# brunohs1993/Nanokappa

Hardware: AMD Instinct MI355X
Metric: phonon-steps/sec (whole node) (higher is better)
Workload: dtype f64

## Files before the change

nanokappa_amd/csrc/nk_device.h:

```cpp
#pragma once
#include <hip/hip_runtime.h>
#include <stdint.h>

#define NK_WG 256
#ifndef NK_NREP
#define NK_NREP 8
#endif
#define NK_PLANE_DOUBLES 6
#define NK_FACE_DOUBLES 16
#define NK_LDS_FACES 256
#define NK_LDS_RESFACES 64
#define NK_TAU_ROWS 3
#define NK_MAX_SEGMENTS 16384
#define NK_EMIT_CHUNK 128
#define NK_LREC 128
#define NK_NEWBORN 0x80000000u
#define NK_LOST 0x40000000u

#define NK_TAG_REFLECT 0x00000u
#define NK_TAG_EMIT 0x10000u
#define NK_TAG_RESAMP 0x20000u
#define NK_TAG_DICE 0x30000u
#define NK_TAG_INIT 0x40000u

template <class T>
struct NkField {
    T *p;
    int32_t blk;
    __host__ __device__ __forceinline__ int64_t off(int64_t i) const { return (i >> 6) * (int64_t)blk + (i & 63); }
    __host__ __device__ __forceinline__ T &operator[](int64_t i) const { return p[off(i)]; }
    __host__ __device__ __forceinline__ T *operator+(int64_t i) const { return p + off(i); }
    __host__ __device__ __forceinline__ T *tile(int64_t i0, int lane) const { return p + ((i0 >> 6) * (int64_t)blk + lane); }
    __host__ __device__ __forceinline__ explicit operator bool() const { return p != nullptr; }
};

template <bool NTS, bool PID>
struct NkBlock {
    static constexpr int NF = 4 + (NTS ? 1 : 0) + (PID ? 1 : 0);
    static constexpr int BD = NF * 64 + 32;
    static constexpr int O_Y = 64, O_Z = 128, O_OCC = 192, O_NTS = 256, O_PID = 64 * (NTS ? 5 : 4), O_W0 = 64 * NF;
    static __device__ __forceinline__ double *slot(double *s0, int64_t i) { return s0 + (i >> 6) * (int64_t)BD + (i & 63); }
    static __device__ __forceinline__ double *tile(double *s0, int64_t i0, int lane) { return s0 + (i0 >> 6) * (int64_t)BD + lane; }
    static __device__ __forceinline__ uint32_t *word(double *s0, int64_t i) { return reinterpret_cast<uint32_t *>(s0 + (i >> 6) * (int64_t)BD + O_W0) + (i & 63); }
};

struct __attribute__((aligned(16))) NkFacet {
    double cx, cy, cz;
    double nx, ny, nz;
    double tx, ty, tz;
    int32_t bc;
    int32_t partner;
    int32_t res;
    int32_t rough;
    int32_t pad[2];
};

struct __attribute__((aligned(64))) NkMode {
    double omega, vx, vy, vz;
    double E0;
    double tau[NK_TAU_ROWS];
};

struct NkDev {
    int32_t Q, J, NT, M;
    const NkMode *modetab;
    const NkMode *modetab_p;
    const int32_t *m2s;
    const int32_t *s2m;
    const int32_t *seg_nl;
    int32_t tau_row0;
    double tau_g[NK_TAU_ROWS];
    double tau_ig[NK_TAU_ROWS - 1];
    double T0, invT0;
    double c_hk;
    const double *tau;
    const double *Tgrid;
    int32_t nE;
    const double *Tarr, *Earr;
    double Tfill_lo, Tfill_hi;
    double hbar, kb, QV;
    double active_modes;
    int32_t F, Fc, NP;
    const float *tree_boxes;
    double tree_bound;
    const int32_t *tree_tags;
    const double *facet_skip;
    const double *tree_faces;
    int32_t tree_base[8];
    int32_t tree_top, tree_leaves;
    int32_t tree_nfam, tree_lds_fam0, tree_lds_off;
    int32_t NG;
    const double *planes;
    const double *faces;
    const NkFacet *facets;
    double tol;
    double bbox[6];
    int32_t box;
    double box_k[6];
    uint64_t box_ids;
    double inv_dt;
    const double *face_verts;
    const int32_t *facet_face_off;
    const int32_t *facet_face_idx;
    const double *facet_face_cdf;
    int32_t nS;
    const double *simplex_pts;
    const double *simplex_cdf;
    int32_t S, sv_kind, sv_axis, sv_interp;
    const double *centers;
    const double *sv_volume;
    double sv_lo, sv_invL;
    double *T_sv;
    const double *rbf_inv;
    int32_t rbf_P, rbf_used[3];
    double rbf_shift[3], rbf_scale[3];
    int32_t R, res_gen;
    const int32_t *res_facet;
    const double *res_T;
    const int32_t *res_face_off;
    const double *res_face_cdf;
    const double *res_face_verts;
    int32_t res_nf;
    int32_t res_lds;
    const double *enter_prob;
    double *res_counter;
    const double *ep_p;
    double *rc_p;
    int64_t rc_len;
    const double *res_roulette;
    int32_t *nleave_prev;
    uint64_t *sp_inbox;
    int32_t *sp_inbox_n;
    int32_t sp_icap;
    int32_t Fr;
    const double *specularity;
    const uint8_t *true_spec;
    const int32_t *spec_map;
    const double *roulette;
    const int32_t *roul_lut;
    int32_t roul_nlut;
    const int32_t *degen_j2;
    double dt;
    int32_t norm_fixed, T_ref_local;
    double particle_density, T_ref;
    uint64_t seed;
    int32_t rank, nranks;
    int64_t cap;
    int32_t nseg, segcap;
    int32_t *seg_count;
    int32_t *seg_new;
    int32_t *seg_lo;
    int32_t down;
    int32_t *seg_bound;
    NkField<double> x, y, z, occ, nts;
    NkField<uint32_t> w0;
    NkField<uint64_t> pid;
    int32_t part;
    int32_t lb;
    int32_t nlmax;
    int32_t nlrec;
    int32_t *ticket;
    int32_t *overflow;
    int32_t *halt;
    double *qx, *qy, *qz, *qocc, *qnts;
    uint32_t *qw0;
    uint64_t *qpid;
    int32_t *seg_evq;
    int32_t *ev_ticket;
    double2 *mig_buf;
    int32_t *mig_n;
    int32_t mig_cap;
    double *partials;
    int32_t NB;
    unsigned long long *stamps;
};

struct NkSlot { int64_t od, ow; };
__device__ __forceinline__ NkSlot nk_slot(const NkDev &d, int64_t i) {
    const int64_t b = i >> 6, l = i & 63;
    NkSlot s;
    s.od = b * (int64_t)d.x.blk + l;
    s.ow = b * (int64_t)d.w0.blk + l;
    return s;
}

__device__ __forceinline__ void nk_philox(uint32_t c0, uint32_t c1, uint32_t c2, uint32_t c3, uint32_t k0, uint32_t k1,
                                          uint32_t o[4]) {
#pragma unroll
    for (int r = 0; r < 10; ++r) {
        uint32_t hi0 = __umulhi(0xD2511F53u, c0), lo0 = 0xD2511F53u * c0;
        uint32_t hi1 = __umulhi(0xCD9E8D57u, c2), lo1 = 0xCD9E8D57u * c2;
        uint32_t n0 = hi1 ^ c1 ^ k0, n2 = hi0 ^ c3 ^ k1;
        c0 = n0; c1 = lo1; c2 = n2; c3 = lo0;
        k0 += 0x9E3779B9u; k1 += 0xBB67AE85u;
    }
    o[0] = c0; o[1] = c1; o[2] = c2; o[3] = c3;
}
__device__ __forceinline__ double nk_u53(uint32_t hi, uint32_t lo) {
    uint64_t w = ((uint64_t)hi << 32) | lo;
    return (double)(w >> 11) * (1.0 / 9007199254740992.0);
}
__device__ __forceinline__ void nk_uniform2_dev(uint64_t seed, uint64_t pid, uint32_t step, uint32_t tag, double &u0,
                                                double &u1) {
    uint32_t o[4];
    nk_philox((uint32_t)pid, (uint32_t)(pid >> 32), step, tag, (uint32_t)seed, (uint32_t)(seed >> 32), o);
    u0 = nk_u53(o[0], o[1]);
    u1 = nk_u53(o[2], o[3]);
}

__device__ __forceinline__ int nk_ss_left(const double *a, int n, double x) {
    int lo = 0, hi = n;
    while (lo < hi) { int mid = (lo + hi) >> 1; if (a[mid] < x) lo = mid + 1; else hi = mid; }
    return lo;
}
__device__ __forceinline__ int nk_ss_right(const double *a, int n, double x) {
    int lo = 0, hi = n;
    while (lo < hi) { int mid = (lo + hi) >> 1; if (a[mid] <= x) lo = mid + 1; else hi = mid; }
    return lo;
}
__device__ __forceinline__ int nk_ss_left_hint(const double *a, int n, double x, int hint) {
    int lo, hi;
    hint = hint < 0 ? 0 : (hint > n - 1 ? n - 1 : hint);
    if (a[hint] < x) {
        int stepw = 1;
        lo = hint + 1; hi = lo;
        while (hi < n && a[hi] < x) { lo = hi + 1; hi += stepw; stepw <<= 1; }
        if (hi > n) hi = n;
    } else {
        int stepw = 1;
        hi = hint; lo = hint;
        while (lo > 0 && !(a[lo - 1] < x)) { hi = lo - 1; lo -= stepw; stepw <<= 1; if (lo < 0) lo = 0; }
        if (lo > 0 && !(a[lo - 1] < x)) lo = 0;
    }
    while (lo < hi) { int mid = (lo + hi) >> 1; if (a[mid] < x) lo = mid + 1; else hi = mid; }
    return lo;
}
__device__ __forceinline__ double nk_interp_lin_hint(const double *xs, const double *ys, int n, double x, int hint, int &idx_out) {
    int idx = nk_ss_left_hint(xs, n, x, hint);
// ... 664 lines not shown
```

nanokappa_amd/csrc/nk_engine.hip:

```cpp
#include <hip/hip_runtime.h>
#include <dlfcn.h>
#include <math.h>
#include <stdio.h>
#include <stdlib.h>
#include <string.h>
#include <algorithm>
#include <functional>
#include <queue>
#include <string>
#include <type_traits>
#include <chrono>
#include <time.h>
#include <vector>

#include <rccl/rccl.h>

#include "../../include/nanokappa_hip.h"
#include "nk_kernels.h"
#include "nk_field.h"
#include "nk_fgroups.h"
#include "nk_modes.h"
#include "nk_group.h"
#ifndef NK_PLAIN_IN_ENGINE
extern template __global__ void k_sweep<1, false, false, false, false, true, 1>(NkDev, uint32_t, int, int);
// ... 59 lines not shown
    double *rb_k2 = nullptr, *rb_nin = nullptr, *rb_eta = nullptr, *rb_sub = nullptr, *rb_spec = nullptr, *rb_roul = nullptr;
    uint8_t *rb_ts = nullptr;
    unsigned int *rb_map = nullptr;
    std::vector<int32_t> rb_facet;
    int64_t o2o_first = 0;
    bool stepped = false;
    int64_t emitted_for = -1;
    std::vector<double> h_vg;
    std::vector<int32_t> h_m2s, h_s2m;
    int32_t *m2s_dev = nullptr, *s2m_dev = nullptr, *nl_dev = nullptr;
    unsigned int *rbar = nullptr;
    bool walked = false;
    int64_t ev_lds_set = -1;
    int map_nseg = 0;
    NkMode *modetab_p = nullptr;
    int64_t modetab_p_len = 0;
    void *inbox = nullptr, *inbox_n = nullptr;
    void *mig_buf = nullptr, *mig_n = nullptr;
    double *ep_p = nullptr, *rc_p = nullptr;
    int rm_nseg = 0, rm_nlmax = 0;
    void *pin = nullptr;
    size_t pin_bytes = 0;
    int32_t halt_words[4] = {0, 0, 0, 0};
    double *acc = nullptr;
    double *hist = nullptr;
    int hist_cap = 0;
    nk_params params;
    nk_timing timing;
    NkRccl rccl;
    ncclComm_t comm = nullptr;
    int comm_rank = -1, comm_nranks = 0;
    double comm_selftest = 0.0;
    int num_cu = 256;
    std::vector<int32_t> h_ffo, h_ffi;
    std::vector<double> h_fcdf, h_verts;
    std::vector<double> h_rbf_inv;
    std::vector<NkFacet> host_facets;
    const double *d_omega = nullptr, *d_vg = nullptr;
    std::vector<double> h_Tgrid;
    double T_lo = 0.0, T_hi = 0.0;
    int32_t band_B = 0;
    int32_t *band_map = nullptr;
    double *band_slabs = nullptr;
    size_t band_slabs_n = 0;
    double *band_rows_d = nullptr;
    size_t band_rows_n = 0;
    std::vector<double> band_rows;
    std::vector<int64_t> band_steps;
    NkFieldHost field;
    NkFGroupsHost fgroups;
    int64_t map_gen = 0;
    NkModesHost modes;
    double res_T_max = 0.0;
};

#define NK_HIP(call)                                                                                   \
    do {                                                                                               \
        hipError_t e_ = (call);                                                                        \
        if (e_ != hipSuccess) {                                                                        \
            ctx->err = std::string(#call) + ": " + hipGetErrorString(e_);                              \
            return NK_ERR_HIP;                                                                         \
        }                                                                                              \
    } while (0)
#define NK_ARG(cond, msg)                                                                              \
    do {                                                                                               \
        if (!(cond)) { ctx->err = msg; return NK_ERR_ARG; }                                            \
    } while (0)

template <class T>
static int nk_upload(nk_ctx *ctx, const T *src, size_t n, const T **dst, bool particle = false) {
    void *p = nullptr;
    size_t bytes = (n ? n : 1) * sizeof(T);
    NK_HIP(hipMalloc(&p, bytes));
    (particle ? ctx->pallocs : ctx->allocs).push_back(p);
    if (src && n) NK_HIP(hipMemcpy(p, src, n * sizeof(T), hipMemcpyHostToDevice));
    else NK_HIP(hipMemset(p, 0, bytes));
    *dst = (const T *)p;
    return NK_OK;
}
#define NK_UP(src, n, dst)                                                                             \
    do { int rc_ = nk_upload(ctx, src, n, dst); if (rc_) return rc_; } while (0)

static inline bool nk_layout_soa() { return false; }
static inline int nk_particle_bytes(bool with_pid, bool with_nts) { return 36 + (with_nts ? 8 : 0) + (with_pid ? 8 : 0); }
static inline size_t nk_store_bytes(int64_t cap, bool with_pid, bool with_nts) {
    const int64_t nblk = (cap + 63) / 64;
    const int nf = 4 + (with_nts ? 1 : 0) + (with_pid ? 1 : 0);
    const int bd = nf * 64 + 32;
    const size_t bytes = nk_layout_soa() ? (size_t)nblk * 64 * (nf * 8 + 4) : (size_t)nblk * bd * 8;
    return bytes ? bytes : 64;
}
static void nk_point_fields(NkDev &d, double *b, int64_t cap, bool with_pid, bool with_nts) {
    const int64_t nblk = (cap + 63) / 64;
    const int nf = 4 + (with_nts ? 1 : 0) + (with_pid ? 1 : 0);
    const int bd = nf * 64 + 32;
    if (nk_layout_soa()) {
        const int64_t n = nblk * 64;
        int k = 4;
        d.x = {b, 64}; d.y = {b + n, 64}; d.z = {b + 2 * n, 64}; d.occ = {b + 3 * n, 64};
        d.nts = {with_nts ? b + (k++) * n : nullptr, 64};
        d.pid = {with_pid ? (uint64_t *)(b + (k++) * n) : nullptr, 64};
        d.w0 = {(uint32_t *)(b + k * n), 64};
    } else {
        int k = 4;
        d.x = {b, bd}; d.y = {b + 64, bd}; d.z = {b + 128, bd}; d.occ = {b + 192, bd};
        d.nts = {with_nts ? b + 64 * (k++) : nullptr, bd};
        d.pid = {with_pid ? (uint64_t *)(b + 64 * (k++)) : nullptr, bd};
        d.w0 = {(uint32_t *)(b + 64 * k), 2 * bd};
    }
}
static int nk_alloc_fields(nk_ctx *ctx, NkDev &d, int64_t cap, bool with_pid, bool with_nts) {
    const size_t bytes = nk_store_bytes(cap, with_pid, with_nts);
    void *buf = nullptr;
    const size_t pad = getenv("NK_STORE_PAD_KB") ? (size_t)atol(getenv("NK_STORE_PAD_KB")) * 1024 : 0;
    NK_HIP(hipMalloc(&buf, bytes + pad));
    ctx->pallocs.push_back(buf);
    NK_HIP(hipMemsetAsync(buf, 0, bytes + pad, ctx->stream));
    ctx->store_buf = buf; ctx->store_pad = pad; ctx->store_pid = with_pid; ctx->store_nts = with_nts;
    nk_point_fields(d, (double *)((char *)buf + pad), cap, with_pid, with_nts);
    return NK_OK;
}
template <class T>
static int nk_field_download(nk_ctx *ctx, const NkDev &d, const NkField<T> &f, std::vector<T> &out) {
    out.resize((size_t)d.cap);
    const int64_t nblk = d.cap / 64;
    if (nblk == 0) return NK_OK;
    NK_HIP(hipMemcpy2D(out.data(), 64 * sizeof(T), f.p, (size_t)f.blk * sizeof(T), 64 * sizeof(T), (size_t)nblk, hipMemcpyDeviceToHost));
    return NK_OK;
}
template <class T>
static int nk_field_upload(nk_ctx *ctx, const NkDev &d, const NkField<T> &f, const T *src) {
    const int64_t nblk = d.cap / 64;
    if (nblk == 0) return NK_OK;
    NK_HIP(hipMemcpy2D(f.p, (size_t)f.blk * sizeof(T), src, 64 * sizeof(T), 64 * sizeof(T), (size_t)nblk, hipMemcpyHostToDevice));
    return NK_OK;
}

static inline int nk_geom_mode(const nk_ctx *ctx) { return (ctx->d.F <= NK_LDS_FACES && ctx->d.Fc <= NK_LDS_FACES) ? 1 : 2; }
static inline bool nk_want_split(const nk_ctx *ctx);
static inline size_t nk_lds(const nk_ctx *ctx, bool geom, int kind = 0) {
    const NkDev &d = ctx->d;
    const int gm = geom ? nk_geom_mode(ctx) : 0;
    return nk_lds_bytes(d.S, d.R, d.F, d.NP, d.Fc, gm, kind, (gm == 1 && d.res_lds) ? d.res_nf : 0, d.rbf_P, d.nlrec, nk_want_split(ctx) ? 0 : 1);
}
#define NK_GEOM_LAUNCH(kernel, grid, lds, ...)                                                        \
    do {                                                                                               \
        if (nk_geom_mode(ctx) == 1) kernel<1><<<grid, NK_WG, lds, ctx->stream>>>(__VA_ARGS__);         \
        else kernel<2><<<grid, NK_WG, lds, ctx->stream>>>(__VA_ARGS__);                                \
    } while (0)
#define NK_EMIT_LAUNCH(kernel, grid, lds, ...)                                                        \
    do {                                                                                               \
        if (ctx->d.box) kernel<1, true><<<grid, NK_WG, lds, ctx->stream>>>(__VA_ARGS__);               \
        else if (nk_geom_mode(ctx) == 1) kernel<1, false><<<grid, NK_WG, lds, ctx->stream>>>(__VA_ARGS__);   \
        else kernel<2, false><<<grid, NK_WG, lds, ctx->stream>>>(__VA_ARGS__);                         \
    } while (0)
static inline int nk_sweep_grid(const nk_ctx *ctx) { return ctx->num_cu * 8; }
#define NK_SWEEP_CASE(G, R, B, P, S, lrec, STMT) { if (lrec) { auto KERNEL = k_sweep<G, R, B, P, S, true>; STMT; } else { auto KERNEL = k_sweep<G, R, B, P, S, false>; STMT; } }
#define NK_SWEEP_CASE_FAST(lrec, fast, STMT)                                                                                   \
    { if (lrec) { if ((fast) == 1) { auto KERNEL = k_sweep<1, false, false, false, false, true, 1>; STMT; } else { auto KERNEL = k_sweep<1, false, false, false, false, true, 2>; STMT; } } \
      else { if ((fast) == 1) { auto KERNEL = k_sweep<1, false, false, false, false, false, 1>; STMT; } else { auto KERNEL = k_sweep<1, false, false, false, false, false, 2>; STMT; } } }
#define NK_SWEEP_CASE_S(G, R, B, P, split, lrec, STMT) { if (split) NK_SWEEP_CASE(G, R, B, P, true, lrec, STMT) else NK_SWEEP_CASE(G, R, B, P, false, lrec, STMT) }
#define NK_SWEEP_CASE_RP(G, B, rough, pid, split, lrec, STMT)                                         \
    { if (rough) NK_SWEEP_CASE_S(G, true, B, true, split, lrec, STMT) else if (pid) NK_SWEEP_CASE_S(G, false, B, true, split, lrec, STMT) else NK_SWEEP_CASE_S(G, false, B, false, split, lrec, STMT) }
#define NK_SWEEP_CASE_BOX(R, B, P, lrec, STMT) { if (lrec) { auto KERNEL = k_sweep<1, R, B, P, false, true, 0, true>; STMT; } else { auto KERNEL = k_sweep<1, R, B, P, false, false, 0, true>; STMT; } }
#define NK_SWEEP_CASE_BOX_RP(B, rough, pid, lrec, STMT)                                               \
    { if (rough) NK_SWEEP_CASE_BOX(true, B, true, lrec, STMT) else if (pid) NK_SWEEP_CASE_BOX(false, B, true, lrec, STMT) else NK_SWEEP_CASE_BOX(false, B, false, lrec, STMT) }
#define NK_SWEEP_CASE_FAST_BOX(lrec, fast, STMT)                                                                               \
    { if (lrec) { if ((fast) == 1) { auto KERNEL = k_sweep<1, false, false, false, false, true, 1, true>; STMT; } else { auto KERNEL = k_sweep<1, false, false, false, false, true, 2, true>; STMT; } } \
      else { if ((fast) == 1) { auto KERNEL = k_sweep<1, false, false, false, false, false, 1, true>; STMT; } else { auto KERNEL = k_sweep<1, false, false, false, false, false, 2, true>; STMT; } } }
#define NK_SWEEP_DISPATCH(gm, rough, rbf, pid, split, lrec, STMT)                                     \
    do {                                                                                               \
        const int fast_ = ((gm) == 1 && !(rough) && !(rbf) && !(pid) && !(split)) ? nk_sweep_fast(ctx) : 0;   \
        if (ctx->d.box && (gm) == 1 && !(split)) {                                                     \
            if (fast_) { NK_SWEEP_CASE_FAST_BOX(lrec, fast_, STMT) break; }                            \
            if (rbf) NK_SWEEP_CASE_BOX_RP(true, rough, pid, lrec, STMT) else NK_SWEEP_CASE_BOX_RP(false, rough, pid, lrec, STMT)   \
            break;                                                                                     \
        }                                                                                              \
        if (fast_) { NK_SWEEP_CASE_FAST(lrec, fast_, STMT) break; }                                    \
        if ((gm) == 1) { if (rbf) NK_SWEEP_CASE_RP(1, true, rough, pid, split, lrec, STMT) else NK_SWEEP_CASE_RP(1, false, rough, pid, split, lrec, STMT) }   \
        else { if (rbf) NK_SWEEP_CASE_RP(2, true, rough, pid, split, lrec, STMT) else NK_SWEEP_CASE_RP(2, false, rough, pid, split, lrec, STMT) }             \
    } while (0)
static inline int nk_sweep_fast(const nk_ctx *ctx) {
    const NkDev &d = ctx->d;
    if (getenv("NK_NO_FAST")) return 0;
    return (d.sv_kind == 0 && d.T_ref_local && (d.sv_interp == 0 || d.sv_interp == 1)) ? 1 + d.sv_interp : 0;
}
static inline bool nk_want_lrec(const nk_ctx *ctx) { return ctx->d.nlrec > 0; }
#define NK_EVENTS_CASE(G, R, B, P, STMT) { auto KERNEL = k_events<G, R, B, P>; STMT; }
#define NK_EVENTS_CASE_RP(G, B, rough, pid, STMT)                                                     \
    { if (rough) NK_EVENTS_CASE(G, true, B, true, STMT) else if (pid) NK_EVENTS_CASE(G, false, B, true, STMT) else NK_EVENTS_CASE(G, false, B, false, STMT) }
#define NK_EVENTS_DISPATCH(gm, rough, rbf, pid, STMT)                                                 \
// ... 478 lines not shown
    ctx->host_facets = fct;
    NK_UP(fct.data(), fct.size(), &d.facets);
    {
        std::vector<double> fs((size_t)m->Fc * 2, 0.0);
        for (int f = 0; f < m->F; ++f) {
            const int fc = m->face_facet[f];
            if (fc < 0 || fc >= m->Fc) continue;
            const NkFacet &q = fct[fc];
            const double nx = m->normals[3 * f], ny = m->normals[3 * f + 1], nz = m->normals[3 * f + 2];
            const double dn = std::max(fabs(nx - q.nx), std::max(fabs(ny - q.ny), fabs(nz - q.nz)));
            const double dk = fabs(nx * q.cx + ny * q.cy + nz * q.cz + m->k[f]);
            fs[2 * (size_t)fc] = std::max(fs[2 * (size_t)fc], dn);
            fs[2 * (size_t)fc + 1] = std::max(fs[2 * (size_t)fc + 1], dk);
        }
        std::vector<int> nfaces((size_t)m->Fc, 0);
        for (int f = 0; f < m->F; ++f) if (m->face_facet[f] >= 0 && m->face_facet[f] < m->Fc) ++nfaces[m->face_facet[f]];
        for (int fc = 0; fc < m->Fc; ++fc) if (nfaces[fc] < 16) fs[2 * (size_t)fc] = 1e300;
        NK_UP(fs.data(), fs.size(), &d.facet_skip);
    }
    d.nS = m->nS;
    if (m->nS > 0) {
        NK_UP(m->simplex_pts, (size_t)m->nS * 12, &d.simplex_pts);
        std::vector<double> sc((size_t)m->nS);
        double tot = 0.0, acc = 0.0;
        for (int s = 0; s < m->nS; ++s) tot += m->simplex_vol[s];
        for (int s = 0; s < m->nS; ++s) { acc += m->simplex_vol[s] / tot; sc[s] = acc; }
        for (int s = 0; s < m->nS; ++s) sc[s] /= sc[m->nS - 1];
        NK_UP(sc.data(), sc.size(), &d.simplex_cdf);
    }
    ctx->mesh_box = false;
    if (d.cap == 0) d.box = 0;
    if (m->F == 12 && m->Fc == 6 && d.NP == 6) {
        bool ok = true;
        int seen = 0;
        int box_facet[6] = {0, 0, 0, 0, 0, 0};
        d.box_ids = 0;
        for (int pl = 0; pl < 6 && ok; ++pl) {
            const double *pn = &planes[(size_t)pl * NK_PLANE_DOUBLES];
            int a = -1, sgn = 0;
            for (int k = 0; k < 3; ++k) {
                if (pn[k] == 1.0 || pn[k] == -1.0) { if (a >= 0) ok = false; a = k; sgn = pn[k] > 0 ? 1 : 0; }
                else if (pn[k] != 0.0) ok = false;
            }
            if (!ok || a < 0) { ok = false; break; }
            const int w = 2 * a + sgn;
            if (seen & (1 << w)) { ok = false; break; }
            seen |= 1 << w;
            const double wall = sgn ? -pn[3] : pn[3];
            if (!(fabs(wall - m->bbox[(sgn ? 3 : 0) + a]) <= 1e-9 * (1.0 + fabs(wall)))) { ok = false; break; }
            if (members[pl].size() != 2) { ok = false; break; }
            int fct0 = -1, face0 = 0x7fffffff;
            double area = 0.0;
            for (int f : members[pl]) {
                if (fct0 < 0) fct0 = m->face_facet[f]; else if (m->face_facet[f] != fct0) ok = false;
                face0 = std::min(face0, f);
                area += m->face_area[f];
                const double *V = m->vertices + 9 * (size_t)f;
                for (int c = 0; c < 3 && ok; ++c)
                    for (int k = 0; k < 3; ++k) {
                        const double v = V[3 * c + k], lo = m->bbox[k], hi = m->bbox[3 + k];
                        const double e = 1e-9 * (1.0 + fabs(lo) + fabs(hi));
                        if (k == a) { if (fabs(v - wall) > e) ok = false; }
                        else if (fabs(v - lo) > e && fabs(v - hi) > e) ok = false;
                    }
            }
            const int b = (a + 1) % 3, c = (a + 2) % 3;
            const double side = (m->bbox[3 + b] - m->bbox[b]) * (m->bbox[3 + c] - m->bbox[c]);
            if (!(fabs(area - side) <= 1e-9 * side) || fct0 < 0 || fct0 >= m->Fc) ok = false;
            if (!ok) break;
            d.box_k[w] = pn[3];
            box_facet[w] = fct0;
            d.box_ids = (d.box_ids & ~(0xFFull << (8 * w))) | ((uint64_t)(fct0 & 15) << (8 * w)) | ((uint64_t)(face0 & 15) << (8 * w + 4));
        }
        if (ok && seen == 63) {
            int fm = 0;
            for (int w = 0; w < 6; ++w) fm |= 1 << box_facet[w];
            ctx->mesh_box = fm == 63;
        }
    }
    ctx->have_mesh = true;
    return NK_OK;
}

static inline bool nk_want_box(const nk_ctx *ctx) {
    return ctx->have_mesh && ctx->mesh_box && !ctx->box_forbidden && !getenv("NK_NO_BOX") && !getenv("NK_SPLIT") && !nk_layout_soa() &&
           ctx->d.F <= NK_LDS_FACES && ctx->d.Fc <= NK_LDS_FACES;
}

static int nk_patch_facets(nk_ctx *ctx) {
    NK_HIP(hipMemcpy((void *)ctx->d.facets, ctx->host_facets.data(), (size_t)ctx->d.Fc * sizeof(NkFacet), hipMemcpyHostToDevice));
    return NK_OK;
}

static int nk_entry_tables_drop(nk_ctx *ctx, bool keep_counters) {
    NkDev &d = ctx->d;
    if (ctx->rm_nseg > 0 && keep_counters && d.R > 0 && d.res_counter) {
        const int64_t n = (int64_t)d.R * d.M;
        k_perm_rm<<<(int)((n + 255) / 256), 256, 0, ctx->stream>>>(0, d.R, d.M, ctx->rm_nseg, ctx->rm_nlmax,
                                                                   d.m2s, d.res_counter, ctx->rc_p + (ctx->step & 1) * d.rc_len);
        NK_HIP(hipGetLastError());
        NK_HIP(hipStreamSynchronize(ctx->stream));
    }
    if (ctx->ep_p) { hipFree(ctx->ep_p); ctx->ep_p = nullptr; }
    if (ctx->rc_p) { hipFree(ctx->rc_p); ctx->rc_p = nullptr; }
    d.ep_p = nullptr; d.rc_p = nullptr;
    ctx->rm_nseg = 0;
    return NK_OK;
}
static int nk_entry_tables_build(nk_ctx *ctx) {
    NkDev &d = ctx->d;
    if (!(d.R > 0 && d.nseg > 0 && d.m2s && d.enter_prob && d.res_counter) || ctx->rm_nseg == d.nseg) return NK_OK;
    int rc = nk_entry_tables_drop(ctx, true);
    if (rc) return rc;
    const size_t len = (size_t)d.nseg * d.R * d.nlmax;
    NK_HIP(hipMalloc((void **)&ctx->ep_p, len * 8));
    NK_HIP(hipMalloc((void **)&ctx->rc_p, 2 * len * 8));
    NK_HIP(hipMemsetAsync(ctx->ep_p, 0, len * 8, ctx->stream));
    NK_HIP(hipMemsetAsync(ctx->rc_p, 0, 2 * len * 8, ctx->stream));
    d.rc_len = (int64_t)len;
    const int64_t n = (int64_t)d.R * d.M;
    k_perm_rm<<<(int)((n + 255) / 256), 256, 0, ctx->stream>>>(1, d.R, d.M, d.nseg, d.nlmax, d.m2s, (double *)d.enter_prob, ctx->ep_p);
    k_perm_rm<<<(int)((n + 255) / 256), 256, 0, ctx->stream>>>(1, d.R, d.M, d.nseg, d.nlmax, d.m2s, d.res_counter, ctx->rc_p + (ctx->step & 1) * d.rc_len);
    NK_HIP(hipGetLastError());
    d.ep_p = ctx->ep_p; d.rc_p = ctx->rc_p;
    ctx->rm_nseg = d.nseg;
    ctx->rm_nlmax = d.nlmax;
    return NK_OK;
}

static int nk_alloc_tally(nk_ctx *ctx) {
    NkDev &d = ctx->d;
    d.NB = 5 * d.S + 5 * d.R + 1;
    if (ctx->acc) { hipFree(ctx->acc); ctx->acc = nullptr; }
    if (ctx->hist) { hipHostFree(ctx->hist); ctx->hist = nullptr; }
    ctx->hist_cap = 0;
    NK_HIP(hipMalloc((void **)&ctx->acc, (size_t)(d.NB + 2) * sizeof(double)));
    NK_HIP(hipMemset(ctx->acc, 0, (size_t)(d.NB + 2) * sizeof(double)));
    const double *p;
    NK_UP((const double *)nullptr, (size_t)(ctx->num_cu * 16) * d.NB, &p);
    d.partials = (double *)p;
    return NK_OK;
}

static void nk_rbf_coefficients(nk_ctx *ctx, std::vector<double> &T) {
    const int S = ctx->d.S, P = ctx->d.rbf_P;
    T.resize((size_t)S + P);
    for (int j = 0; j < P; ++j) {
        double a = 0.0;
        for (int i = 0; i < S; ++i) a += ctx->h_rbf_inv[(size_t)j * P + i] * T[i];
        T[(size_t)S + j] = a;
    }
}

int nk_set_subvolumes(nk_ctx *ctx, const nk_subvols *s, const double *T_sv_init) {
    if (ctx) ctx->emitted_for = -1;
    NK_ARG(ctx && s && T_sv_init, "nk_set_subvolumes: NULL argument");
    NK_ARG(s->S > 0 && s->S <= 512, "nk_set_subvolumes: S must be in [1, 512]");
    NK_ARG(ctx->have_material, "nk_set_subvolumes: call nk_set_material first");
    NK_HIP(hipSetDevice(ctx->device));
    NkDev &d = ctx->d;
    d.S = s->S; d.sv_kind = s->kind; d.sv_axis = s->axis; d.sv_interp = s->interp;
    NK_ARG(s->axis >= 0 && s->axis < 3, "nk_set_subvolumes: axis");
    NK_ARG(!(s->kind != 0 && s->interp != 2 && s->interp != 3), "nk_set_subvolumes: slice interpolation needs slice subvolumes");
    NK_ARG(s->interp >= 0 && s->interp <= 3, "nk_set_subvolumes: interp must be 0..3");
    NK_UP(s->centers, (size_t)s->S * 3, &d.centers);
    NK_UP(s->volumes, (size_t)s->S, &d.sv_volume);
    d.rbf_P = 0;
// ... 134 lines not shown
        }
        if (r->degen_j2) NK_UP(r->degen_j2, (size_t)d.M, &d.degen_j2); else d.degen_j2 = nullptr;
        for (int i = 0; i < r->Fr; ++i) {
            NK_ARG(r->facet[i] >= 0 && r->facet[i] < d.Fc, "nk_set_rough: facet index");
            ctx->host_facets[r->facet[i]].rough = i;
        }
        return nk_patch_facets(ctx);
    }
    return NK_OK;
}

int nk_set_params(nk_ctx *ctx, const nk_params *p) {
    if (ctx) ctx->emitted_for = -1;
    NK_ARG(ctx && p, "nk_set_params: NULL argument");
    NK_ARG(p->dt > 0, "nk_set_params: dt must be positive");
    ctx->params = *p;
    NkDev &d = ctx->d;
    d.dt = p->dt; d.inv_dt = 1.0 / p->dt; d.norm_fixed = p->norm_fixed; d.particle_density = p->particle_density;
    d.T_ref_local = p->T_ref_local; d.T_ref = p->T_ref;
    ctx->have_params = true;
    return NK_OK;
}

struct NkHostParticles {
    std::vector<double> x, y, z, occ, nts;
    std::vector<int32_t> mode, facet;
    std::vector<uint64_t> pid;
};
static int nk_normalize(nk_ctx *ctx, int honor_halt = 0) {
    NkDev &d = ctx->d;
    d.down = 0;
    if (!ctx->walked || !d.seg_lo) return NK_OK;
    k_anchor<<<ctx->num_cu * 8, NK_WG, 0, ctx->stream>>>(d, honor_halt);
    NK_HIP(hipGetLastError());
    if (!honor_halt) ctx->walked = false;
    return NK_OK;
}
static int nk_gather_live(nk_ctx *ctx, NkHostParticles &h, bool want_all) {
    NkDev &d = ctx->d;
    if (d.cap == 0) return NK_OK;
    { int rcn_ = nk_normalize(ctx); if (rcn_) return rcn_; }
    NK_HIP(hipStreamSynchronize(ctx->stream));
    std::vector<int32_t> cnt((size_t)d.nseg);
    NK_HIP(hipMemcpy(cnt.data(), d.seg_count, (size_t)d.nseg * 4, hipMemcpyDeviceToHost));
    int64_t live = 0;
    for (int c : cnt) live += c;
    ctx->h_seg_count = cnt;
    if (!want_all) { h.x.resize((size_t)live); return NK_OK; }
    std::vector<double> bd;
    std::vector<uint32_t> bw;
    std::vector<uint64_t> bu;
    auto keep = [&](const auto &all, auto *dst) {
        for (int sgm = 0; sgm < d.nseg; ++sgm) {
            memcpy(dst, all.data() + (size_t)sgm * d.segcap, (size_t)cnt[sgm] * sizeof(*dst));
            dst += cnt[sgm];
        }
    };
    h.x.resize(live); h.y.resize(live); h.z.resize(live); h.occ.resize(live); h.nts.resize(live);
    h.mode.resize(live); h.facet.resize(live); h.pid.assign(live, 0);
    std::vector<uint32_t> w0((size_t)live);
    int rc;
    if ((rc = nk_field_download(ctx, d, d.x, bd))) return rc; keep(bd, h.x.data());
    if ((rc = nk_field_download(ctx, d, d.y, bd))) return rc; keep(bd, h.y.data());
    if ((rc = nk_field_download(ctx, d, d.z, bd))) return rc; keep(bd, h.z.data());
    if ((rc = nk_field_download(ctx, d, d.occ, bd))) return rc; keep(bd, h.occ.data());
    std::vector<int32_t> bfc;
    if (d.nts) { if ((rc = nk_field_download(ctx, d, d.nts, bd))) return rc; keep(bd, h.nts.data()); }
    else {
        if (ctx->have_material && ctx->have_mesh && ctx->have_sv && d.modetab) {
            double *dn = nullptr; int32_t *df = nullptr;
            NK_HIP(hipMalloc((void **)&dn, (size_t)d.cap * 8));
            if (hipMalloc((void **)&df, (size_t)d.cap * 4) != hipSuccess) { hipFree(dn); ctx->err = "nk_gather_live: out of memory"; return NK_ERR_HIP; }
            hipMemsetAsync(dn, 0, (size_t)d.cap * 8, ctx->stream); hipMemsetAsync(df, 0xff, (size_t)d.cap * 4, ctx->stream);
            k_next_hit<1><<<nk_sweep_grid(ctx), NK_WG, nk_lds(ctx, true), ctx->stream>>>(d, dn, df);
            bd.resize((size_t)d.cap); bfc.resize((size_t)d.cap);
            hipError_t e1 = hipGetLastError();
            if (e1 == hipSuccess) e1 = hipMemcpy(bd.data(), dn, (size_t)d.cap * 8, hipMemcpyDeviceToHost);
            if (e1 == hipSuccess) e1 = hipMemcpy(bfc.data(), df, (size_t)d.cap * 4, hipMemcpyDeviceToHost);
            hipFree(dn); hipFree(df);
            if (e1 != hipSuccess) { ctx->err = std::string("nk_gather_live: ") + hipGetErrorString(e1); return NK_ERR_HIP; }
            keep(bd, h.nts.data());
        } else { std::fill(h.nts.begin(), h.nts.end(), 0.0); }
    }
    if ((rc = nk_field_download(ctx, d, d.w0, bw))) return rc; keep(bw, w0.data());
    if (d.pid) { if ((rc = nk_field_download(ctx, d, d.pid, bu))) return rc; keep(bu, h.pid.data()); }
    const uint32_t lbmask = (1u << d.lb) - 1u;
    int64_t k = 0;
    for (int sgm = 0; sgm < d.nseg; ++sgm)
        for (int j = 0; j < cnt[sgm]; ++j, ++k) {
            const uint32_t idx = w0[(size_t)k] & lbmask;
            h.mode[(size_t)k] = d.part ? ctx->h_s2m[(size_t)sgm * d.nlmax + idx] : (int32_t)idx;
            if (d.nts) h.facet[(size_t)k] = (int32_t)(w0[(size_t)k] >> d.lb) - 1;
            else h.facet[(size_t)k] = (w0[(size_t)k] & NK_LOST) ? -1 : (bfc.empty() ? 0 : bfc[(size_t)sgm * d.segcap + j]);
        }
    return NK_OK;
}

static int nk_scatter(nk_ctx *ctx, int64_t N, const double *x, const double *y, const double *z, const int32_t *mode,
                      const double *occ, const double *n_ts, const int32_t *facet, const uint64_t *pid, uint64_t pid_offset) {
    if (ctx) ctx->emitted_for = -1;
    NkDev &d = ctx->d;
    const int M = d.M;
    for (int64_t i = 0; i < N; ++i) NK_ARG(mode[i] >= 0 && mode[i] < M, "nk_upload_particles: mode index out of range");
    std::vector<int64_t> order((size_t)N);
    std::vector<int64_t> start((size_t)d.nseg + 1, 0);
    if (d.part) {
        const std::vector<int32_t> &m2s = ctx->h_m2s;
        for (int64_t i = 0; i < N; ++i) start[(size_t)(m2s[(size_t)mode[i]] % d.nseg) + 1] += 1;
        for (int sgm = 0; sgm < d.nseg; ++sgm) start[(size_t)sgm + 1] += start[(size_t)sgm];
        std::vector<int64_t> key((size_t)N);
        for (int64_t i = 0; i < N; ++i) { order[(size_t)i] = i; key[(size_t)i] = (int64_t)(m2s[(size_t)mode[i]] % d.nseg) * ((int64_t)d.nlmax + 1) + m2s[(size_t)mode[i]] / d.nseg; }
        std::stable_sort(order.begin(), order.end(), [&](int64_t a, int64_t b) { return key[(size_t)a] < key[(size_t)b]; });
    } else {
        std::vector<int64_t> mstart((size_t)M + 1, 0);
        for (int64_t i = 0; i < N; ++i) mstart[(size_t)mode[i] + 1] += 1;
        for (int m = 0; m < M; ++m) mstart[(size_t)m + 1] += mstart[(size_t)m];
        std::vector<int64_t> cur(mstart.begin(), mstart.end() - 1);
        for (int64_t i = 0; i < N; ++i) order[(size_t)cur[(size_t)mode[i]]++] = i;
        for (int sgm = 0; sgm <= d.nseg; ++sgm) start[(size_t)sgm] = (N * sgm) / d.nseg;
    }
    std::vector<int32_t> cnt((size_t)d.nseg);
    for (int sgm = 0; sgm < d.nseg; ++sgm) {
        cnt[(size_t)sgm] = (int32_t)(start[(size_t)sgm + 1] - start[(size_t)sgm]);
        NK_ARG(cnt[(size_t)sgm] <= d.segcap, "nk_upload_particles: segment capacity too small");
    }
    auto put = [&](const auto *src, const auto &field) -> int {
        typedef typename std::remove_const<typename std::remove_pointer<decltype(src)>::type>::type T;
        std::vector<T> all((size_t)d.cap, T(0));
        for (int sgm = 0; sgm < d.nseg; ++sgm) {
            const int64_t lo = start[(size_t)sgm], n = cnt[(size_t)sgm];
            T *o = all.data() + (size_t)sgm * d.segcap;
            for (int64_t k = 0; k < n; ++k) o[k] = src[order[(size_t)(lo + k)]];
        }
        return nk_field_upload(ctx, d, field, all.data());
    };
    int rc;
    if ((rc = put(x, d.x)) || (rc = put(y, d.y)) || (rc = put(z, d.z)) || (rc = put(occ, d.occ))) return rc;
    if (n_ts && d.nts && (rc = put(n_ts, d.nts))) return rc;
    {
        std::vector<uint32_t> w0((size_t)N);
        for (int64_t i = 0; i < N; ++i) {
            const int32_t fc = facet ? facet[i] : -1;
            NK_ARG(fc >= -1 && fc < d.Fc, "nk_upload_particles: facet index out of range");
            const uint32_t idx = d.part ? (uint32_t)(ctx->h_m2s[(size_t)mode[i]] / d.nseg) : (uint32_t)mode[i];
            w0[(size_t)i] = d.nts ? (((uint32_t)(fc + 1) << d.lb) | idx) : (((facet && fc < 0) ? NK_LOST : 0u) | idx);
        }
        if ((rc = put((const uint32_t *)w0.data(), d.w0))) return rc;
    }
    if (d.pid) {
        if (pid) { if ((rc = put(pid, d.pid))) return rc; }
        else {
            std::vector<uint64_t> ids((size_t)N);
            for (int64_t i = 0; i < N; ++i) ids[(size_t)i] = pid_offset + (uint64_t)i;
            if ((rc = put((const uint64_t *)ids.data(), d.pid))) return rc;
        }
    }
    NK_HIP(hipMemcpy(d.seg_count, cnt.data(), (size_t)d.nseg * 4, hipMemcpyHostToDevice));
    if (d.seg_lo) NK_HIP(hipMemset(d.seg_lo, 0, (size_t)d.nseg * 4));
    ctx->walked = false;
    ctx->h_seg_count = cnt;
    return NK_OK;
}

static inline bool nk_want_pid(const nk_ctx *ctx) { return ctx->d.Fr > 0 || ctx->params.track_ids != 0; }
static inline bool nk_want_split(const nk_ctx *ctx) {
    if (const char *e = getenv("NK_SPLIT")) return atoi(e) != 0;
    return ctx->have_mesh && !(ctx->d.F <= NK_LDS_FACES && ctx->d.Fc <= NK_LDS_FACES);
}
static inline bool nk_want_part(const nk_ctx *ctx) { return !getenv("NK_NO_PARTITION"); }

static int nk_sweep_blocks(nk_ctx *ctx) {
    NkDev &d = ctx->d;
    if (!(ctx->have_material && ctx->have_mesh && ctx->have_sv)) return ctx->num_cu * NK_SWEEP_OCC;
    const int gm_ = nk_geom_mode(ctx);
    const bool rough_ = d.Fr > 0, rbf_ = d.sv_interp == 3, pid_ = nk_want_pid(ctx), split_ = nk_want_split(ctx);
    const bool lrec_ = nk_want_lrec(ctx);
    const int key = gm_ | (rough_ << 2) | (rbf_ << 3) | (pid_ << 4) | (split_ << 5) | (lrec_ << 6) | (nk_sweep_fast(ctx) << 7) | ((d.box ? 1 : 0) << 9);
    const size_t lds_w = nk_lds(ctx, true, pid_ ? 3 : 2);
    if (ctx->g_sweep == 0 || ctx->g_sweep_key != key || ctx->g_sweep_lds != lds_w) {
        int per_cu = 0;
        hipError_t e_ = hipSuccess;
        NK_SWEEP_DISPATCH(gm_, rough_, rbf_, pid_, split_, lrec_, (e_ = hipOccupancyMaxActiveBlocksPerMultiprocessor(&per_cu, KERNEL, NK_WG, lds_w)));
        if (e_ != hipSuccess || per_cu < 1) per_cu = 1;
        if (per_cu > 8) per_cu = 8;
        { const int bound = NK_SWEEP_BOUND(gm_, rough_, rbf_, split_); if (per_cu > bound) per_cu = bound; }
        if (const char *e = getenv("NK_SWEEP_PER_CU")) { int v = atoi(e); if (v >= 1 && v < per_cu) per_cu = v; }
        ctx->g_sweep = ctx->num_cu * per_cu;
        ctx->g_sweep_key = key;
        ctx->g_sweep_lds = lds_w;
        if (getenv("NK_VERBOSE")) fprintf(stderr, "[nanokappa_hip] sweep: %d workgroups per CU (occupancy query rc %d), %zu B LDS each\n", per_cu, (int)e_, lds_w);
    }
    return ctx->g_sweep;
}

static inline int nk_mode_seg(const nk_ctx *ctx, int m, int nseg) {
    return (ctx->map_nseg == nseg && !ctx->h_m2s.empty()) ? ctx->h_m2s[(size_t)m] % nseg : m % nseg;
}

static int nk_build_mode_map(nk_ctx *ctx) {
    NkDev &d = ctx->d;
    if (ctx->m2s_dev) { hipFree(ctx->m2s_dev); ctx->m2s_dev = nullptr; }
    if (ctx->s2m_dev) { hipFree(ctx->s2m_dev); ctx->s2m_dev = nullptr; }
    if (ctx->nl_dev) { hipFree(ctx->nl_dev); ctx->nl_dev = nullptr; }
    d.m2s = nullptr; d.s2m = nullptr; d.seg_nl = nullptr;
    ctx->h_m2s.clear(); ctx->h_s2m.clear(); ctx->map_nseg = 0;
    ctx->map_gen += 1;
    if (d.M <= 0 || d.nseg <= 0) return NK_OK;
    const int M = d.M, nseg = d.nseg, nlmax = d.nlmax;
    const bool plain = !d.part;
    std::vector<int32_t> nl((size_t)nseg, 0);
    ctx->h_m2s.assign((size_t)M, 0);
    ctx->h_s2m.assign((size_t)nseg * nlmax, -1);
    auto place = [&](int m, int seg) {
        const int l = nl[(size_t)seg]++;
        ctx->h_m2s[(size_t)m] = l * nseg + seg;
        ctx->h_s2m[(size_t)seg * nlmax + l] = m;
    };
    if (plain) {
        for (int m = 0; m < M; ++m) place(m, m % nseg);
    } else {
        std::vector<double> rate((size_t)M, 0.0);
        std::vector<char> active((size_t)M, 1);
        const bool have_v = ctx->h_vg.size() == (size_t)M * 3;
        if (have_v) {
            double inv[3] = {0, 0, 0};
            if (ctx->have_mesh) for (int a = 0; a < 3; ++a) { const double e = d.bbox[3 + a] - d.bbox[a]; inv[a] = e > 0.0 ? 1.0 / e : 0.0; }
            for (int m = 0; m < M; ++m) {
                const double *v = &ctx->h_vg[3 * (size_t)m];
                active[(size_t)m] = (v[0] != 0.0 || v[1] != 0.0 || v[2] != 0.0) ? 1 : 0;
                rate[(size_t)m] = fabs(v[0]) * inv[0] + fabs(v[1]) * inv[1] + fabs(v[2]) * inv[2];
// ... 102 lines not shown
        if (hi > 1.12 * lo && !force) break;
        if (bytes * cand.size() > free_b / 3) break;
        if (std::chrono::duration<double, std::milli>(std::chrono::steady_clock::now() - wall0).count() > 1000.0) break;
        void *buf = nullptr;
        if (hipMalloc(&buf, bytes) != hipSuccess) { (void)hipGetLastError(); break; }
        cand.push_back(buf); ms.push_back(0.0);
        if (hipMemsetAsync(buf, 0, bytes, ctx->stream) != hipSuccess) { rc = NK_ERR_HIP; ctx->err = "nk_place_store: hipMemsetAsync failed"; break; }
        rc = probe(buf, ms.back());
    }
    hipEventDestroy(e0); hipEventDestroy(e1);
    size_t best = 0, worst = 0;
    for (size_t k = 1; k < cand.size(); ++k) { if (ms[k] < ms[best]) best = k; if (ms[k] > ms[worst]) worst = k; }
    if (force) best = cand.size() - 1;
    if (!rc && best != 0 && (ms[best] < 0.97 * ms[0] || force)) {
        if (hipMemcpyAsync(cand[best], cand[0], bytes, hipMemcpyDeviceToDevice, ctx->stream) != hipSuccess ||
            hipStreamSynchronize(ctx->stream) != hipSuccess) { rc = NK_ERR_HIP; ctx->err = "nk_place_store: copy into the chosen store failed"; }
        else {
            for (void *&p : ctx->pallocs) if (p == cand[0]) p = cand[best];
            ctx->store_buf = cand[best];
            nk_point_fields(d, (double *)cand[best], d.cap, ctx->store_pid, ctx->store_nts);
            std::swap(cand[0], cand[best]);
        }
    } else best = 0;
    for (size_t k = 1; k < cand.size(); ++k) hipFree(cand[k]);
    const double gb = 2.0 * (double)d.nseg * tiles * 64 * (pbytes - (ctx->store_pid ? 8 : 0)) / 1e9;
    ctx->timing.place_tries = (int64_t)cand.size();
    ctx->timing.place_gbps = ms[best] > 0.0 ? gb / (ms[best] * 1e-3) : 0.0;
    ctx->timing.place_worst_gbps = ms[worst] > 0.0 ? gb / (ms[worst] * 1e-3) : 0.0;
    if (rc) {
        if (getenv("NK_VERBOSE")) fprintf(stderr, "[nanokappa_hip] store placement: probe failed (%s); the store stays where it is\n", ctx->err.c_str());
        (void)hipGetLastError();
        rc = NK_OK;
    }
    if (getenv("NK_VERBOSE")) {
        fprintf(stderr, "[nanokappa_hip] store placement: %zu allocation(s) of %.0f MB probed:", cand.size(), (double)bytes / 1048576.0);
        for (size_t k = 0; k < ms.size(); ++k) fprintf(stderr, " %.1f", ms[k] * 1e3);
        fprintf(stderr, " us per pass; kept number %zu (%.2f TB/s); %.1f ms\n", best, ctx->timing.place_gbps / 1e3,
                std::chrono::duration<double, std::milli>(std::chrono::steady_clock::now() - wall0).count());
    }
    return rc;
}

static inline int64_t nk_tiled_count(int64_t u, int64_t nu, int64_t pid_lo, int64_t N) {
    const int64_t first = pid_lo % nu;
    return N / nu + (((u - first + nu) % nu) < N % nu ? 1 : 0);
}
static int nk_alloc_particles(nk_ctx *ctx, int64_t capacity, const int32_t *mode = nullptr, int64_t N = 0,
                              const int32_t *umodes = nullptr, int64_t nu = 0, int64_t pid_lo = 0) {
    if (ctx) ctx->emitted_for = -1;
    NkDev &d = ctx->d;
    { int rc0 = nk_entry_tables_drop(ctx, true); if (rc0) return rc0; }
    for (void *p : ctx->pallocs) hipFree(p);
    ctx->pallocs.clear();
    d.part = nk_want_part(ctx) ? 1 : 0;
    d.box = nk_want_box(ctx) ? 1 : 0;
    d.nlrec = 0;
    int64_t nseg = 0;
    for (int round = 0; round < 4; ++round) {
        const int64_t waves = (int64_t)nk_sweep_blocks(ctx) * (NK_WG / 64);
        int64_t ns = capacity / 128;
        if (const char *e = getenv("NK_SEGMENTS")) ns = atoi(e) > 0 ? atoi(e) : ns;
        else if (ns >= waves) ns = waves;
        ns = ns < 64 ? 64 : (ns > NK_MAX_SEGMENTS ? NK_MAX_SEGMENTS : ns);
        const bool same = ns == nseg;
        nseg = ns;
        d.nseg = (int32_t)nseg;
        d.nlmax = d.M > 0 ? (int32_t)((d.M + nseg - 1) / nseg) : 1;
        if (d.part && d.M > nseg) d.nlmax += d.nlmax / 6 + 2;
        d.nlrec = 0;
        if (d.part && d.nlmax <= NK_LREC && !getenv("NK_NO_LREC")) {
            const int without = nk_sweep_blocks(ctx);
            d.nlrec = d.nlmax;
            if (nk_sweep_blocks(ctx) < without) d.nlrec = 0;
        }
        if (same) break;
    }
    NK_ARG(d.nlmax < (1 << 14), "too many modes per segment for k_emit's packed entry word: use more particles (segments) or fewer modes");
    { int rcm = nk_build_mode_map(ctx); if (rcm) return rcm; }
    {
        const int64_t maxidx = d.part ? d.nlmax - 1 : (d.M > 0 ? d.M - 1 : 0);
        int lb = 1;
        while ((1ll << lb) <= maxidx) ++lb;
        NK_ARG(lb < 30 && (int64_t)d.Fc + 1 < (1ll << (31 - lb)), "mesh has too many facets for the packed particle word (facets x modes)");
        d.lb = lb;
    }
    int64_t segcap = (capacity + nseg - 1) / nseg;
    if (d.part && (mode || umodes) && N > 0) {
        std::vector<int64_t> per((size_t)nseg, 0);
        if (mode) { for (int64_t i = 0; i < N; ++i) if (mode[i] >= 0 && mode[i] < d.M) per[(size_t)nk_mode_seg(ctx, mode[i], (int)nseg)] += 1; }
        else for (int64_t u = 0; u < nu; ++u) per[(size_t)nk_mode_seg(ctx, umodes[u], (int)nseg)] += nk_tiled_count(u, nu, pid_lo, N);
        int64_t mx = 0;
        for (int64_t v : per) mx = std::max(mx, v);
        segcap = std::max(segcap, mx + mx / 4 + 64);
    }
    const bool tight = getenv("NK_TIGHT_STORE") != nullptr;
    if (ctx->have_material && d.R > 0 && !ctx->h_enter_prob.empty())
        segcap = (tight ? segcap : std::max(segcap, segcap / 8 * 9)) + (tight ? 1 : 2) * nk_spawn_bound(ctx, (int)nseg) + 2 * NK_TILE;
    segcap = ((segcap + 63) / 64) * 64;
    NK_ARG(nseg * segcap < (1ll << 31), "particle store too large for 32-bit slot arithmetic");
    d.segcap = (int32_t)segcap;
    d.cap = nseg * segcap;
    ctx->timing.slots = d.cap;
    const double *pd; const uint32_t *pw; const int32_t *pi; const uint64_t *pu;
#define NK_PALLOC(T, field, ptr, count)                                                                \
    do { int rc_ = nk_upload<T>(ctx, nullptr, (size_t)(count), &ptr, true); if (rc_) return rc_; d.field = (T *)ptr; } while (0)
    { int rcf = nk_alloc_fields(ctx, d, d.cap, nk_want_pid(ctx), !d.box); if (rcf) return rcf; }
    NK_PALLOC(int32_t, seg_count, pi, d.nseg);
    NK_PALLOC(int32_t, seg_new, pi, d.nseg);
    NK_PALLOC(int32_t, seg_bound, pi, d.nseg);
    d.seg_lo = nullptr; d.down = 0; ctx->walked = false;
    NK_PALLOC(int32_t, seg_lo, pi, d.nseg);
    d.qx = d.qy = d.qz = d.qocc = d.qnts = nullptr; d.qw0 = nullptr; d.qpid = nullptr; d.seg_evq = nullptr;
    if (nk_want_split(ctx)) {
        NK_PALLOC(double, qx, pd, d.cap); NK_PALLOC(double, qy, pd, d.cap); NK_PALLOC(double, qz, pd, d.cap);
        NK_PALLOC(double, qocc, pd, d.cap); NK_PALLOC(double, qnts, pd, d.cap);
        NK_PALLOC(uint32_t, qw0, pw, d.cap);
        if (d.pid) NK_PALLOC(uint64_t, qpid, pu, d.cap);
        NK_PALLOC(int32_t, seg_evq, pi, 2 * (size_t)d.nseg + 1);
    }
#ifdef NK_STAMPS
    { const unsigned long long *ps; int rc_ = nk_upload<unsigned long long>(ctx, nullptr, (size_t)d.nseg * 16, &ps, true); if (rc_) return rc_; d.stamps = (unsigned long long *)ps; }
#endif
#undef NK_PALLOC
    ctx->layout_key = (d.part ? 1 : 0) | (d.pid ? 2 : 0) | (d.qx ? 4 : 0) | (d.box ? 8 : 0);
    if (ctx->have_material) { int rc = nk_update_tau_window(ctx, true); if (rc) return rc; }
    if (ctx->inbox) { hipFree(ctx->inbox); ctx->inbox = nullptr; }
    if (ctx->inbox_n) { hipFree(ctx->inbox_n); ctx->inbox_n = nullptr; }
    d.sp_inbox = nullptr; d.sp_inbox_n = nullptr; d.sp_icap = 0;
    if (ctx->mig_buf) { hipFree(ctx->mig_buf); ctx->mig_buf = nullptr; }
    if (ctx->mig_n) { hipFree(ctx->mig_n); ctx->mig_n = nullptr; }
    d.mig_buf = nullptr; d.mig_n = nullptr; d.mig_cap = 0;
    { int rcp = nk_place_store(ctx); if (rcp) return rcp; }
    return nk_entry_tables_build(ctx);
}

static int nk_ensure_migration(nk_ctx *ctx, int64_t cap) {
    NkDev &d = ctx->d;
    if (!(d.Fr > 0 && d.part)) return NK_OK;
    if (cap <= 0) cap = std::max<int64_t>(256, d.segcap / 2);
    if (d.mig_buf && d.mig_cap >= cap) return NK_OK;
    if (ctx->mig_buf) { hipFree(ctx->mig_buf); ctx->mig_buf = nullptr; }
    if (ctx->mig_n) { hipFree(ctx->mig_n); ctx->mig_n = nullptr; }
    d.mig_buf = nullptr; d.mig_n = nullptr; d.mig_cap = 0;
    NK_HIP(hipMalloc(&ctx->mig_buf, (size_t)d.nseg * cap * 64));
    NK_HIP(hipMalloc(&ctx->mig_n, (size_t)d.nseg * 4));
    NK_HIP(hipMemset(ctx->mig_n, 0, (size_t)d.nseg * 4));
    d.mig_buf = (double2 *)ctx->mig_buf; d.mig_n = (int32_t *)ctx->mig_n; d.mig_cap = (int32_t)cap;
    return NK_OK;
}

static int nk_ensure_inbox(nk_ctx *ctx) {
    NkDev &d = ctx->d;
    if (!(d.R > 0 && d.res_gen == 2) || d.sp_inbox) return NK_OK;
    const int64_t icap = 4 * (ctx->o2o_first / d.nseg + 64);
    NK_HIP(hipMalloc(&ctx->inbox, (size_t)d.nseg * icap * 8));
    NK_HIP(hipMalloc(&ctx->inbox_n, (size_t)d.nseg * 4));
    NK_HIP(hipMemset(ctx->inbox_n, 0, (size_t)d.nseg * 4));
    d.sp_inbox = (uint64_t *)ctx->inbox; d.sp_inbox_n = (int32_t *)ctx->inbox_n; d.sp_icap = (int32_t)icap;
    return NK_OK;
}

static int nk_regrow(nk_ctx *ctx, int64_t segcap_new) {
    if (ctx) ctx->emitted_for = -1;
    { int rcn_ = nk_normalize(ctx); if (rcn_) return rcn_; }
    NkDev &d = ctx->d;
    NK_HIP(hipStreamSynchronize(ctx->stream));
// ... 1866 lines not shown
    NK_BUF(double, dxc, nullptr, n * 3); NK_BUF(double, dtc, nullptr, n); NK_BUF(int32_t, dfc, nullptr, n);
    const bool verbose = getenv("NK_VERBOSE") != nullptr;
    hipEvent_t e0 = nullptr, e1 = nullptr;
    if (verbose) { NK_HIP(hipEventCreate(&e0)); NK_HIP(hipEventCreate(&e1)); NK_HIP(hipEventRecord(e0, ctx->stream)); }
    NK_GEOM_LAUNCH(k_tap_find_boundary, (int)((n + NK_WG - 1) / NK_WG), nk_lds(ctx, true), d, n, dx.p, dv.p, dxc.p, dtc.p, dfc.p);
    NK_HIP(hipGetLastError());
    if (verbose) NK_HIP(hipEventRecord(e1, ctx->stream));
    NK_HIP(hipStreamSynchronize(ctx->stream));
    if (verbose) {
        float ms = 0.f;
        hipEventElapsedTime(&ms, e0, e1);
        fprintf(stderr, "[nanokappa_hip] find_boundary: %lld rays in %.3f ms\n", (long long)n, ms);
        hipEventDestroy(e0); hipEventDestroy(e1);
    }
    NK_HIP(dxc.get(xc, n * 3)); NK_HIP(dtc.get(tc, n)); NK_HIP(dfc.get(fc, n));
    return NK_OK;
}
int nk_classify(nk_ctx *ctx, int64_t n, const double *x, int32_t *id) {
    NK_ARG(ctx && ctx->have_sv && n > 0 && x && id, "nk_classify: bad arguments");
    NK_HIP(hipSetDevice(ctx->device));
    NK_BUF(double, dx, x, n * 3); NK_BUF(int32_t, did, nullptr, n);
    k_tap_classify<<<(int)((n + NK_WG - 1) / NK_WG), NK_WG, nk_lds(ctx, false), ctx->stream>>>(ctx->d, n, dx.p, did.p);
    NK_HIP(hipGetLastError());
    NK_HIP(hipStreamSynchronize(ctx->stream));
    NK_HIP(did.get(id, n));
    return NK_OK;
}
int nk_eval(nk_ctx *ctx, int32_t what, int64_t n, const double *a, const int32_t *mode, double *out) {
    NK_ARG(ctx && ctx->have_material && n > 0 && a && out && what >= 0 && what <= 5, "nk_eval: bad arguments");
    NK_ARG(what > 1 || mode, "nk_eval: mode required");
    NK_ARG(ctx->have_sv, "nk_eval: subvolumes required");
    NK_HIP(hipSetDevice(ctx->device));
    const int64_t na = what == 4 ? 3 * n : n;
    NK_BUF(double, da, a, na); NK_BUF(int32_t, dm, mode, n); NK_BUF(double, dout, nullptr, n);
    k_tap_eval<<<(int)((n + NK_WG - 1) / NK_WG), NK_WG, nk_lds(ctx, false), ctx->stream>>>(ctx->d, what, n, da.p, mode ? dm.p : nullptr, dout.p);
    NK_HIP(hipGetLastError());
    NK_HIP(hipStreamSynchronize(ctx->stream));
    NK_HIP(dout.get(out, n));
    return NK_OK;
}
int nk_reflect(nk_ctx *ctx, int64_t n, const int32_t *facet, const int32_t *mode_in, const double *col_pos,
               const double *n_in, const double *omega_in, const double *r_spec, const double *r_deg,
               const double *r_diff, int32_t *mode_out, double *n_out, double *omega_out) {
    NK_ARG(ctx && ctx->have_material && ctx->have_sv && ctx->have_mesh && ctx->d.Fr > 0 && n > 0, "nk_reflect: engine not configured");
    NK_ARG(facet && mode_in && col_pos && n_in && omega_in && r_spec && r_diff, "nk_reflect: NULL input");
    for (int64_t i = 0; i < n; ++i)
        NK_ARG(facet[i] >= 0 && facet[i] < ctx->d.Fc && ctx->host_facets[facet[i]].rough >= 0, "nk_reflect: facet is not rough");
    NK_HIP(hipSetDevice(ctx->device));
    NK_BUF(int32_t, df, facet, n); NK_BUF(int32_t, dm, mode_in, n); NK_BUF(double, dc, col_pos, n * 3);
    NK_BUF(double, dn, n_in, n); NK_BUF(double, dom, omega_in, n); NK_BUF(double, drs, r_spec, n);
    NK_BUF(double, drd, r_deg, n); NK_BUF(double, drf, r_diff, n);
    NK_BUF(int32_t, dmo, nullptr, n); NK_BUF(double, dno, nullptr, n); NK_BUF(double, doo, nullptr, n);
    k_tap_reflect<<<(int)((n + NK_WG - 1) / NK_WG), NK_WG, nk_lds(ctx, false), ctx->stream>>>(
        ctx->d, n, df.p, dm.p, dc.p, dn.p, dom.p, drs.p, r_deg ? drd.p : nullptr, drf.p, dmo.p, dno.p, doo.p);
    NK_HIP(hipGetLastError());
    NK_HIP(hipStreamSynchronize(ctx->stream));
    NK_HIP(dmo.get(mode_out, n)); NK_HIP(dno.get(n_out, n)); NK_HIP(doo.get(omega_out, n));
    return NK_OK;
}
int nk_calibrate_stream(nk_ctx *ctx, int32_t launches, int64_t *bytes_read, int64_t *bytes_written) {
    NK_ARG(ctx && launches > 0 && ctx->d.cap > 0, "nk_calibrate_stream: bad arguments");
    NK_HIP(hipSetDevice(ctx->device));
    NK_HIP(hipStreamSynchronize(ctx->stream));
    NkHostParticles h;
    { int rc = nk_gather_live(ctx, h, false); if (rc) return rc; }
    const int64_t ns = (int64_t)h.x.size();
    for (int k = 0; k < launches; ++k) k_cal_stream<<<nk_sweep_grid(ctx), NK_WG, 0, ctx->stream>>>(ctx->d);
    NK_HIP(hipGetLastError());
    NK_HIP(hipStreamSynchronize(ctx->stream));
    if (const char *pc = getenv("NK_PROBE_COPY")) {
        hipEvent_t e0, e1;
        NK_HIP(hipEventCreate(&e0)); NK_HIP(hipEventCreate(&e1));
        const int g = ctx->g_sweep > 0 ? ctx->g_sweep : ctx->num_cu * 3;
        for (int w = 8; w <= 16; w += 8) {
            if (atoi(pc) != w && atoi(pc) != 0) continue;
            for (int rep = 0; rep < 3; ++rep) {
                NK_HIP(hipEventRecord(e0, ctx->stream));
                for (int k = 0; k < 10; ++k) { if (w == 8) k_probe_copy<8><<<g, NK_WG, 0, ctx->stream>>>(ctx->d); else k_probe_copy<16><<<g, NK_WG, 0, ctx->stream>>>(ctx->d); }
                NK_HIP(hipEventRecord(e1, ctx->stream));
                NK_HIP(hipStreamSynchronize(ctx->stream));
                float ms = 0.f;
                hipEventElapsedTime(&ms, e0, e1);
                fprintf(stderr, "[nanokappa_hip] copy probe, %d-byte accesses: %.1f us per pass over %lld particles (%.2f TB/s)\n", w, 100.0 * ms,
                        (long long)ns, (ctx->d.nts ? 88.0 : 72.0) * ns / (ms * 1e-4) / 1e12);
            }
        }
        hipEventDestroy(e0); hipEventDestroy(e1);
    }
    if (bytes_read) *bytes_read = ns * (ctx->d.nts ? 44 : 36);
    if (bytes_written) *bytes_written = ns * (ctx->d.nts ? 32 : 24);
    return NK_OK;
}
int nk_uniform2(uint64_t seed, uint64_t pid, uint32_t step, uint32_t tag, double *u0, double *u1) {
    if (!u0 || !u1) return NK_ERR_ARG;
    double *dout = nullptr, h[2];
    if (hipMalloc((void **)&dout, 16) != hipSuccess) return NK_ERR_HIP;
    k_tap_uniform<<<1, 1>>>(seed, pid, step, tag, dout);
    if (hipMemcpy(h, dout, 16, hipMemcpyDeviceToHost) != hipSuccess) { hipFree(dout); return NK_ERR_HIP; }
    hipFree(dout);
    *u0 = h[0]; *u1 = h[1];
    return NK_OK;
}

}


static void nk_specular_free(nk_ctx *ctx) {
    for (void *p : {(void *)ctx->spec_v, (void *)ctx->spec_om, (void *)ctx->spec_dl, (void *)ctx->spec_modes,
                    (void *)ctx->spec_in, (void *)ctx->spec_out, (void *)ctx->spec_count, (void *)ctx->spec_svx,
                    (void *)ctx->spec_rank, (void *)ctx->ks_kv, (void *)ctx->ks_mat})
        if (p) hipFree(p);
    ctx->ks_kv = ctx->ks_mat = nullptr; ctx->ks_Q = 0;
    ctx->spec_v = ctx->spec_om = ctx->spec_dl = ctx->spec_svx = nullptr;
    ctx->spec_rank = nullptr;
    ctx->spec_modes = nullptr; ctx->spec_in = ctx->spec_out = nullptr; ctx->spec_count = nullptr;
    ctx->spec_M = 0; ctx->spec_cap = 0;
}
int nk_specular_begin(nk_ctx *ctx, int64_t M, const double *group_vel, const double *omega, const double *delta_omega) {
    NK_ARG(ctx && M > 0 && M < (1ll << 31) && group_vel && omega && delta_omega, "nk_specular_begin: bad arguments");
    NK_HIP(hipSetDevice(ctx->device));
    nk_specular_free(ctx);
    NK_HIP(hipMalloc((void **)&ctx->spec_v, (size_t)M * 24));
    NK_HIP(hipMalloc((void **)&ctx->spec_om, (size_t)M * 8));
    NK_HIP(hipMalloc((void **)&ctx->spec_dl, (size_t)M * 8));
    NK_HIP(hipMalloc((void **)&ctx->spec_modes, (size_t)M * sizeof(NkSpecMode)));
    NK_HIP(hipMalloc((void **)&ctx->spec_count, 8));
    NK_HIP(hipMemcpy(ctx->spec_v, group_vel, (size_t)M * 24, hipMemcpyHostToDevice));
    NK_HIP(hipMemcpy(ctx->spec_om, omega, (size_t)M * 8, hipMemcpyHostToDevice));
    NK_HIP(hipMemcpy(ctx->spec_dl, delta_omega, (size_t)M * 8, hipMemcpyHostToDevice));
    std::vector<int32_t> order((size_t)M), rank((size_t)M);
    for (int64_t m = 0; m < M; ++m) order[(size_t)m] = (int32_t)m;
    std::stable_sort(order.begin(), order.end(), [&](int32_t p, int32_t q) { return group_vel[3 * (size_t)p] < group_vel[3 * (size_t)q]; });
    std::vector<double> svx((size_t)M);
    double vmax = 0.0;
    for (int64_t k = 0; k < M; ++k) {
        const size_t m = (size_t)order[(size_t)k];
        rank[m] = (int32_t)k;
        svx[(size_t)k] = group_vel[3 * m];
        const double vx = group_vel[3 * m], vy = group_vel[3 * m + 1], vz = group_vel[3 * m + 2];
        vmax = std::max(vmax, sqrt((vx * vx + vy * vy) + vz * vz));
    }
    NK_HIP(hipMalloc((void **)&ctx->spec_rank, (size_t)M * 4));
    NK_HIP(hipMalloc((void **)&ctx->spec_svx, (size_t)M * 8));
    NK_HIP(hipMemcpy(ctx->spec_rank, rank.data(), (size_t)M * 4, hipMemcpyHostToDevice));
    NK_HIP(hipMemcpy(ctx->spec_svx, svx.data(), (size_t)M * 8, hipMemcpyHostToDevice));
    ctx->spec_vmax = vmax;
    ctx->spec_M = M;
    return NK_OK;
}
int nk_specular_pairs(nk_ctx *ctx, const double *normal, double crit, int64_t cap, int32_t *pair_in, int32_t *pair_out,
                      int64_t *n_pairs) {
    NK_ARG(ctx && normal && n_pairs && cap >= 0 && ((pair_in != nullptr) == (pair_out != nullptr)), "nk_specular_pairs: bad arguments");
    NK_ARG(ctx->spec_M > 0, "nk_specular_pairs: call nk_specular_begin first");
    NK_HIP(hipSetDevice(ctx->device));
    const int M = (int)ctx->spec_M;
    if (cap > ctx->spec_cap) {
        if (ctx->spec_in) hipFree(ctx->spec_in);
        if (ctx->spec_out) hipFree(ctx->spec_out);
        ctx->spec_in = ctx->spec_out = nullptr;
        NK_HIP(hipMalloc((void **)&ctx->spec_in, (size_t)cap * 4));
        NK_HIP(hipMalloc((void **)&ctx->spec_out, (size_t)cap * 4));
        ctx->spec_cap = cap;
    }
    const int blocks = (M + NK_WG - 1) / NK_WG;
    NK_HIP(hipMemsetAsync(ctx->spec_count, 0, 8, ctx->stream));
    k_specular_prepare<<<blocks, NK_WG, 0, ctx->stream>>>(M, ctx->spec_v, ctx->spec_om, ctx->spec_dl, ctx->spec_rank, normal[0],
                                                          normal[1], normal[2], ctx->spec_modes);
    k_specular_pairs<<<blocks, NK_WG, 0, ctx->stream>>>(M, ctx->spec_modes, ctx->spec_svx, ctx->spec_vmax, normal[0], normal[1],
                                                        normal[2], crit, cap, ctx->spec_in, ctx->spec_out, ctx->spec_count);
    NK_HIP(hipGetLastError());
    NK_HIP(hipStreamSynchronize(ctx->stream));
    unsigned long long n = 0;
    NK_HIP(hipMemcpy(&n, ctx->spec_count, 8, hipMemcpyDeviceToHost));
// ... 179 lines not shown
```

nanokappa_amd/csrc/nk_fgroups.hip:

```cpp
#include <hip/hip_runtime.h>
#include <math.h>
#include <stdint.h>
#include <stdlib.h>
#include <string.h>
#include <algorithm>
#include "../../include/nanokappa_hip.h"
#define NK_KERNEL_LINKAGE template <int NK_NOT_IN_THIS_TU = 0>
#include "nk_kernels.h"
#include "nk_fgroups.h"

static const size_t NK_FG_LDS_MAX = 160 * 1024;
static const size_t NK_FG_LDS_LINE = 36;

struct NkFGroupsDev {
    const int32_t *gtab;
    int32_t gstride, glim;
    int32_t G, lines;
    unsigned long long *grid;
};
template <bool STATE>
__global__ __launch_bounds__(NK_FIELD_WG) void k_field_groups(NkDev d, NkFieldDev f, NkFGroupsDev q) {
    extern __shared__ __align__(16) unsigned char smem[];
    if (!STATE && d.halt[0]) return;
    NkLds L;
    nk_lds_setup<0, 0>(d, smem, L);
    const int nl = q.lines;
    unsigned long long *bR = (unsigned long long *)(smem + f.lds0);
    unsigned int *bN = (unsigned int *)(bR + 4 * (size_t)nl);
    if (f.lds_bins) {
        for (int i = threadIdx.x; i < 4 * nl; i += blockDim.x) bR[i] = 0ull;
        for (int i = threadIdx.x; i < nl; i += blockDim.x) bN[i] = 0u;
        __syncthreads();
    }
    unsigned long long *hdr = q.grid + (size_t)nl * 8;
    unsigned int n_clamped = 0, n_ovE = 0, n_ovF = 0, n_ung = 0, stuck = 0;
    const uint32_t lbmask = (1u << d.lb) - 1u;
    for (int seg = blockIdx.x; seg < d.nseg; seg += gridDim.x) {
        const int64_t base = (int64_t)seg * d.segcap + (d.seg_lo ? d.seg_lo[seg] : 0);
        const int count = d.seg_count[seg];
        if (!STATE && d.mig_buf && threadIdx.x == 0 && d.mig_n[seg] > 0) stuck = 1;
        const NkSegModes sm = nk_seg_modes(d, seg);
        const int32_t *gs = q.gtab + (int64_t)seg * q.gstride;
        for (int k = threadIdx.x; k < count; k += blockDim.x) {
            const int64_t i = base + k;
            const int idx = (int)(d.w0[i] & lbmask);
            const int g = idx < q.glim ? gs[idx] : -1;
            if ((unsigned)g >= (unsigned)q.G) { n_ung += 1u; continue; }
            const NkMode *rec = sm.rec + idx;
            const double x = d.x[i], y = d.y[i], z = d.z[i];
            double e;
            if (STATE) {
                double invT;
                const double T = nk_interp_T(d, L.tb, x, y, z, invT);
                const double n0 = !d.T_ref_local ? nk_occupation(d, d.T_ref, rec->omega, rec->E0)
                                                 : (T > 0.0 ? nk_be(rec->omega * d.c_hk, rec->E0, invT, d.invT0) : 0.0);
                e = d.hbar * rec->omega * (d.occ[i] - n0);
            } else {
                const int s = nk_classify(d, L.tb, x, y, z);
                e = nk_tally_e(d, L.tb, s, d.occ[i], rec->omega, rec->E0);
            }
            bool cl = false;
            const int ix = nk_field_axis(x, f.lo[0], f.inv_h[0], f.n[0], cl);
            const int iy = nk_field_axis(y, f.lo[1], f.inv_h[1], f.n[1], cl);
            const int iz = nk_field_axis(z, f.lo[2], f.inv_h[2], f.n[2], cl);
            n_clamped += cl ? 1u : 0u;
            const int b = ((ix * f.n[1] + iy) * f.n[2] + iz) * q.G + g;
            const double fx = rec->vx * e, fy = rec->vy * e, fz = rec->vz * e;
            const bool okE = fabs(e) <= f.BE;
            const bool okF = fabs(fx) <= f.BF && fabs(fy) <= f.BF && fabs(fz) <= f.BF;
            n_ovE += okE ? 0u : 1u;
            n_ovF += okF ? 0u : 1u;
            const unsigned long long qE = okE ? (unsigned long long)(long long)rint(e * f.sE) : 0ull;
            const unsigned long long qx = okF ? (unsigned long long)(long long)rint(fx * f.sF) : 0ull;
            const unsigned long long qy = okF ? (unsigned long long)(long long)rint(fy * f.sF) : 0ull;
            const unsigned long long qz = okF ? (unsigned long long)(long long)rint(fz * f.sF) : 0ull;
            if (f.lds_bins) {
                atomicAdd(bN + b, 1u);
                atomicAdd(bR + 4 * b + 0, qE);
                atomicAdd(bR + 4 * b + 1, qx);
                atomicAdd(bR + 4 * b + 2, qy);
                atomicAdd(bR + 4 * b + 3, qz);
            } else {
                unsigned long long *w = q.grid + (size_t)b * 8;
                atomicAdd(w + 0, 1ull);
                atomicAdd(w + 1, qE);
                atomicAdd(w + 2, qx);
                atomicAdd(w + 3, qy);
                atomicAdd(w + 4, qz);
            }
        }
    }
    if (n_clamped) atomicAdd(hdr + NK_FG_CLAMPED, (unsigned long long)n_clamped);
    if (n_ovE) atomicAdd(hdr + NK_FG_OVE, (unsigned long long)n_ovE);
    if (n_ovF) atomicAdd(hdr + NK_FG_OVF, (unsigned long long)n_ovF);
    if (n_ung) atomicAdd(hdr + NK_FG_UNGROUPED, (unsigned long long)n_ung);
    if (stuck) atomicAdd(hdr + NK_FG_SKIP, 1ull);
    if (blockIdx.x == 0 && threadIdx.x == 0) atomicAdd(hdr + NK_FG_RAN, 1ull);
    if (f.lds_bins) {
        __syncthreads();
        for (int b = threadIdx.x; b < nl; b += blockDim.x) {
            const unsigned int n = bN[b];
            if (n == 0u) continue;
            unsigned long long *w = q.grid + (size_t)b * 8;
            atomicAdd(w + 0, (unsigned long long)n);
#pragma unroll
            for (int k = 0; k < 4; ++k) { const unsigned long long v = bR[4 * b + k]; if (v) atomicAdd(w + 1 + k, v); }
        }
    }
}
__global__ __launch_bounds__(256) void k_fgroups_permute(const int32_t *s2m, const int32_t *table, int32_t *slot, int64_t n, int M) {
    const int64_t i = (int64_t)blockIdx.x * blockDim.x + threadIdx.x;
    if (i >= n) return;
    const int m = s2m[i];
    slot[i] = (unsigned)m < (unsigned)M ? table[m] : -1;
}
__global__ __launch_bounds__(256) void k_fgroups_accum(unsigned long long *grid, int lines, double sE, double sF, double *acc, int nranks) {
    const int b = blockIdx.x * blockDim.x + threadIdx.x;
    if (b >= lines) return;
    const unsigned long long *hdr = grid + (size_t)lines * 8;
    const bool take = hdr[NK_FG_RAN] == (unsigned long long)nranks && hdr[NK_FG_SKIP] == 0ull;
    unsigned long long *w = grid + (size_t)b * 8;
    if (take) {
        const double iE = 1.0 / sE, iF = 1.0 / sF;
        double *a = acc + (size_t)b * 5;
        a[0] += (double)(long long)w[0];
        a[1] += (double)(long long)w[1] * iE;
        a[2] += (double)(long long)w[2] * iF;
        a[3] += (double)(long long)w[3] * iF;
// ... 144 lines not shown
```

nanokappa_amd/csrc/nk_kernels.h:

```cpp
#pragma once
#ifndef NK_KERNEL_LINKAGE
#define NK_KERNEL_LINKAGE
#endif
#include "nk_device.h"

#define NK_TILE 64
#ifndef NK_NT
#define NK_NT 0
#endif
#if NK_NT
#define NK_LD(p) __builtin_nontemporal_load(p)
#define NK_ST(p, v) __builtin_nontemporal_store(v, p)
#else
#define NK_LD(p) (*(p))
#define NK_ST(p, v) (*(p) = (v))
#endif
#ifdef NK_STAMPS
#define NK_STAMP(k)                                                                                    \
    do {                                                                                               \
        unsigned long long t_;                                                                         \
        __builtin_amdgcn_sched_barrier(0);                                                             \
        asm volatile("s_memtime %0\n\ts_waitcnt lgkmcnt(0)" : "=s"(t_)::"memory");                     \
        __builtin_amdgcn_sched_barrier(0);                                                             \
        st_acc[k] += t_ - st_last;                                                                     \
// ... 345 lines not shown
        if (!em_t2) em_t2 = __builtin_amdgcn_s_memrealtime();
#endif
        for (int spj = 0; spj < spn; spj += NK_TILE) {
            const int j = spj + lane;
            if (j >= spn) continue;
            int64_t rm;
            int level, r, idx;
            double prob = 0.0, cval = 0.0;
            uint64_t o2o = 0;
            if (d.res_gen == 2) {
                const uint64_t recd = d.sp_inbox[(int64_t)seg * d.sp_icap + j];
                rm = (int64_t)((recd >> 12) & 0xFFFFFFFull);
                level = 0;
                o2o = recd >> 40;
                r = (int)((uint32_t)rm / (uint32_t)d.M);
                const int mode = (int)((uint32_t)rm - (uint32_t)r * (uint32_t)d.M);
                idx = d.part ? (int)((uint32_t)d.m2s[mode] / (uint32_t)d.nseg) : mode;
            } else {
                int lo = 0, hi = NK_EMIT_CHUNK;
                while (hi - lo > 1) { const int mid = (lo + hi) >> 1; if ((int)sp_pref[mid] <= j) lo = mid; else hi = mid; }
                const unsigned int cw = sp_cnt[lo];
                const int q = j - (int)sp_pref[lo], c = (int)(cw & 0xFFFu);
                r = (int)((cw >> 12) & 0x3Fu);
                rm = (int64_t)sp_rm[lo];
                idx = d.part ? (int)(cw >> 18) : (int)((uint32_t)rm - (uint32_t)r * (uint32_t)d.M);
                cval = sp_cv[lo];
                prob = sp_pr[lo];
                if (d.nranks == 1) level = c - q;
                else {
                    const uint32_t n = (uint32_t)d.nranks;
                    const uint32_t tq = ((uint32_t)d.rank + n - (((uint32_t)rm + step) % n)) % n;
                    const uint32_t top = (uint32_t)c - (((uint32_t)c + n - tq) % n);
                    level = (int)(top - (uint32_t)q * n);
                }
            }
            const NkMode *rec = sm.rec + idx;
            const double4 ra = *reinterpret_cast<const double4 *>(rec);
            const double E0 = rec->E0;
            const uint64_t pid = level > 0 ? ((uint64_t)((step + 1u) & 0xFFFFFFu) << 40) | ((uint64_t)rm << 12) | (uint64_t)level
                                           : ((uint64_t)((step + 1u) & 0xFFFFFFu) << 40) | ((uint64_t)r << 32) | o2o;
            double uf, us, ur, ut;
            nk_uniform2_dev(d.seed, pid, step, NK_TAG_EMIT, uf, us);
            nk_uniform2_dev(d.seed, pid, step, NK_TAG_EMIT + 1, ur, ut);
            const double iprob = level > 0 ? nk_rcp(prob) : 0.0;
            const double dt_in = (level == 0) ? d.dt * ut
                               : (level == 1) ? d.dt * (1.0 - cval * iprob)
                                              : d.dt * (1.0 - ((double)(level - 1) + ut) * iprob);
            double x0, y0, z0;
            if (GEOM == 1 && d.res_lds) nk_sample_res_face(L.rf_off, L.rf_cdf, L.rf_verts, r, uf, us, ur, x0, y0, z0);
            else nk_sample_res_face(d.res_face_off, d.res_face_cdf, d.res_face_verts, r, uf, us, ur, x0, y0, z0);
            const double omega = ra.x, vx = ra.y, vy = ra.z, vz = ra.w;
            const double occ = nk_be(omega * d.c_hk, E0, L.resT[2 * r + 1], d.invT0);
            if (GEOM == 2 && to_queue) {
                const int o = made + j;
                if (o < d.segcap) {
                    const int64_t i = base + o;
                    const int rf = d.res_facet[r];
                    const NkFacet &fq = d.facets[rf];
                    const int skip = nk_tree_skip(d, rf, fq.cx, fq.cy, fq.cz, fq.nx, fq.ny, fq.nz, x0, y0, z0, vx, vy, vz);
                    d.qx[i] = x0; d.qy[i] = y0; d.qz[i] = z0; d.qocc[i] = occ; d.qnts[i] = dt_in;
                    d.qw0[i] = NK_NEWBORN | ((uint32_t)((skip == rf ? rf : -1) + 1) << d.lb) | (uint32_t)idx;
                    if (d.qpid) d.qpid[i] = pid;
                } else if (!(ahead && d.halt[1])) atomicOr(d.overflow, 1);
                continue;
            }
            double tc = 0.0;
            int facet = -1;
            int skip = NK_TREE_NO_SKIP;
            if (GEOM == 2 && d.NG > 0) {
                const int rf = d.res_facet[r];
                const NkFacet &fq = d.facets[rf];
                skip = nk_tree_skip(d, rf, fq.cx, fq.cy, fq.cz, fq.nx, fq.ny, fq.nz, x0, y0, z0, vx, vy, vz);
            }
            if (!BOX) NK_RAY(GEOM, d, L, skip, x0, y0, z0, vx, vy, vz, tc, facet);
            const int o = count + made + j;
            if (plo + o < d.segcap) {
                const int64_t i = base + plo + o;
                const NkSlot q = nk_slot(d, i);
                double xa, ya, za, na;
                nk_newborn_place(d, x0, y0, z0, vx, vy, vz, dt_in, tc, xa, ya, za, na);
                d.x.p[q.od] = xa; d.y.p[q.od] = ya; d.z.p[q.od] = za;
                d.occ.p[q.od] = occ;
                if (!BOX) d.nts.p[q.od] = na;
                d.w0.p[q.ow] = BOX ? (NK_NEWBORN | (uint32_t)idx) : (NK_NEWBORN | ((uint32_t)(facet + 1) << d.lb) | (uint32_t)idx);
                if (d.pid) d.pid.p[q.od] = pid;
            } else if (!(ahead && d.halt[1])) atomicOr(d.overflow, 1);
        }
        made += spn;
        __builtin_amdgcn_fence(__ATOMIC_SEQ_CST, "wavefront");
    }
#pragma unroll
    for (int o = 32; o > 0; o >>= 1) sp_bound += __shfl_xor(sp_bound, o, 64);
    const int room = d.segcap - plo - count;
    const int put = (GEOM == 2 && to_queue) ? 0 : (made < room ? made : (room > 0 ? room : 0));
    if (lane == 0) {
        if (GEOM == 2 && to_queue) { d.seg_new[seg] = 0; d.seg_evq[seg] = made < d.segcap ? made : d.segcap; }
        else d.seg_new[seg] = put;
        d.seg_bound[seg] = sp_bound;
        if (d.res_gen == 2) d.sp_inbox_n[seg] = 0;
#ifdef NK_STAMPS
        if (d.stamps) { unsigned long long *w = d.stamps + ((int64_t)d.nseg + seg) * 8 + 4; w[0] = em_t0; w[1] = em_t1; w[2] = em_t2; w[3] = __builtin_amdgcn_s_memrealtime(); }
#endif
    }
    bound_out = sp_bound;
    return put;
}

template <int GEOM, bool BOX = false>
__device__ __forceinline__ void nk_emit_segments(const NkDev &d, NkLds L, uint32_t step, int bid, int nblocks, bool ahead
#ifdef NK_STAMPS
                                                 , unsigned long long em_t0, unsigned long long em_t1
#endif
) {
#ifdef NK_STAMPS
    unsigned long long em_t2 = 0;
#endif
    const int tid = threadIdx.x, lane = tid & 63, wave = __builtin_amdgcn_readfirstlane(tid >> 6);
    unsigned int *sp_pref = L.sp_pref + wave * NK_EMIT_CHUNK, *sp_cnt = L.sp_cnt + wave * NK_EMIT_CHUNK,
                 *sp_rm = L.sp_rm + wave * NK_EMIT_CHUNK;
    double *sp_cv = L.sp_cv + wave * NK_EMIT_CHUNK, *sp_pr = L.sp_pr + wave * NK_EMIT_CHUNK;
    const int nwaves = nblocks * (NK_WG / 64);
    const bool to_queue = GEOM == 2 && d.NG > 0 && d.qx != nullptr;
    for (int seg = bid * (NK_WG / 64) + wave; seg < d.nseg; seg += nwaves) {
        int bound_;
#ifdef NK_STAMPS
        (void)nk_emit_one<GEOM, BOX>(d, L, step, seg, lane, sp_pref, sp_cnt, sp_rm, sp_cv, sp_pr, ahead, to_queue, bound_, em_t0, em_t1, em_t2);
#else
        (void)nk_emit_one<GEOM, BOX>(d, L, step, seg, lane, sp_pref, sp_cnt, sp_rm, sp_cv, sp_pr, ahead, to_queue, bound_);
#endif
    }
}

template <int GEOM, bool BOX = false>
__device__ __forceinline__ void nk_emit_body(const NkDev &d, uint32_t step, unsigned char *smem, int bid, int nblocks, bool ahead = false) {
#ifdef NK_STAMPS
    const unsigned long long em_t0 = __builtin_amdgcn_s_memrealtime();
#endif
    if (d.halt[0]) return;
    NkLds L;
    nk_lds_setup<GEOM, 1>(d, smem, L);
#ifdef NK_STAMPS
    nk_emit_segments<GEOM, BOX>(d, L, step, bid, nblocks, ahead, em_t0, __builtin_amdgcn_s_memrealtime());
#else
    nk_emit_segments<GEOM, BOX>(d, L, step, bid, nblocks, ahead);
#endif
}

template <int GEOM, bool BOX = false>
__global__ __launch_bounds__(NK_WG) void k_emit(NkDev d, uint32_t step) {
    extern __shared__ __align__(16) unsigned char smem[];
    nk_emit_body<GEOM, BOX>(d, step, smem, (int)blockIdx.x, (int)gridDim.x);
}

template <bool PID>
struct NkOut {
    double *x, *y, *z, *occ, *nts, *pid;
    unsigned int *w0;
    int on, ob, wout;
    int64_t m0; int ms, mroom;
    __device__ __forceinline__ void place(int64_t first, int sign, int room) { m0 = first; ms = sign; mroom = room; }
    __device__ __forceinline__ void init(const NkLds &L, int wave) {
        double *p = L.oring + wave * NK_ORING * (PID ? 6 : 5);
        x = p; y = p + NK_ORING; z = p + 2 * NK_ORING; occ = p + 3 * NK_ORING; nts = p + 4 * NK_ORING; pid = PID ? p + 5 * NK_ORING : nullptr;
        w0 = L.oring_w + wave * NK_ORING;
        on = ob = wout = 0;
    }
    __device__ __forceinline__ int reserve(int rank, int n) { const int o = wout + rank; wout += n; return o; }
    template <bool BOX>
    static __device__ __forceinline__ void put_slot(const NkDev &d, int64_t i, double px, double py, double pz, double pocc, double pnts,
                                                    uint32_t pw0, unsigned long long ppid) {
        typedef NkBlock<!BOX, PID> B;
        double *q = B::slot(d.x.p, i);
        NK_ST(q, px); NK_ST(q + B::O_Y, py); NK_ST(q + B::O_Z, pz); NK_ST(q + B::O_OCC, pocc);
        if (!BOX) NK_ST(q + B::O_NTS, pnts);
        if (PID) NK_ST(reinterpret_cast<unsigned long long *>(q + B::O_PID), ppid);
        NK_ST(B::word(d.x.p, i), pw0);
    }
    template <bool BOX = false>
    __device__ __forceinline__ void store(const NkDev &d, int64_t base, bool put, int o, double px, double py, double pz, double pocc,
                                          double pnts, uint32_t pw0, unsigned long long ppid) {
        if (put) {
            if (o < mroom) put_slot<BOX>(d, m0 + ms * (int64_t)o, px, py, pz, pocc, pnts, pw0, ppid);
            else atomicOr(d.overflow, 2);
        }
    }
    template <bool BOX = false>
    __device__ __forceinline__ void push(const NkDev &d, int64_t base, int lane, bool put, int rank, int n, double px, double py,
                                         double pz, double pocc, double pnts, uint32_t pw0, unsigned long long ppid) {
        if (!NK_OUT_RING) {
            if (put) {
                const int o = wout + rank;
                if (o < mroom) put_slot<BOX>(d, m0 + ms * (int64_t)o, px, py, pz, pocc, pnts, pw0, ppid);
                else atomicOr(d.overflow, 2);
            }
            wout += n;
            return;
        }
        if (put) {
            const int e = (ob + on + rank) & (NK_ORING - 1);
            x[e] = px; y[e] = py; z[e] = pz; occ[e] = pocc; nts[e] = pnts; w0[e] = pw0;
            if (PID) pid[e] = __longlong_as_double((long long)ppid);
        }
        on += n;
        __builtin_amdgcn_fence(__ATOMIC_SEQ_CST, "wavefront");
        if (on >= NK_TILE) flush(d, base, lane, NK_TILE);
    }
    __device__ __forceinline__ void flush(const NkDev &d, int64_t base, int lane, int n) {
        if (wout + n <= d.segcap) {
            if (lane < n) {
                const int e = (ob + lane) & (NK_ORING - 1);
                const int64_t i = base + wout + lane;
                d.x[i] = x[e]; d.y[i] = y[e]; d.z[i] = z[e]; d.occ[i] = occ[e]; d.nts[i] = nts[e]; d.w0[i] = w0[e];
                if (PID) d.pid[i] = (unsigned long long)__double_as_longlong(pid[e]);
            }
            wout += n;
        } else if (lane == 0) atomicOr(d.overflow, 2);
        ob = (ob + n) & (NK_ORING - 1);
        on -= n;
        __builtin_amdgcn_fence(__ATOMIC_SEQ_CST, "wavefront");
    }
};

typedef double nk_v2d __attribute__((ext_vector_type(2)));
typedef const __attribute__((address_space(3))) nk_v2d *NkLdsRec;
__device__ __forceinline__ NkLdsRec nk_lds_rec(const double2 *q) { return (NkLdsRec)(const void *)q; }

#ifndef NK_SWEEP_OCC
#define NK_SWEEP_OCC 3
#endif
#ifndef NK_PREFETCH2
#define NK_PREFETCH2 0
#endif
#ifndef NK_PARK_TAU
#define NK_PARK_TAU 1
#endif
#ifndef NK_PRIO_ROT
#define NK_PRIO_ROT 0
#endif
#ifndef NK_DEFER_STORE
#define NK_DEFER_STORE 0
#endif
#ifndef NK_SWEEP_OCC_BIG
#define NK_SWEEP_OCC_BIG 2
#endif
#ifndef NK_SWEEP_OCC_SPLIT
#define NK_SWEEP_OCC_SPLIT 4
#endif
#define NK_SWEEP_BOUND(GEOM, ROUGH, RBF, SPLIT) ((SPLIT) ? NK_SWEEP_OCC_SPLIT : (((GEOM) == 2 || (RBF)) ? NK_SWEEP_OCC_BIG : NK_SWEEP_OCC))
template <int GEOM, bool ROUGH, bool RBF, bool PID, bool SPLIT, bool LREC, int FAST = 0, bool BOX = false>
__device__ __forceinline__ void nk_sweep_body(const NkDev &d, NkLds L, uint32_t step, int do_relax, int flags, int wg, int nwg
#ifdef NK_STAMPS
                                              , unsigned long long st_entry_r
#endif
) {
    static_assert(!BOX || (GEOM == 1 && !SPLIT && !NK_PREFETCH2 && !NK_OUT_RING), "the box store goes with the fused sweep over LDS tables");
    const bool do_flux = (flags & 1) != 0;
    const int tid = threadIdx.x, lane = tid & 63, wave = __builtin_amdgcn_readfirstlane(tid >> 6);
    const int rep = lane & (NK_NREP - 1);
    const uint32_t lbmask = (1u << d.lb) - 1u;
    NkBoxWalls bw;
    if (BOX) bw.load(d);
    NkTauWin tw;
    tw.load(d, NK_PARK_TAU != 0);
    double2 *lrec = reinterpret_cast<double2 *>(L.lrec) + wave * d.nlrec * NK_LREC_STRIDE;
    double *const cX = L.carry ? L.carry + wave * NK_CARRY_DOUBLES(PID ? 3 : 2) : nullptr;
    double *const cP = cX + 6 * 64;
    uint32_t *const cW = reinterpret_cast<uint32_t *>(cX + (PID ? 7 : 6) * 64);
    const int nwaves = nwg * (NK_WG / 64);
#if NK_PRIO_ROT
    const int prio_phase = (int)(wg / (nwg > 3 ? (nwg + 3) / 4 : 1));
#endif
    for (int seg = wg * (NK_WG / 64) + wave; seg < d.nseg; seg += nwaves) {
        const int64_t base = (int64_t)seg * d.segcap;
        const int nnew = d.R > 0 ? d.seg_new[seg] : 0;
        const int count = d.seg_count[seg] + nnew;
        if (lane == 0 && nnew > 0) atomicAdd(&L.bins.misc[0], (unsigned int)nnew);
        const NkSegModes sm = nk_seg_modes(d, seg);
        constexpr bool use_lrec = LREC;
        if (use_lrec) {
            for (int r0 = lane; r0 < sm.nl; r0 += 64) {
                const double4 *g = reinterpret_cast<const double4 *>(sm.rec + r0);
                const double4 a = g[0], b = g[1];
                double2 *q = lrec + r0 * NK_LREC_STRIDE;
                q[0] = make_double2(a.x, a.y); q[1] = make_double2(a.z, a.w); q[2] = make_double2(b.x, b.y); q[3] = make_double2(b.z, b.w);
                if (NK_LREC_STRIDE > 4 && (ROUGH || PID)) *reinterpret_cast<int *>(q + 4) = sm.mode(r0);
            }
            __builtin_amdgcn_fence(__ATOMIC_SEQ_CST, "wavefront");
        }
        auto mode_of = [&](int i) -> int {
            if (use_lrec && NK_LREC_STRIDE > 4) return *(const __attribute__((address_space(3))) int *)(const void *)(lrec + i * NK_LREC_STRIDE + 4);
            return sm.mode(i);
        };
        constexpr bool ALT = GEOM == 1 || SPLIT;
        const bool down = ALT && d.down != 0;
        const int lo = (ALT && d.seg_lo) ? d.seg_lo[seg] : 0, hi = lo + count;
        const int blo = lo & ~(NK_TILE - 1), bhi = count > 0 ? ((hi - 1) & ~(NK_TILE - 1)) : blo;
        const int nA = count > 0 ? (bhi - blo) / NK_TILE + 1 : 0;
        const int wlo = (!down && lo > (d.segcap - count) / 2) ? 0 : lo;
        NkOut<PID> O;
        O.init(L, wave);
        O.place(down ? base + hi - 1 : base + wlo, down ? -1 : 1, down ? count : d.segcap - wlo);
        int qn = SPLIT ? d.seg_evq[seg] : 0;
        if (SPLIT && lane == 0 && qn > 0) atomicAdd(&L.bins.misc[0], (unsigned int)qn);
        int cn = 0;
#ifdef NK_STAMPS
        unsigned long long st_acc[8] = {0, 0, 0, 0, 0, 0, 0, 0}, st_last;
        asm volatile("s_memtime %0\n\ts_waitcnt lgkmcnt(0)" : "=s"(st_last)::"memory");
        const unsigned long long st_c0 = st_last, st_r0 = __builtin_amdgcn_s_memrealtime();
#endif
        constexpr bool PF2 = NK_PREFETCH2 || SPLIT;
        constexpr bool DEFER = (NK_DEFER_STORE || PF2) && !NK_OUT_RING;
        struct NkTileBuf { uint32_t w0; double x, y, z, occ, nts; unsigned long long pid; };
        NkTileBuf bA = {0u, 0, 0, 0, 0, 0, 0ull}, bB = bA;
        auto fetch = [&](NkTileBuf &b, int r) {
            int rr = down ? bhi - r : blo + r;
            rr = rr < 0 ? 0 : (rr < d.segcap - NK_TILE ? rr : d.segcap - NK_TILE);
            const int64_t i0 = base + rr;
            if (PF2) {
                typedef NkBlock<!BOX, PID> B;
                const double *px = B::tile(d.x.p, i0, lane), *py = px + B::O_Y, *pz = px + B::O_Z, *po = px + B::O_OCC, *pn = px + B::O_NTS;
                const uint32_t *pw = B::word(d.x.p, i0) + lane;
                asm volatile("global_load_dword %0, %1, off" : "=v"(b.w0) : "v"(pw) : "memory");
                asm volatile("global_load_dwordx2 %0, %1, off" : "=v"(b.x) : "v"(px) : "memory");
                asm volatile("global_load_dwordx2 %0, %1, off" : "=v"(b.y) : "v"(py) : "memory");
                asm volatile("global_load_dwordx2 %0, %1, off" : "=v"(b.z) : "v"(pz) : "memory");
                asm volatile("global_load_dwordx2 %0, %1, off" : "=v"(b.occ) : "v"(po) : "memory");
                asm volatile("global_load_dwordx2 %0, %1, off" : "=v"(b.nts) : "v"(pn) : "memory");
                if (PID) { const double *pp = px + B::O_PID; asm volatile("global_load_dwordx2 %0, %1, off" : "=v"(b.pid) : "v"(pp) : "memory"); }
                return;
            }
            if (rr + lane >= lo && rr + lane < hi && r < nA * NK_TILE) {
                typedef NkBlock<!BOX, PID> B;
                const double *q = B::tile(d.x.p, i0, lane);
                b.w0 = NK_LD(B::word(d.x.p, i0) + lane); b.x = NK_LD(q); b.y = NK_LD(q + B::O_Y); b.z = NK_LD(q + B::O_Z); b.occ = NK_LD(q + B::O_OCC);
                if (!BOX) b.nts = NK_LD(q + B::O_NTS);
                if (PID) b.pid = NK_LD(reinterpret_cast<const unsigned long long *>(q + B::O_PID));
            }
        };
        auto arrived = [&](NkTileBuf &b) {
            if (!PF2) return;
            if (PID) asm volatile("s_waitcnt vmcnt(7)" : "+v"(b.w0), "+v"(b.x), "+v"(b.y), "+v"(b.z), "+v"(b.occ), "+v"(b.nts), "+v"(b.pid) : : "memory");
            else asm volatile("s_waitcnt vmcnt(6)" : "+v"(b.w0), "+v"(b.x), "+v"(b.y), "+v"(b.z), "+v"(b.occ), "+v"(b.nts) : : "memory");
        };
        auto drained = [&](NkTileBuf &b) {
            if (PF2) asm volatile("s_waitcnt vmcnt(0)" : "+v"(b.w0), "+v"(b.x), "+v"(b.y), "+v"(b.z), "+v"(b.occ), "+v"(b.nts), "+v"(b.pid) : : "memory");
        };
        fetch(bA, 0);
        if (PF2) fetch(bB, NK_TILE);
        bool sdone = false, sev = false;
        int so = 0, sq = 0;
        double sx = 0, sy = 0, sz = 0, socc = 0, snts = 0;
        uint32_t sw0 = 0u;
        unsigned long long spid = 0;
        auto turn = [&](NkTileBuf &buf, const int t) __attribute__((always_inline)) {
            const bool flush = t == nA;
            arrived(buf);
#if NK_PRIO_ROT
            if ((t & ((1 << NK_PRIO_ROT) - 1)) == 0) {
                switch (((t >> NK_PRIO_ROT) + prio_phase) & 3) {
                    case 0: __builtin_amdgcn_s_setprio(0); break;
                    case 1: __builtin_amdgcn_s_setprio(1); break;
                    case 2: __builtin_amdgcn_s_setprio(2); break;
                    default: __builtin_amdgcn_s_setprio(3); break;
                }
            }
#endif
            bool act = false;
            double x = 0, y = 0, z = 0, occ = 0, nts = 0, omega = 0, E0 = 0, vx = 0, vy = 0, vz = 0;
            uint32_t w0 = 0u;
            unsigned long long pid = 0;
            if (!flush) {
                const int r = t * NK_TILE;
                { const int rr = down ? bhi - r : blo + r; act = rr + lane >= lo && rr + lane < hi; }
                w0 = buf.w0; x = buf.x; y = buf.y; z = buf.z; occ = buf.occ; nts = buf.nts; pid = buf.pid;
            }
            if (DEFER) {
                asm volatile("" : "+v"(x), "+v"(y), "+v"(z), "+v"(occ), "+v"(nts), "+v"(w0));
                O.template store<BOX>(d, base, sdone, so, sx, sy, sz, socc, snts, sw0, spid);
                sdone = false;
                if (SPLIT && sev) {
                    if (sq < d.segcap) {
                        const int64_t i = base + sq;
                        d.qx[i] = sx; d.qy[i] = sy; d.qz[i] = sz; d.qocc[i] = socc; d.qnts[i] = snts; d.qw0[i] = sw0;
                        if (PID) d.qpid[i] = spid;
                    }
                }
                sev = false;
            }
            if (PF2) fetch(buf, (t + 2) * NK_TILE);
            if (!flush) {
                const int r = t * NK_TILE;
                if (!PF2) fetch(buf, r + NK_TILE);
                const bool newborn = (w0 & NK_NEWBORN) != 0u;
                w0 &= ~NK_NEWBORN;
                const int idx = act ? (int)(w0 & lbmask) : 0;
                double4 ra, rb;
                if (use_lrec) {
                    const NkLdsRec q = nk_lds_rec(lrec + idx * NK_LREC_STRIDE);
                    const nk_v2d q0 = q[0], q1 = q[1], q2 = q[2], q3 = q[3];
                    ra = make_double4(q0.x, q0.y, q1.x, q1.y); rb = make_double4(q2.x, q2.y, q3.x, q3.y);
                }
                else { const double4 *g = reinterpret_cast<const double4 *>(sm.rec + idx); ra = g[0]; rb = g[1]; }
                omega = ra.x; vx = ra.y; vy = ra.z; vz = ra.w; E0 = rb.x;
#ifdef NK_STAMPS
                { const double fence_ = x + omega; asm volatile("" ::"v"(fence_)); }
#endif
                NK_STAMP(0);
                if (act && !newborn) {
                    if (do_relax) occ = nk_relax<RBF>(d, L, tw, ra, rb, x, y, z, occ, sm, idx);
                    x += vx * d.dt; y += vy * d.dt; z += vz * d.dt;
                    if (!BOX) nts -= 1.0;
                }
#ifdef NK_STAMPS
                { const double fence_ = x + occ; asm volatile("" ::"v"(fence_)); }
#endif
                NK_STAMP(1);
            }
            const bool ev = BOX ? (act && (w0 & NK_LOST) == 0u && nk_box_out(bw, x, y, z, vx, vy, vz)) : (act && nts < 0.0);
            const bool done = act && !ev;
            const unsigned long long mD = __ballot(done), mE = __ballot(ev);
            if (done) nk_tally_one(d, L.tb, L.bins, x, y, z, occ, omega, E0, vx, vy, vz, do_flux, rep);
            if (DEFER) {
                so = O.reserve(nk_rank(mD), __popcll(mD));
                sdone = done; sx = x; sy = y; sz = z; socc = occ; snts = nts; sw0 = w0; spid = pid;
            } else O.template push<BOX>(d, base, lane, done, nk_rank(mD), __popcll(mD), x, y, z, occ, nts, w0, pid);
            NK_STAMP(2);
            if (SPLIT) {
                if (DEFER) { sev = ev; sq = qn + nk_rank(mE); }
                else if (ev) {
                    const int o = qn + nk_rank(mE);
                    if (o < d.segcap) {
                        const int64_t i = base + o;
                        d.qx[i] = x; d.qy[i] = y; d.qz[i] = z; d.qocc[i] = occ; d.qnts[i] = nts; d.qw0[i] = w0;
                        if (PID) d.qpid[i] = pid;
                    }
                }
                qn += __popcll(mE);
                return;
            }
            const int pn = __popcll(mE), erank = nk_rank(mE);
            int taken = 0;
            while (taken < pn || (flush && cn > 0)) {
                if (taken < pn) {
                    const int k = pn - taken < 64 - cn ? pn - taken : 64 - cn;
                    if (ev && erank >= taken && erank < taken + k) {
                        const int sl = cn + erank - taken;
                        cX[sl] = x; cX[64 + sl] = y; cX[128 + sl] = z; cX[192 + sl] = occ; cX[256 + sl] = nts; cX[320 + sl] = 0.0;
                        cW[sl] = w0; cW[64 + sl] = 0u;
                        if (PID) { cP[sl] = __longlong_as_double((long long)pid); cW[128 + sl] = (uint32_t)mode_of((int)(w0 & lbmask)); cW[192 + sl] = (w0 & lbmask) * (uint32_t)d.nseg + (uint32_t)seg; }
                    }
                    cn += k; taken += k;
                }
                if (cn < 64 && !(flush && taken == pn)) break;
                NK_STAMP(3);
                __builtin_amdgcn_fence(__ATOMIC_SEQ_CST, "wavefront");
                const bool eact = lane < cn;
                NkParticle p;
// ... 268 lines not shown
            const int st = nk_event_pre<ROUGH, RBF>(d, L.facets, L.tb, L.resT, L.bins, p, cts, evc, pid, step);
            if (st == NK_EV_DEAD) phase = NK_PH_NEED;
            else if (tree) { nk_walk_begin(d, W, p.x, p.y, p.z, p.vx, p.vy, p.vz); npend = 0; wdone = false; skipl = NK_TREE_NO_SKIP; phase = NK_PH_WALK; }
            else {
                nk_find_boundary(L.planes, L.faces, d.NP, d.tol, p.x, p.y, p.z, p.vx, p.vy, p.vz, W.h.t, W.h.facet);
                phase = NK_PH_POST;
            }
        }
        {
            const int low = more ? NK_EVENTS_LOW : 0;
#ifdef NK_STAMPS
            unsigned long long st_a, st_b;
            asm volatile("s_memtime %0\n\ts_waitcnt lgkmcnt(0)" : "=s"(st_a)::"memory");
#endif
            for (;;) {
                const bool walking = phase == NK_PH_WALK;
                const bool boxes = walking && !wdone && npend < NK_EVENTS_PEND;
                const unsigned long long mW = __ballot(walking), mB = __ballot(boxes), mL = __ballot(walking && npend > 0);
                const int nw = __popcll(mW), nb = __popcll(mB), nl = __popcll(mL);
                if (nw <= low) break;
                if (nb == 0 || nl >= NK_EVENTS_LEAVES || nw - nb >= NK_EVENTS_STUCK) {
#ifdef NK_STAMPS
                    unsigned long long st_c, st_d;
                    asm volatile("s_memtime %0\n\ts_waitcnt lgkmcnt(0)" : "=s"(st_c)::"memory");
#endif
                    if (walking && npend > 0) {
                        --npend;
                        W.leaf = pend[npend * NK_EV_WG + tid];
                        nk_walk_leaf(d, W, p.x, p.y, p.z, p.vx, p.vy, p.vz);
                        if (wdone && npend == 0) phase = NK_PH_POST;
                    }
#ifdef NK_STAMPS
                    asm volatile("s_waitcnt vmcnt(0)\n\ts_memtime %0\n\ts_waitcnt lgkmcnt(0)" : "=s"(st_d)::"memory");
                    st_leaf += st_d - st_c; st_nleaf += 1;
#endif
                } else {
                    bool over = false;
                    if (__ballot(boxes && skipl != NK_TREE_NO_SKIP) != 0ull) { if (boxes) over = nk_walk_boxes(d, skipl, W, tl, tl_fam0); }
                    else if (boxes) over = nk_walk_boxes(d, NK_TREE_NO_SKIP, W, tl, tl_fam0);
                    if (boxes) {
                        if (W.leaf >= 0) { pend[npend * NK_EV_WG + tid] = W.leaf; ++npend; W.leaf = -1; }
                        if (over) { wdone = true; if (npend == 0) phase = NK_PH_POST; }
                    }
                }
#ifdef NK_STAMPS
                st_pass += 1;
#endif
            }
#ifdef NK_STAMPS
            asm volatile("s_memtime %0\n\ts_waitcnt lgkmcnt(0)" : "=s"(st_b)::"memory");
            st_walk += st_b - st_a;
#endif
        }
        bool fin = false;
        if (phase == NK_PH_POST) {
            if (first) {
                first = false;
                double xa, ya, za, na;
                nk_newborn_place(d, p.x, p.y, p.z, p.vx, p.vy, p.vz, p.nts, W.h.t, xa, ya, za, na);
                p.x = xa; p.y = ya; p.z = za; p.nts = na;
                p.facet = W.h.facet;
                if (na < 0.0) phase = NK_PH_PRE; else { fin = true; phase = NK_PH_NEED; }
            } else {
                const int st = nk_event_post(d, p, cts, evc, W.h.t, W.h.facet);
                if (st == NK_EV_MORE) phase = NK_PH_PRE; else { fin = true; phase = NK_PH_NEED; }
            }
        }
        if (fin) {
            nk_tally_one(d, L.tb, L.bins, p.x, p.y, p.z, p.occ, p.omega, p.E0, p.vx, p.vy, p.vz, do_flux, rep);
            bool stay = true;
            uint32_t idxe = (uint32_t)idx0;
            int hseg = seg;
            if (ROUGH) {
                if (d.part) { const uint32_t hi = (uint32_t)p.slot / (uint32_t)d.nseg; hseg = (int)((uint32_t)p.slot - hi * (uint32_t)d.nseg); stay = hseg == seg; idxe = hi; }
                else idxe = (uint32_t)p.mode;
            }
            const uint32_t w0e = ((uint32_t)(p.facet + 1) << d.lb) | idxe;
            if (stay) {
                const int slo = d.seg_lo ? d.seg_lo[seg] : 0;
                const int o = atomicAdd(d.seg_count + seg, 1);
                if (slo + o < d.segcap) {
                    const int64_t i = (int64_t)seg * d.segcap + slo + o;
                    const NkSlot q = nk_slot(d, i);
                    d.x.p[q.od] = p.x; d.y.p[q.od] = p.y; d.z.p[q.od] = p.z; d.occ.p[q.od] = p.occ; d.nts.p[q.od] = p.nts; d.w0.p[q.ow] = w0e;
                    if (PID) d.pid.p[q.od] = pid;
                } else atomicOr(d.overflow, 4);
            } else {
                const int dst = hseg;
                const int at = atomicAdd(d.mig_n + dst, 1);
                if (at < d.mig_cap) {
                    double2 *r = d.mig_buf + ((int64_t)dst * d.mig_cap + at) * 4;
                    r[0] = make_double2(p.x, p.y); r[1] = make_double2(p.z, p.occ);
                    r[2] = make_double2(p.nts, __longlong_as_double((long long)pid));
                    r[3] = make_double2(__longlong_as_double((long long)w0e), 0.0);
                } else atomicOr(d.overflow, 32);
            }
        }
        if (!more && __ballot(phase != NK_PH_NEED) == 0ull) break;
    }
#ifdef NK_STAMPS
    if (lane == 0 && d.stamps) {
        unsigned long long t1;
        asm volatile("s_memtime %0\n\ts_waitcnt lgkmcnt(0)" : "=s"(t1)::"memory");
        const int wv = blockIdx.x * (blockDim.x >> 6) + (tid >> 6);
        if (wv < d.nseg) {
            unsigned long long *o = d.stamps + (int64_t)wv * 8;
            o[3] = t1 - st_t0; o[4] = st_walk; o[5] = (st_got << 32) | st_pass; o[6] = (st_nleaf << 40) | st_leaf;
        }
    }
#endif
    nk_lds_flush(d, L, row0 + blockIdx.x);
}

NK_KERNEL_LINKAGE __global__ __launch_bounds__(NK_WG) void k_anchor(NkDev d, int honor_halt) {
    if (!d.seg_lo || (honor_halt && d.halt[0])) return;
    const int lane = threadIdx.x & 63, wave = threadIdx.x >> 6;
    const int nwaves = gridDim.x * (NK_WG / 64);
    for (int seg = blockIdx.x * (NK_WG / 64) + wave; seg < d.nseg; seg += nwaves) {
        const int lo = d.seg_lo[seg];
        if (lo <= 0) continue;
        const int64_t base = (int64_t)seg * d.segcap;
        int n = d.seg_count[seg] + (d.R > 0 ? d.seg_new[seg] : 0);
        n = lo + n <= d.segcap ? n : d.segcap - lo;
        for (int j0 = 0; j0 < n; j0 += 64) {
            const bool on = j0 + lane < n;
            const NkSlot qs = nk_slot(d, base + lo + j0 + (on ? lane : 0)), qd = nk_slot(d, base + j0 + (on ? lane : 0));
            double vx = 0, vy = 0, vz = 0, vo = 0, vn = 0;
            uint32_t vw = 0u;
            uint64_t vp = 0;
            if (on) {
                vx = d.x.p[qs.od]; vy = d.y.p[qs.od]; vz = d.z.p[qs.od]; vo = d.occ.p[qs.od]; vw = d.w0.p[qs.ow];
                if (d.nts.p) vn = d.nts.p[qs.od];
                if (d.pid.p) vp = d.pid.p[qs.od];
            }
            asm volatile("s_waitcnt vmcnt(0)" ::: "memory");
            __builtin_amdgcn_fence(__ATOMIC_SEQ_CST, "wavefront");
            if (on) {
                d.x.p[qd.od] = vx; d.y.p[qd.od] = vy; d.z.p[qd.od] = vz; d.occ.p[qd.od] = vo; d.w0.p[qd.ow] = vw;
                if (d.nts.p) d.nts.p[qd.od] = vn;
                if (d.pid.p) d.pid.p[qd.od] = vp;
            }
            asm volatile("s_waitcnt vmcnt(0)" ::: "memory");
        }
        if (lane == 0) d.seg_lo[seg] = 0;
    }
}

NK_KERNEL_LINKAGE __global__ __launch_bounds__(NK_WG) void k_regrow(NkDev o, NkDev n) {
    for (int seg = blockIdx.x; seg < o.nseg; seg += gridDim.x) {
        const int cnt = o.seg_count[seg];
        const int64_t a = (int64_t)seg * o.segcap, b = (int64_t)seg * n.segcap;
        for (int i = threadIdx.x; i < cnt; i += blockDim.x) {
            n.x[b + i] = o.x[a + i]; n.y[b + i] = o.y[a + i]; n.z[b + i] = o.z[a + i];
            n.occ[b + i] = o.occ[a + i]; if (o.nts && n.nts) n.nts[b + i] = o.nts[a + i];
            n.w0[b + i] = o.w0[a + i];
            if (o.pid && n.pid) n.pid[b + i] = o.pid[a + i];
        }
        if (threadIdx.x == 0) n.seg_count[seg] = cnt;
    }
}

NK_KERNEL_LINKAGE __global__ __launch_bounds__(NK_WG) void k_deliver(NkDev d, int in_step) {
    const int lane = threadIdx.x & 63, wave = __builtin_amdgcn_readfirstlane(threadIdx.x >> 6);
    const int nwaves = gridDim.x * (NK_WG / 64);
    for (int seg = blockIdx.x * (NK_WG / 64) + wave; seg < d.nseg; seg += nwaves) {
        int n = d.mig_n[seg];
        if (n <= 0) continue;
        if (n > d.mig_cap) n = d.mig_cap;
        const int count = d.seg_count[seg];
        const int lo = d.seg_lo ? d.seg_lo[seg] : 0;
        if (lo + count + n > d.segcap) { if (lane == 0 && !in_step) { atomicOr(d.halt + 2, 1); atomicOr(d.halt, 1); } continue; }
        const int64_t base = (int64_t)seg * d.segcap + lo + count;
        for (int j = lane; j < n; j += 64) {
            const double2 *r = d.mig_buf + ((int64_t)seg * d.mig_cap + j) * 4;
            const double2 a = r[0], b = r[1], c = r[2], e = r[3];
            d.x[base + j] = a.x; d.y[base + j] = a.y; d.z[base + j] = b.x; d.occ[base + j] = b.y; if (d.nts) d.nts[base + j] = c.x;
            d.pid[base + j] = (uint64_t)__double_as_longlong(c.y);
            d.w0[base + j] = (uint32_t)__double_as_longlong(e.x);
        }
        if (lane == 0) {
            d.seg_count[seg] = count + n;
            d.mig_n[seg] = 0;
            const int bound = d.R > 0 ? d.seg_bound[seg] : 0;
            if ((int64_t)lo + count + n + 2 * (bound + 2 * n) + NK_TILE > (int64_t)d.segcap) atomicOr(d.halt + 1, 1);
            if (2 * n > d.mig_cap) atomicOr(d.halt + 3, 1);
        }
    }
}

__device__ __forceinline__ void nk_update_sv(const NkDev &d, double Eraw, double Ns, double Told, int t, double Ta, double Tb, double Tz,
                                             double Ea, double Ez, double &Tnew_out, double &E_out) {
    const int n = d.nE;
        double norm;
        if (d.norm_fixed) norm = d.active_modes / (d.particle_density * d.sv_volume[t]);
        else { norm = d.active_modes / Ns; if (isnan(norm)) norm = 0.0; }
        double E = Eraw * norm / d.QV;
        int it = (int)((Told - Ta) / (Tb - Ta));
        it = it < 0 ? 0 : (it > n - 1 ? n - 1 : it);
        int base = it - 1;
        base = base < 0 ? 0 : (base > n - 4 ? n - 4 : base);
        double wT[4], wE[4];
#pragma unroll
        for (int j = 0; j < 4; ++j) { const int q = n >= 4 ? base + j : 0; wT[j] = d.Tarr[q]; wE[j] = d.Earr[q]; }
        double ref;
        if (Told < Ta) ref = Ea;
        else if (Told > Tz) ref = Ez;
        else if (n >= 4 && wT[0] < Told && !(wT[3] < Told)) {
            const int c = (wT[1] < Told) + (wT[2] < Told);
            const double xlo = c == 0 ? wT[0] : (c == 1 ? wT[1] : wT[2]), xhi = c == 0 ? wT[1] : (c == 1 ? wT[2] : wT[3]);
            const double ylo = c == 0 ? wE[0] : (c == 1 ? wE[1] : wE[2]), yhi = c == 0 ? wE[1] : (c == 1 ? wE[2] : wE[3]);
            ref = (yhi - ylo) / (xhi - xlo) * (Told - xlo) + ylo;
        } else { int io; ref = nk_interp_lin_hint(d.Tarr, d.Earr, n, Told, it, io); }
        E += ref;
        double Tnew;
        if (E < Ea) Tnew = d.Tfill_lo;
        else if (E > Ez) Tnew = d.Tfill_hi;
        else if (n >= 4 && wE[0] < E && !(wE[3] < E)) {
            const int c = (wE[1] < E) + (wE[2] < E);
            const double xlo = c == 0 ? wE[0] : (c == 1 ? wE[1] : wE[2]), xhi = c == 0 ? wE[1] : (c == 1 ? wE[2] : wE[3]);
            const double ylo = c == 0 ? wT[0] : (c == 1 ? wT[1] : wT[2]), yhi = c == 0 ? wT[1] : (c == 1 ? wT[2] : wT[3]);
            Tnew = (yhi - ylo) / (xhi - xlo) * (E - xlo) + ylo;
        } else { int io; Tnew = nk_interp_lin_hint(d.Earr, d.Tarr, n, E, it, io); }
        Tnew_out = Tnew;
        E_out = E;
}
__device__ __forceinline__ void nk_update_body(const NkDev &d, const double *acc, double *hist_row, int do_flux) {
    const int tid = threadIdx.x, nth = blockDim.x;
    const int S = d.S, NB = d.NB, n = d.nE;
    const double Ta = d.Tarr[0], Tb = d.Tarr[1], Tz = d.Tarr[n - 1], Ea = d.Earr[0], Ez = d.Earr[n - 1];
    for (int t = tid; t < S; t += nth) {
        double Tnew, E;
        nk_update_sv(d, acc[t], acc[S + t], d.T_ref_local ? d.T_sv[t] : d.T_ref, t, Ta, Tb, Tz, Ea, Ez, Tnew, E);
        hist_row[NB + t] = Tnew;
        hist_row[NB + S + t] = E;
        d.T_sv[t] = Tnew;
    }
    for (int b = tid; b < NB; b += nth) hist_row[b] = acc[b];
    if (d.sv_interp == 3) {
        __syncthreads();
        const int P = d.rbf_P;
        for (int j = tid; j < P; j += nth) {
            double a = 0.0;
            for (int i = 0; i < S; ++i) a += d.rbf_inv[(int64_t)j * P + i] * d.T_sv[i];
            d.T_sv[S + j] = a;
        }
    }
    if (d.res_gen == 2) for (int r = tid; r < d.R; r += nth) d.nleave_prev[r] = (int32_t)acc[5 * S + r];
    if (tid == 0) {
        hist_row[NB + 2 * S + 0] = (double)do_flux;
        hist_row[NB + 2 * S + 1] = 1.0;
        const bool hdel = acc[NB + 1] > 0.0;
        const bool hreq = acc[NB] > 0.0 || hdel;
        hist_row[NB + 2 * S + 2] = hreq ? 1.0 : 0.0;
        hist_row[NB + 2 * S + 3] = (double)*d.overflow;
        if (hreq) d.halt[0] = 1;
        if (hdel) d.halt[2] = 1;
        hist_row[NB + 2 * S + 4] = hreq ? 1.0 : 0.0;
        hist_row[NB + 2 * S + 5] = (double)d.halt[1];
        hist_row[NB + 2 * S + 6] = (hdel || d.halt[2]) ? 1.0 : 0.0;
        hist_row[NB + 2 * S + 7] = (double)d.halt[3];
    }
// ... 136 lines not shown
            for (int k = wg; k < ntask; k += G) {
                const int c0 = k < S ? k : 2 * S + (k - S), c1 = k < S ? S + k : -1;
                double v0 = 0.0, v1 = 0.0;
                for (int g = tid; g < G; g += NK_WG) {
                    v0 += __longlong_as_double((long long)__hip_atomic_load(rows_s + (size_t)g * NBP + c0, __ATOMIC_RELAXED, __HIP_MEMORY_SCOPE_AGENT));
                    if (c1 >= 0) v1 += __longlong_as_double((long long)__hip_atomic_load(rows_s + (size_t)g * NBP + c1, __ATOMIC_RELAXED, __HIP_MEMORY_SCOPE_AGENT));
                }
                double *red = L.colsum;
                red[tid] = v0; red[NK_WG + tid] = v1;
                __syncthreads();
                for (int o = NK_WG / 2; o > 0; o >>= 1) {
                    if (tid < o) { red[tid] += red[tid + o]; red[NK_WG + tid] += red[NK_WG + tid + o]; }
                    __syncthreads();
                }
                if (tid == 0) {
                    const double t0 = red[0], t1 = red[NK_WG];
                    if (k < S) {
                        double Tnew, E;
                        nk_update_sv(d, t0, t1, d.T_ref_local ? Tsv[k] : d.T_ref, k, Ta, Tb, Tz, Ea, Ez, Tnew, E);
                        __hip_atomic_store(Tpub + k, (unsigned long long)__double_as_longlong(Tnew), __ATOMIC_RELAXED, __HIP_MEMORY_SCOPE_AGENT);
                        if (k == 0 && hreq) { d.halt[0] = 1; __hip_atomic_store(bar + 1, 1u, __ATOMIC_RELAXED, __HIP_MEMORY_SCOPE_AGENT); }
                        asm volatile("s_waitcnt vmcnt(0) lgkmcnt(0)" ::: "memory");
                        __hip_atomic_store(flagsT + k, (unsigned int)(s + 1), __ATOMIC_RELAXED, __HIP_MEMORY_SCOPE_AGENT);
                        hrowp[k] = t0; hrowp[S + k] = t1; hrowp[NB + k] = Tnew; hrowp[NB + S + k] = E;
                        if (k == 0) {
                            hrowp[NB + 2 * S + 0] = (double)do_flux;
                            hrowp[NB + 2 * S + 1] = 1.0;
                            hrowp[NB + 2 * S + 2] = hreq ? 1.0 : 0.0;
                            hrowp[NB + 2 * S + 3] = (double)__hip_atomic_load(d.overflow, __ATOMIC_RELAXED, __HIP_MEMORY_SCOPE_AGENT);
                            hrowp[NB + 2 * S + 4] = hreq ? 1.0 : 0.0;
                            hrowp[NB + 2 * S + 5] = (double)hreq;
                            hrowp[NB + 2 * S + 6] = (double)d.halt[2];
                            hrowp[NB + 2 * S + 7] = (double)d.halt[3];
                        }
                    } else hrowp[c0] = t0;
                }
                __syncthreads();
            }
            if (mark) mk[5] = __builtin_amdgcn_s_memrealtime();
        }
        for (int t = tid; t < S; t += NK_WG) {
            if (!nk_wait_word(flagsT + t, (unsigned int)(s + 1))) ok = 0;
            else Tsv[t] = __longlong_as_double((long long)__hip_atomic_load(Tpub + t, __ATOMIC_RELAXED, __HIP_MEMORY_SCOPE_AGENT));
        }
        ok = __syncthreads_and(ok);
        if (!ok) { if (tid == 0) atomicOr(d.overflow, 256); return; }
        if (wg != 0) hreq = (int)__hip_atomic_load(bar + 1, __ATOMIC_RELAXED, __HIP_MEMORY_SCOPE_AGENT);
        hreq = __syncthreads_or(hreq);
        if (mark) mk[wg == 0 ? 6 : 3] = __builtin_amdgcn_s_memrealtime();
        __builtin_amdgcn_s_dcache_inv();
        __syncthreads();
        for (int t = tid; t < S; t += NK_WG) {
            const int jn = t + 1 < S ? t + 1 : t;
            NkSv q;
            q.c = L.tb.cen[3 * t + a]; q.T = Tsv[t];
            q.slope = jn > t ? (Tsv[jn] - Tsv[t]) / (L.tb.cen[3 * jn + a] - L.tb.cen[3 * t + a]) : 0.0;
            q.invT = 1.0 / Tsv[t];
            sv[t] = q;
        }
        __syncthreads();
        if (hreq) return;
    }
}

NK_KERNEL_LINKAGE __global__ __launch_bounds__(NK_WG) void k_update(NkDev d, const double *acc, double *hist_row, int do_flux) {
    if (d.halt[0]) return;
    nk_update_body(d, acc, hist_row, do_flux);
}

NK_KERNEL_LINKAGE __global__ __launch_bounds__(NK_WG) void k_relax(NkDev d, int honor_halt) {
    extern __shared__ __align__(16) unsigned char smem[];
    if (honor_halt && d.halt[0]) return;
    NkLds L;
    nk_lds_setup<0, 0>(d, smem, L);
    const uint32_t lbmask = (1u << d.lb) - 1u;
    NkTauWin tw;
    tw.load(d, false);
    for (int seg = blockIdx.x; seg < d.nseg; seg += gridDim.x) {
        const int64_t base = (int64_t)seg * d.segcap;
        const int count = d.seg_count[seg];
        const NkSegModes sm = nk_seg_modes(d, seg);
        for (int k = threadIdx.x; k < count; k += NK_WG) {
            const int64_t i = base + k;
            const int idx = (int)(d.w0[i] & lbmask);
            const double4 *mrec = reinterpret_cast<const double4 *>(sm.rec + idx);
            const double4 ra = mrec[0], rb = mrec[1];
            d.occ[i] = nk_relax(d, L, tw, ra, rb, d.x[i], d.y[i], d.z[i], d.occ[i], sm, idx);
        }
    }
}

template <int GEOM>
__global__ __launch_bounds__(NK_WG) void k_init_boundaries(NkDev d, int32_t *anomalies) {
    extern __shared__ __align__(16) unsigned char smem[];
    NkLds L;
    nk_lds_setup<GEOM, 0>(d, smem, L);
    const uint32_t lbmask = (1u << d.lb) - 1u;
    for (int seg = blockIdx.x; seg < d.nseg; seg += gridDim.x) {
        const int64_t base = (int64_t)seg * d.segcap;
        const int count = d.seg_count[seg];
        const NkSegModes sm = nk_seg_modes(d, seg);
        for (int k = threadIdx.x; k < count; k += NK_WG) {
            const int64_t i = base + k;
            const uint32_t idx = d.w0[i] & lbmask;
            const NkMode *rec = sm.rec + idx;
            double tc; int fc;
            const double x = d.x[i], y = d.y[i], z = d.z[i];
            NK_RAY(GEOM, d, L, NK_TREE_NO_SKIP, x, y, z, rec->vx, rec->vy, rec->vz, tc, fc);
            if (d.box) {
                const bool inside = x >= d.box_k[0] && x <= -d.box_k[1] && y >= d.box_k[2] && y <= -d.box_k[3] && z >= d.box_k[4] && z <= -d.box_k[5];
                if (!inside && fc >= 0) atomicAdd(anomalies, 1);
                d.w0[i] = (fc < 0 ? NK_LOST : 0u) | idx;
            } else {
                d.nts[i] = tc / d.dt;
                d.w0[i] = ((uint32_t)(fc + 1) << d.lb) | idx;
            }
        }
    }
}
template <int GEOM>
__global__ __launch_bounds__(NK_WG) void k_next_hit(NkDev d, double *nts_out, int32_t *facet_out) {
    extern __shared__ __align__(16) unsigned char smem[];
    NkLds L;
    nk_lds_setup<GEOM, 0>(d, smem, L);
    const uint32_t lbmask = (1u << d.lb) - 1u;
    for (int seg = blockIdx.x; seg < d.nseg; seg += gridDim.x) {
        const int64_t base = (int64_t)seg * d.segcap;
        const int count = d.seg_count[seg];
        const NkSegModes sm = nk_seg_modes(d, seg);
        for (int k = threadIdx.x; k < count; k += NK_WG) {
            const int64_t i = base + k;
            const uint32_t w0 = d.w0[i];
            if (w0 & NK_LOST) { nts_out[i] = __builtin_inf(); facet_out[i] = -1; continue; }
            const NkMode *rec = sm.rec + (w0 & lbmask);
            double x = d.x[i], y = d.y[i], z = d.z[i];
            const double vx = rec->vx, vy = rec->vy, vz = rec->vz;
            double tin = 0.0;
            if (vx > 0.0 && x < d.box_k[0]) tin = fmax(tin, (d.box_k[0] - x) / vx);
            if (vx < 0.0 && x > -d.box_k[1]) tin = fmax(tin, (-d.box_k[1] - x) / vx);
            if (vy > 0.0 && y < d.box_k[2]) tin = fmax(tin, (d.box_k[2] - y) / vy);
            if (vy < 0.0 && y > -d.box_k[3]) tin = fmax(tin, (-d.box_k[3] - y) / vy);
            if (vz > 0.0 && z < d.box_k[4]) tin = fmax(tin, (d.box_k[4] - z) / vz);
            if (vz < 0.0 && z > -d.box_k[5]) tin = fmax(tin, (-d.box_k[5] - z) / vz);
            if (tin > 0.0) { x += vx * tin; y += vy * tin; z += vz * tin; }
            double tc; int fc;
            NK_RAY(GEOM, d, L, NK_TREE_NO_SKIP, x, y, z, vx, vy, vz, tc, fc);
            nts_out[i] = (tc + tin) / d.dt;
            facet_out[i] = fc;
        }
    }
}

__device__ __forceinline__ uint64_t nk_state_key(int mode, double x, double y, double z) {
    uint64_t k = (uint64_t)(uint32_t)mode;
    k = k * 0x9E3779B97F4A7C15ull + (uint64_t)__double_as_longlong(x);
    k = k * 0x9E3779B97F4A7C15ull + (uint64_t)__double_as_longlong(y);
    k = k * 0x9E3779B97F4A7C15ull + (uint64_t)__double_as_longlong(z);
    return k;
}

#define NK_XMAX 24
NK_KERNEL_LINKAGE __global__ __launch_bounds__(NK_WG) void k_mesh_crossings(int64_t n, const double *orig, const double *dir, int64_t F, const double *v0,
                                                          const double *e1, const double *e2, int skip_self, int32_t *counts) {
#pragma clang fp contract(off)
    __shared__ double tile[NK_WG * 9];
    const int64_t r = (int64_t)blockIdx.x * NK_WG + threadIdx.x;
    const bool act = r < n;
    double ox = 0, oy = 0, oz = 0, dx = 0, dy = 0, dz = 1;
    if (act) { ox = orig[3 * r]; oy = orig[3 * r + 1]; oz = orig[3 * r + 2]; dx = dir[3 * r]; dy = dir[3 * r + 1]; dz = dir[3 * r + 2]; }
    double seen[NK_XMAX];
    int ns = 0;
    bool over = false;
    const double eps = 1e-9;
    for (int64_t f0 = 0; f0 < F; f0 += NK_WG) {
        __syncthreads();
        const int64_t tf = f0 + threadIdx.x;
        if (tf < F)
            for (int c = 0; c < 3; ++c) { tile[9 * threadIdx.x + c] = v0[3 * tf + c]; tile[9 * threadIdx.x + 3 + c] = e1[3 * tf + c]; tile[9 * threadIdx.x + 6 + c] = e2[3 * tf + c]; }
        __syncthreads();
        const int nt = F - f0 < NK_WG ? (int)(F - f0) : NK_WG;
        if (!act) continue;
        for (int i = 0; i < nt; ++i) {
            const double *q = tile + 9 * i;
            const double e1x = q[3], e1y = q[4], e1z = q[5], e2x = q[6], e2y = q[7], e2z = q[8];
            const double px = dy * e2z - dz * e2y, py = dz * e2x - dx * e2z, pz = dx * e2y - dy * e2x;
            const double det = e1x * px + e1y * py + e1z * pz;
            const double tx = ox - q[0], ty = oy - q[1], tz = oz - q[2];
            const double inv = 1.0 / det;
            const double u = (tx * px + ty * py + tz * pz) * inv;
            const double qx = ty * e1z - tz * e1y, qy = tz * e1x - tx * e1z, qz = tx * e1y - ty * e1x;
            const double w = (dx * qx + dy * qy + dz * qz) * inv;
            const double t = (e2x * qx + e2y * qy + e2z * qz) * inv;
            const bool ok = (fabs(det) > 1e-14) && (u >= -eps) && (w >= -eps) && (u + w <= 1 + eps) && (t > 1e-9);
            if (!ok || (skip_self && f0 + i == r)) continue;
            const double tr = rint(t * 1e8) / 1e8;
            bool dup = false;
            for (int k = 0; k < ns; ++k) dup |= seen[k] == tr;
            if (dup) continue;
            if (ns < NK_XMAX) seen[ns++] = tr; else over = true;
        }
    }
    if (act) counts[r] = over ? -1 : ns;
}

NK_KERNEL_LINKAGE __global__ __launch_bounds__(NK_WG) void k_init_particles(NkDev d, int64_t n, uint64_t pid_lo, const int32_t *umodes, int32_t nu,
                                                          const int64_t *sv_first) {
    extern __shared__ __align__(16) unsigned char smem[];
    NkLds L;
    nk_lds_setup<0, 0>(d, smem, L);
    const int64_t stride = (int64_t)gridDim.x * blockDim.x;
    for (int64_t i = (int64_t)blockIdx.x * blockDim.x + threadIdx.x; i < n; i += stride) {
        const uint64_t pid = pid_lo + (uint64_t)i;
        const int mode = umodes[pid % (uint64_t)nu];
        int seg, idx;
        nk_mode_home(d, mode, seg, idx);
        int want = -1;
        if (sv_first) { int lo = 0, hi = d.S; while (hi - lo > 1) { const int mid = (lo + hi) >> 1; if (sv_first[mid] <= (int64_t)pid) lo = mid; else hi = mid; } want = lo; }
        double x = 0.0, y = 0.0, z = 0.0;
        int s = 0;
        for (uint32_t t = 0; t < 4096u; ++t) {
            double u[6];
            nk_uniform2_dev(d.seed, pid, 0u, NK_TAG_INIT + 3u * t + 0u, u[0], u[1]);
            nk_uniform2_dev(d.seed, pid, 0u, NK_TAG_INIT + 3u * t + 1u, u[2], u[3]);
            nk_uniform2_dev(d.seed, pid, 0u, NK_TAG_INIT + 3u * t + 2u, u[4], u[5]);
            int sx = nk_ss_right(d.simplex_cdf, d.nS, u[0]);
            sx = sx > d.nS - 1 ? d.nS - 1 : sx;
            double a[4], asum = 0.0;
            for (int q = 0; q < 4; ++q) { a[q] = -log(u[1 + q]); asum += a[q]; }
            const double *sp = d.simplex_pts + 12 * (int64_t)sx;
            x = y = z = 0.0;
            for (int q = 0; q < 4; ++q) { const double wq = a[q] / asum; x += wq * sp[3 * q]; y += wq * sp[3 * q + 1]; z += wq * sp[3 * q + 2]; }
            s = nk_classify(d, L.tb, x, y, z);
            if (want < 0 || s == want) break;
            if (t == 4095u) atomicOr(d.overflow, 64);
        }
        const NkMode *rec = d.modetab + mode;
        const double occ = nk_occupation(d, L.tb.Tsv[s], rec->omega, rec->E0);
        const int slot = atomicAdd(d.seg_count + seg, 1);
        if (slot < d.segcap) {
            const int64_t o = (int64_t)seg * d.segcap + slot;
            d.x[o] = x; d.y[o] = y; d.z[o] = z; d.occ[o] = occ; if (d.nts) d.nts[o] = 0.0; d.w0[o] = (uint32_t)idx;
            if (d.pid) d.pid[o] = pid;
        } else atomicOr(d.overflow, 2);
    }
}
NK_KERNEL_LINKAGE __global__ __launch_bounds__(NK_WG) void k_tally_state(NkDev d) {
    extern __shared__ __align__(16) unsigned char smem[];
    NkLds L;
    nk_lds_setup<0, 0>(d, smem, L);
    const uint32_t lbmask = (1u << d.lb) - 1u;
    const int rep = threadIdx.x & (NK_NREP - 1);
    for (int seg = blockIdx.x; seg < d.nseg; seg += gridDim.x) {
        const int64_t base = (int64_t)seg * d.segcap;
        const int count = d.seg_count[seg];
        const NkSegModes sm = nk_seg_modes(d, seg);
        for (int k = threadIdx.x; k < count; k += NK_WG) {
            const int64_t i = base + k;
            const NkMode *rec = sm.rec + (d.w0[i] & lbmask);
            nk_tally_one(d, L.tb, L.bins, d.x[i], d.y[i], d.z[i], d.occ[i], rec->omega, rec->E0, rec->vx, rec->vy, rec->vz, true, rep);
        }
    }
    nk_lds_flush(d, L, blockIdx.x);
}

#define NK_SPEC_WG 1024
template <bool STATE>
__global__ __launch_bounds__(NK_SPEC_WG) void k_spectral(NkDev d, const int32_t *band_of_mode, int b0, int Bt, int lds0, double *slabs) {
    extern __shared__ __align__(16) unsigned char smem[];
    if (!STATE && d.halt[0]) return;
    NkLds L;
    nk_lds_setup<0, 0>(d, smem, L);
    const int nb = d.S * Bt;
    double *bF = (double *)(smem + lds0);
    unsigned int *bN = (unsigned int *)(bF + 3 * nb);
    for (int i = threadIdx.x; i < 3 * nb; i += blockDim.x) bF[i] = 0.0;
    for (int i = threadIdx.x; i < nb; i += blockDim.x) bN[i] = 0u;
    __syncthreads();
    const uint32_t lbmask = (1u << d.lb) - 1u;
    for (int seg = blockIdx.x; seg < d.nseg; seg += gridDim.x) {
        const int64_t base = (int64_t)seg * d.segcap + (d.seg_lo ? d.seg_lo[seg] : 0);
        const int count = d.seg_count[seg];
        const NkSegModes sm = nk_seg_modes(d, seg);
        for (int k = threadIdx.x; k < count; k += blockDim.x) {
            const int64_t i = base + k;
            const int idx = (int)(d.w0[i] & lbmask);
            const int b = band_of_mode[sm.mode(idx)] - b0;
            if ((unsigned)b >= (unsigned)Bt) continue;
            const NkMode *rec = sm.rec + idx;
            const double x = d.x[i], y = d.y[i], z = d.z[i];
            const int s = nk_classify(d, L.tb, x, y, z);
            double e;
            if (STATE) {
                double invT;
                const double T = nk_interp_T(d, L.tb, x, y, z, invT);
                const double n0 = !d.T_ref_local ? nk_occupation(d, d.T_ref, rec->omega, rec->E0)
                                                 : (T > 0.0 ? nk_be(rec->omega * d.c_hk, rec->E0, invT, d.invT0) : 0.0);
                e = d.hbar * rec->omega * (d.occ[i] - n0);
            } else {
                e = nk_tally_e(d, L.tb, s, d.occ[i], rec->omega, rec->E0);
            }
            const int q = s * Bt + b;
            atomicAdd(bF + 3 * q + 0, rec->vx * e);
            atomicAdd(bF + 3 * q + 1, rec->vy * e);
            atomicAdd(bF + 3 * q + 2, rec->vz * e);
            atomicAdd(bN + q, 1u);
        }
    }
    __syncthreads();
    double *out = slabs + (int64_t)blockIdx.x * 4 * nb;
    for (int c = threadIdx.x; c < 3 * nb; c += blockDim.x) out[c] = bF[c];
    for (int c = threadIdx.x; c < nb; c += blockDim.x) out[3 * nb + c] = (double)bN[c];
}
NK_KERNEL_LINKAGE __global__ __launch_bounds__(256) void k_spectral_reduce(const int32_t *halt, const double *slabs, int G, int S, int B,
                                                                           int b0, int Bt, double *row) {
    if (halt && halt[0]) return;
    const int nb = S * Bt, lane = threadIdx.x & 63;
    const int c = blockIdx.x * 4 + (threadIdx.x >> 6);
    if (c >= 4 * nb) return;
    double v = 0.0;
    for (int g = lane; g < G; g += 64) v += slabs[(int64_t)g * 4 * nb + c];
    for (int o = 32; o > 0; o >>= 1) v += __shfl_down(v, o, 64);
    if (lane == 0) {
        int64_t o;
        if (c < 3 * nb) {
            const int q = c / 3, k = c - 3 * q, s = q / Bt, bl = q - s * Bt;
            o = ((int64_t)s * B + b0 + bl) * 3 + k;
        } else {
            const int q = c - 3 * nb, s = q / Bt, bl = q - s * Bt;
            o = 3 * (int64_t)S * B + (int64_t)s * B + b0 + bl;
        }
        row[o] = v;
    }
}

struct NkFieldDev {
    double lo[3], inv_h[3];
    int32_t n[3], ncells;
    double sE, sF;
    double BE, BF;
    unsigned long long *grid;
    int32_t lds_bins, lds0;
};
#define NK_FIELD_WG 1024
__device__ __forceinline__ int nk_field_axis(double x, double lo, double inv_h, int n, bool &clamped) {
    const double f = floor((x - lo) * inv_h);
    if (!(f >= 0.0)) { clamped = true; return 0; }
    if (f >= (double)n) { clamped = true; return n - 1; }
    return (int)f;
}
template <bool STATE>
__global__ __launch_bounds__(NK_FIELD_WG) void k_field(NkDev d, NkFieldDev f) {
    extern __shared__ __align__(16) unsigned char smem[];
    if (!STATE && d.halt[0]) return;
    NkLds L;
    nk_lds_setup<0, 0>(d, smem, L);
    const int nc = f.ncells;
    unsigned long long *bR = (unsigned long long *)(smem + f.lds0);
    unsigned int *bN = (unsigned int *)(bR + 4 * (size_t)nc);
    if (f.lds_bins) {
        for (int i = threadIdx.x; i < 4 * nc; i += blockDim.x) bR[i] = 0ull;
        for (int i = threadIdx.x; i < nc; i += blockDim.x) bN[i] = 0u;
        __syncthreads();
    }
    unsigned long long *hdr = f.grid + (size_t)nc * 8;
    unsigned int n_clamped = 0, n_ovE = 0, n_ovF = 0, stuck = 0;
    const uint32_t lbmask = (1u << d.lb) - 1u;
    for (int seg = blockIdx.x; seg < d.nseg; seg += gridDim.x) {
        const int64_t base = (int64_t)seg * d.segcap + (d.seg_lo ? d.seg_lo[seg] : 0);
        const int count = d.seg_count[seg];
        if (!STATE && d.mig_buf && threadIdx.x == 0 && d.mig_n[seg] > 0) stuck = 1;
        const NkSegModes sm = nk_seg_modes(d, seg);
        for (int k = threadIdx.x; k < count; k += blockDim.x) {
            const int64_t i = base + k;
            const int idx = (int)(d.w0[i] & lbmask);
            const NkMode *rec = sm.rec + idx;
            const double x = d.x[i], y = d.y[i], z = d.z[i];
            double e;
            if (STATE) {
                double invT;
                const double T = nk_interp_T(d, L.tb, x, y, z, invT);
                const double n0 = !d.T_ref_local ? nk_occupation(d, d.T_ref, rec->omega, rec->E0)
                                                 : (T > 0.0 ? nk_be(rec->omega * d.c_hk, rec->E0, invT, d.invT0) : 0.0);
                e = d.hbar * rec->omega * (d.occ[i] - n0);
            } else {
                const int s = nk_classify(d, L.tb, x, y, z);
                e = nk_tally_e(d, L.tb, s, d.occ[i], rec->omega, rec->E0);
            }
            bool cl = false;
            const int ix = nk_field_axis(x, f.lo[0], f.inv_h[0], f.n[0], cl);
            const int iy = nk_field_axis(y, f.lo[1], f.inv_h[1], f.n[1], cl);
            const int iz = nk_field_axis(z, f.lo[2], f.inv_h[2], f.n[2], cl);
            n_clamped += cl ? 1u : 0u;
            const int c = (ix * f.n[1] + iy) * f.n[2] + iz;
            const double fx = rec->vx * e, fy = rec->vy * e, fz = rec->vz * e;
            const bool okE = fabs(e) <= f.BE;
            const bool okF = fabs(fx) <= f.BF && fabs(fy) <= f.BF && fabs(fz) <= f.BF;
            n_ovE += okE ? 0u : 1u;
            n_ovF += okF ? 0u : 1u;
            const unsigned long long qE = okE ? (unsigned long long)(long long)rint(e * f.sE) : 0ull;
            const unsigned long long qx = okF ? (unsigned long long)(long long)rint(fx * f.sF) : 0ull;
            const unsigned long long qy = okF ? (unsigned long long)(long long)rint(fy * f.sF) : 0ull;
            const unsigned long long qz = okF ? (unsigned long long)(long long)rint(fz * f.sF) : 0ull;
            if (f.lds_bins) {
                atomicAdd(bN + c, 1u);
                atomicAdd(bR + 4 * c + 0, qE);
                atomicAdd(bR + 4 * c + 1, qx);
                atomicAdd(bR + 4 * c + 2, qy);
                atomicAdd(bR + 4 * c + 3, qz);
            } else {
                unsigned long long *g = f.grid + (size_t)c * 8;
                atomicAdd(g + 0, 1ull);
                atomicAdd(g + 1, qE);
                atomicAdd(g + 2, qx);
                atomicAdd(g + 3, qy);
                atomicAdd(g + 4, qz);
            }
        }
    }
    if (n_clamped) atomicAdd(hdr + 0, (unsigned long long)n_clamped);
    if (n_ovE) atomicAdd(hdr + 1, (unsigned long long)n_ovE);
    if (n_ovF) atomicAdd(hdr + 2, (unsigned long long)n_ovF);
    if (stuck) atomicAdd(hdr + 4, 1ull);
    if (blockIdx.x == 0 && threadIdx.x == 0) atomicAdd(hdr + 3, 1ull);
    if (f.lds_bins) {
        __syncthreads();
        for (int c = threadIdx.x; c < nc; c += blockDim.x) {
            const unsigned int n = bN[c];
            if (n == 0u) continue;
            unsigned long long *g = f.grid + (size_t)c * 8;
            atomicAdd(g + 0, (unsigned long long)n);
#pragma unroll
            for (int k = 0; k < 4; ++k) { const unsigned long long v = bR[4 * c + k]; if (v) atomicAdd(g + 1 + k, v); }
        }
    }
}
template <int NK_TU = 0>
__global__ __launch_bounds__(256) void k_field_accum(NkFieldDev f, double *acc, int nranks) {
    const int c = blockIdx.x * blockDim.x + threadIdx.x;
    if (c >= f.ncells) return;
    const unsigned long long *hdr = f.grid + (size_t)f.ncells * 8;
    const bool take = hdr[3] == (unsigned long long)nranks && hdr[4] == 0ull;
    unsigned long long *g = f.grid + (size_t)c * 8;
    if (take) {
        const double iE = 1.0 / f.sE, iF = 1.0 / f.sF;
        double *a = acc + (size_t)c * 5;
        a[0] += (double)(long long)g[0];
        a[1] += (double)(long long)g[1] * iE;
        a[2] += (double)(long long)g[2] * iF;
        a[3] += (double)(long long)g[3] * iF;
        a[4] += (double)(long long)g[4] * iF;
    }
#pragma unroll
    for (int k = 0; k < 5; ++k) g[k] = 0ull;
}
template <int NK_TU = 0>
__global__ void k_field_finish(NkFieldDev f, long long *status, int nranks) {
    unsigned long long *hdr = f.grid + (size_t)f.ncells * 8;
    const bool take = hdr[3] == (unsigned long long)nranks && hdr[4] == 0ull;
    if (take) { status[0] += 1; status[1] += (long long)hdr[0]; }
    status[2] += (long long)hdr[1];
    status[3] += (long long)hdr[2];
    for (int k = 0; k < 8; ++k) hdr[k] = 0ull;
}

struct NkModesDev {
    double sE, BE;
    unsigned long long *tE;
    unsigned int *tN;
    unsigned long long *hdr;
    int32_t owner, lds0, slice;
    int32_t nteam;
};
#define NK_MODES_WG 1024
template <bool STATE>
__global__ __launch_bounds__(NK_MODES_WG) void k_modes(NkDev d, NkModesDev m) {
    extern __shared__ __align__(16) unsigned char smem[];
    if (!STATE && d.halt[0]) return;
    NkLds L;
    nk_lds_setup<0, 0>(d, smem, L);
    const int S = d.S, nteam = m.nteam, tsize = NK_MODES_WG / nteam;
    const int team = threadIdx.x / tsize, tl = threadIdx.x - team * tsize;
    unsigned long long *bE = (unsigned long long *)(smem + m.lds0 + (size_t)team * m.slice);
    unsigned int *bN = (unsigned int *)(bE + (size_t)d.nlmax * S);
    if (m.owner) {
        for (int b = tl; b < d.nlmax * S; b += tsize) { bE[b] = 0ull; bN[b] = 0u; }
        __syncthreads();
    }
    unsigned int n_ovE = 0, stuck = 0;
    const uint32_t lbmask = (1u << d.lb) - 1u;
    const int ngroups = (d.nseg + nteam - 1) / nteam;
    for (int grp = blockIdx.x; grp < ngroups; grp += gridDim.x) {
        const int seg = grp * nteam + team;
        const bool live = seg < d.nseg;
        const int64_t base = live ? (int64_t)seg * d.segcap + (d.seg_lo ? d.seg_lo[seg] : 0) : 0;
        const int count = live ? d.seg_count[seg] : 0;
        if (!STATE && live && d.mig_buf && tl == 0 && d.mig_n[seg] > 0) stuck = 1;
        const NkSegModes sm = nk_seg_modes(d, live ? seg : 0);
        const int nb = (m.owner && live) ? sm.nl * S : 0;
        for (int k = tl; k < count; k += tsize) {
            const int64_t i = base + k;
            const int idx = (int)(d.w0[i] & lbmask);
            const NkMode *rec = sm.rec + idx;
            const double x = d.x[i], y = d.y[i], z = d.z[i];
            const int s = nk_classify(d, L.tb, x, y, z);
            double e;
            if (STATE) {
                double invT;
                const double T = nk_interp_T(d, L.tb, x, y, z, invT);
                const double n0 = !d.T_ref_local ? nk_occupation(d, d.T_ref, rec->omega, rec->E0)
                                                 : (T > 0.0 ? nk_be(rec->omega * d.c_hk, rec->E0, invT, d.invT0) : 0.0);
                e = d.hbar * rec->omega * (d.occ[i] - n0);
            } else {
                e = nk_tally_e(d, L.tb, s, d.occ[i], rec->omega, rec->E0);
            }
            const bool okE = fabs(e) <= m.BE;
            n_ovE += okE ? 0u : 1u;
            const unsigned long long qE = okE ? (unsigned long long)(long long)rint(e * m.sE) : 0ull;
            if (m.owner) {
                const int b = (idx < sm.nl ? idx : 0) * S + s;
                atomicAdd(bN + b, 1u);
                atomicAdd(bE + b, qE);
            } else {
                const int gmode = sm.mode(idx);
                if ((unsigned)gmode >= (unsigned)d.M) continue;
                const int64_t b = (int64_t)gmode * S + s;
                atomicAdd(m.tN + b, 1u);
                atomicAdd(m.tE + b, qE);
            }
        }
        if (m.owner) {
            __syncthreads();
            for (int b = tl; b < nb; b += tsize) {
                const int l = b / S, gmode = sm.mode(l);
                const unsigned long long vE = bE[b];
                const unsigned int vN = bN[b];
                bE[b] = 0ull; bN[b] = 0u;
                if ((unsigned)gmode >= (unsigned)d.M) continue;
                const int64_t o = (int64_t)gmode * S + (b - l * S);
                m.tE[o] = vE;
                m.tN[o] = vN;
            }
            __syncthreads();
        }
    }
    if (n_ovE) atomicAdd(m.hdr + 0, (unsigned long long)n_ovE);
    if (stuck) atomicAdd(m.hdr + 2, 1ull);
    if (blockIdx.x == 0 && threadIdx.x == 0) atomicAdd(m.hdr + 1, 1ull);
}
template <int NK_TU = 0>
__global__ __launch_bounds__(256) void k_modes_accum(NkModesDev m, double *accE, double *accN, int64_t n, int nranks) {
    const bool take = m.hdr[1] == (unsigned long long)nranks && m.hdr[2] == 0ull;
    if (!take) return;
    const double iE = 1.0 / m.sE;
    const int64_t stride = (int64_t)gridDim.x * blockDim.x;
    for (int64_t b = (int64_t)blockIdx.x * blockDim.x + threadIdx.x; b < n; b += stride) {
        accE[b] += (double)(long long)m.tE[b] * iE;
        accN[b] += (double)m.tN[b];
    }
}
template <int NK_TU = 0>
__global__ void k_modes_finish(NkModesDev m, long long *status, int nranks) {
    const bool take = m.hdr[1] == (unsigned long long)nranks && m.hdr[2] == 0ull;
    if (take) status[0] += 1;
    else if (m.hdr[1] == (unsigned long long)nranks) status[1] += 1;
    status[2] += (long long)m.hdr[0];
    for (int k = 0; k < 8; ++k) m.hdr[k] = 0ull;
}

template <int GEOM>
__global__ __launch_bounds__(NK_WG) void k_contains(NkDev d, uint32_t step) {
    extern __shared__ __align__(16) unsigned char smem[];
    if (d.halt[0]) return;
    NkLds L;
    nk_lds_setup<GEOM, 0>(d, smem, L);
    const uint32_t lbmask = (1u << d.lb) - 1u;
    for (int seg = blockIdx.x; seg < d.nseg; seg += gridDim.x) {
        const int64_t base = (int64_t)seg * d.segcap;
        const int count = d.seg_count[seg];
        const NkSegModes sm = nk_seg_modes(d, seg);
        for (int k = threadIdx.x; k < count; k += NK_WG) {
            const int64_t i = base + k;
            double x = d.x[i], y = d.y[i], z = d.z[i];
            bool out = x < d.bbox[0] - 1e-10 || y < d.bbox[1] - 1e-10 || z < d.bbox[2] - 1e-10 || x > d.bbox[3] + 1e-10 ||
                       y > d.bbox[4] + 1e-10 || z > d.bbox[5] + 1e-10;
            if (!out) continue;
            const uint32_t idx = d.w0[i] & lbmask;
            const uint64_t pid = d.pid ? d.pid[i] : nk_state_key(sm.mode((int)idx), x, y, z);
            double u[6];
            nk_uniform2_dev(d.seed, pid, step, NK_TAG_RESAMP + 0, u[0], u[1]);
            nk_uniform2_dev(d.seed, pid, step, NK_TAG_RESAMP + 1, u[2], u[3]);
            nk_uniform2_dev(d.seed, pid, step, NK_TAG_RESAMP + 2, u[4], u[5]);
            int s = nk_ss_right(d.simplex_cdf, d.nS, u[0]);
            s = s > d.nS - 1 ? d.nS - 1 : s;
            double a[4], asum = 0.0;
            for (int q = 0; q < 4; ++q) { a[q] = -log(u[1 + q]); asum += a[q]; }
            const double *sp = d.simplex_pts + 12 * (int64_t)s;
            x = y = z = 0.0;
            for (int q = 0; q < 4; ++q) { double wq = a[q] / asum; x += wq * sp[3 * q]; y += wq * sp[3 * q + 1]; z += wq * sp[3 * q + 2]; }
            const NkMode *rec = sm.rec + idx;
            double tc; int fc;
            NK_RAY(GEOM, d, L, NK_TREE_NO_SKIP, x, y, z, rec->vx, rec->vy, rec->vz, tc, fc);
            d.x[i] = x; d.y[i] = y; d.z[i] = z;
            if (d.box) d.w0[i] = (fc < 0 ? NK_LOST : 0u) | idx;
            else { d.nts[i] = tc / d.dt; d.w0[i] = ((uint32_t)(fc + 1) << d.lb) | idx; }
        }
    }
}

NK_KERNEL_LINKAGE __global__ void k_perm_rm(int to_seg_order, int R, int M, int nseg, int nlmax, const int32_t *m2s, double *canon, double *perm) {
    const int64_t i = (int64_t)blockIdx.x * blockDim.x + threadIdx.x;
    if (i >= (int64_t)R * M) return;
    const int r = (int)(i / M), m = (int)(i - (int64_t)r * M);
    const int slot = m2s[m];
    const int64_t at = ((int64_t)(slot % nseg) * R + r) * nlmax + slot / nseg;
    if (to_seg_order) perm[at] = canon[i]; else canon[i] = perm[at];
}

NK_KERNEL_LINKAGE __global__ void k_build_modetab(const double *omega, const double *vg, const double *tau, int M, int NT, int row0, double c_hk,
                                double invT0, int nseg, int nlmax, const int32_t *m2s, NkMode *out, NkMode *out_p) {
    int m = blockIdx.x * blockDim.x + threadIdx.x;
    if (m >= M) return;
    NkMode r;
    r.omega = omega[m]; r.vx = vg[3 * m]; r.vy = vg[3 * m + 1]; r.vz = vg[3 * m + 2];
    r.E0 = exp(r.omega * c_hk * invT0);
    for (int k = 0; k < NK_TAU_ROWS; ++k) {
        int row = row0 + k;
        r.tau[k] = (row >= 0 && row < NT) ? tau[(int64_t)row * M + m] : 0.0;
    }
    out[m] = r;
    if (out_p) { const int slot = m2s[m]; out_p[(int64_t)(slot % nseg) * nlmax + slot / nseg] = r; }
}

template <int GEOM>
__global__ __launch_bounds__(NK_WG) void k_tap_find_boundary(NkDev d, int64_t n, const double *x, const double *v,
                                                             double *xc, double *tc, int32_t *fc) {
    extern __shared__ __align__(16) unsigned char smem[];
    NkLds L;
    nk_lds_setup<GEOM, 0>(d, smem, L);
    int64_t i = (int64_t)blockIdx.x * NK_WG + threadIdx.x;
    if (i >= n) return;
    double t; int f;
    NK_RAY(GEOM, d, L, NK_TREE_NO_SKIP, x[3 * i], x[3 * i + 1], x[3 * i + 2], v[3 * i], v[3 * i + 1], v[3 * i + 2], t, f);
    tc[i] = t; fc[i] = f;
    for (int k = 0; k < 3; ++k) xc[3 * i + k] = x[3 * i + k] + t * v[3 * i + k];
}
NK_KERNEL_LINKAGE __global__ __launch_bounds__(NK_WG) void k_tap_classify(NkDev d, int64_t n, const double *x, int32_t *id) {
    extern __shared__ __align__(16) unsigned char smem[];
    NkLds L;
    nk_lds_setup<0, 0>(d, smem, L);
    int64_t i = (int64_t)blockIdx.x * NK_WG + threadIdx.x;
    if (i < n) id[i] = nk_classify(d, L.tb, x[3 * i], x[3 * i + 1], x[3 * i + 2]);
}
NK_KERNEL_LINKAGE __global__ __launch_bounds__(NK_WG) void k_tap_eval(NkDev d, int what, int64_t n, const double *a, const int32_t *mode,
                                                    double *out) {
    extern __shared__ __align__(16) unsigned char smem[];
    NkLds L;
    nk_lds_setup<0, 0>(d, smem, L);
    int64_t i = (int64_t)blockIdx.x * NK_WG + threadIdx.x;
    if (i >= n) return;
    switch (what) {
        case 0: out[i] = nk_occupation(d, a[i], d.modetab[mode[i]].omega, d.modetab[mode[i]].E0); break;
        case 1: { const NkMode *rec = d.modetab + mode[i]; NkTauWin tw; tw.load(d, false); out[i] = nk_lifetime(d, tw, rec->tau[0], rec->tau[1], rec->tau[2], a[i], NkPlainModes(), mode[i]); break; }
        case 2: out[i] = nk_T_of_E(d, a[i]); break;
        case 3: out[i] = nk_E_of_T(d, a[i]); break;
        case 5: out[i] = nk_exp(a[i]); break;
        default: { double invT; out[i] = nk_interp_T(d, L.tb, a[3 * i], a[3 * i + 1], a[3 * i + 2], invT); break; }
    }
}
NK_KERNEL_LINKAGE __global__ __launch_bounds__(NK_WG) void k_tap_reflect(NkDev d, int64_t n, const int32_t *facet, const int32_t *mode_in,
                                                       const double *col, const double *n_in, const double *om_in,
                                                       const double *r_spec, const double *r_deg, const double *r_diff,
                                                       int32_t *mode_out, double *n_out, double *om_out) {
    extern __shared__ __align__(16) unsigned char smem[];
    NkLds L;
    nk_lds_setup<0, 0>(d, smem, L);
    int64_t i = (int64_t)blockIdx.x * NK_WG + threadIdx.x;
    if (i >= n) return;
    int mo; double no, oo, eo;
    nk_reflect(d, L.tb, d.facets[facet[i]].rough, mode_in[i], col[3 * i], col[3 * i + 1], col[3 * i + 2],
               n_in[i], om_in[i], d.modetab[mode_in[i]].E0, r_spec[i], r_deg ? r_deg[i] : 0.0, r_diff[i], mo, no, oo, eo);
    mode_out[i] = mo; n_out[i] = no; om_out[i] = oo;
}
NK_KERNEL_LINKAGE __global__ __launch_bounds__(NK_WG) void k_cal_stream(NkDev d) {
    for (int seg = blockIdx.x; seg < d.nseg; seg += gridDim.x) {
        const int64_t base = (int64_t)seg * d.segcap;
        const int count = d.seg_count[seg];
        for (int k = threadIdx.x; k < count; k += NK_WG) {
            const int64_t i = base + k;
            uint32_t w0 = d.w0[i];
            double x = d.x[i], y = d.y[i], z = d.z[i], occ = d.occ[i], nts = d.nts ? d.nts[i] : 0.0;
            asm volatile("" : "+v"(w0), "+v"(occ));
            d.x[i] = x; d.y[i] = y; d.z[i] = z; if (d.nts) d.nts[i] = nts;
        }
    }
}
template <int W>
__global__ __launch_bounds__(NK_WG, 3) void k_probe_copy(NkDev d) {
    const bool hn = (bool)d.nts;
    const int lane = threadIdx.x & 63, wave = __builtin_amdgcn_readfirstlane(threadIdx.x >> 6);
    const int nwaves = gridDim.x * (NK_WG / 64);
    for (int seg = blockIdx.x * (NK_WG / 64) + wave; seg < d.nseg; seg += nwaves) {
        const int64_t base = (int64_t)seg * d.segcap;
        const int count = d.seg_count[seg] & ~63;
        double xN = 0, yN = 0, zN = 0, oN = 0, nN = 0; uint32_t wN = 0;
        if (count > 0) { const int64_t i0 = base; xN = *d.x.tile(i0, lane); yN = *d.y.tile(i0, lane); zN = *d.z.tile(i0, lane); oN = *d.occ.tile(i0, lane); if (hn) nN = *d.nts.tile(i0, lane); wN = *d.w0.tile(i0, lane); }
        for (int r = 0; r < count; r += 64) {
            const double x = xN, y = yN, z = zN, o = oN, n = nN; const uint32_t w = wN;
            if (r + 64 < count) { const int64_t i0 = base + r + 64; xN = *d.x.tile(i0, lane); yN = *d.y.tile(i0, lane); zN = *d.z.tile(i0, lane); oN = *d.occ.tile(i0, lane); if (hn) nN = *d.nts.tile(i0, lane); wN = *d.w0.tile(i0, lane); }
            const int64_t i0 = base + r;
            *d.x.tile(i0, lane) = x + 1e-300; *d.y.tile(i0, lane) = y; *d.z.tile(i0, lane) = z; *d.occ.tile(i0, lane) = o; if (hn) *d.nts.tile(i0, lane) = n; *d.w0.tile(i0, lane) = w;
        }
    }
}
NK_KERNEL_LINKAGE __global__ __launch_bounds__(NK_WG, 3) void k_probe_place(NkDev d, int tiles) {
    const bool hn = (bool)d.nts;
    const int lane = threadIdx.x & 63, wave = __builtin_amdgcn_readfirstlane(threadIdx.x >> 6);
    const int nwaves = gridDim.x * (NK_WG / 64);
    for (int seg = blockIdx.x * (NK_WG / 64) + wave; seg < d.nseg; seg += nwaves) {
        const int64_t base = (int64_t)seg * d.segcap;
        const int64_t step = 64;
        const int count = tiles;
        double xN = 0, yN = 0, zN = 0, oN = 0, nN = 0; uint32_t wN = 0;
        if (count > 0) { const int64_t i0 = base; xN = *d.x.tile(i0, lane); yN = *d.y.tile(i0, lane); zN = *d.z.tile(i0, lane); oN = *d.occ.tile(i0, lane); if (hn) nN = *d.nts.tile(i0, lane); wN = *d.w0.tile(i0, lane); }
        for (int r = 0; r < count; ++r) {
            double x = xN, y = yN, z = zN, o = oN, n = nN; uint32_t w = wN;
            if (r + 1 < count) { const int64_t i0 = base + (r + 1) * step; xN = *d.x.tile(i0, lane); yN = *d.y.tile(i0, lane); zN = *d.z.tile(i0, lane); oN = *d.occ.tile(i0, lane); if (hn) nN = *d.nts.tile(i0, lane); wN = *d.w0.tile(i0, lane); }
            asm volatile("" : "+v"(x), "+v"(y), "+v"(z), "+v"(o), "+v"(n), "+v"(w));
            const int64_t i0 = base + r * step;
            *d.x.tile(i0, lane) = x; *d.y.tile(i0, lane) = y; *d.z.tile(i0, lane) = z; *d.occ.tile(i0, lane) = o; if (hn) *d.nts.tile(i0, lane) = n; *d.w0.tile(i0, lane) = w;
        }
    }
}
NK_KERNEL_LINKAGE __global__ void k_tap_uniform(uint64_t seed, uint64_t pid, uint32_t step, uint32_t tag, double *out) {
    double a, b;
    nk_uniform2_dev(seed, pid, step, tag, a, b);
    out[0] = a; out[1] = b;
}


struct NkSpecMode { double vx, vy, vz, nrm, om, dl, vdn, pad; };
NK_KERNEL_LINKAGE __global__ __launch_bounds__(NK_WG) void k_specular_prepare(int M, const double *v, const double *omega, const double *delta,
                                                            const int32_t *rank, double nx, double ny, double nz, NkSpecMode *out) {
#pragma clang fp contract(off)
    const int m = blockIdx.x * NK_WG + threadIdx.x;
    if (m >= M) return;
    NkSpecMode r;
    r.vx = v[3 * m]; r.vy = v[3 * m + 1]; r.vz = v[3 * m + 2];
    r.vdn = (r.vx * nx + r.vy * ny) + r.vz * nz;
    r.nrm = sqrt((r.vx * r.vx + r.vy * r.vy) + r.vz * r.vz);
    r.om = omega[m]; r.dl = delta[m]; r.pad = (double)m;
    out[rank[m]] = r;
}
NK_KERNEL_LINKAGE __global__ __launch_bounds__(NK_WG) void k_specular_pairs(int M, const NkSpecMode *modes, const double *sorted_vx, double vmax,
                                                          double nx, double ny, double nz, double crit, int64_t cap,
                                                          int32_t *pin, int32_t *pout, unsigned long long *count) {
#pragma clang fp contract(off)
    const int a = blockIdx.x * NK_WG + threadIdx.x;
    if (a >= M) return;
    const NkSpecMode me = modes[a];
    if (!(me.vdn < 0.0)) return;
    const double t2x = 2.0 * nx, t2y = 2.0 * ny, t2z = 2.0 * nz;
    const double rx = me.vx - t2x * me.vdn, ry = me.vy - t2y * me.vdn, rz = me.vz - t2z * me.vdn;
    const double nrm_in = sqrt((rx * rx + ry * ry) + rz * rz);
    const double vn = sqrt((me.vx * me.vx + me.vy * me.vy) + me.vz * me.vz);
    const double ux = me.vx / vn, uy = me.vy / vn, uz = me.vz / vn;
    const double udn = (ux * nx + uy * ny) + uz * nz;
    const double tx = ux - t2x * udn, ty = uy - t2y * udn, tz = uz - t2z * udn;
    const double h = crit * fmax(vmax, nrm_in) * (1.0 + 1e-6);
    int lo = 0, hi = M;
    { int l = 0, r = M; const double key = rx - h; while (l < r) { const int mid = (l + r) >> 1; if (sorted_vx[mid] < key) l = mid + 1; else r = mid; } lo = l; }
    { int l = lo, r = M; const double key = rx + h; while (l < r) { const int mid = (l + r) >> 1; if (sorted_vx[mid] <= key) l = mid + 1; else r = mid; } hi = l; }
    const int a_orig = (int)me.pad;
    for (int k = lo; k < hi; ++k) {
        const NkSpecMode o = modes[k];
        if (!(o.vdn > 0.0)) continue;
        const double ref = fmax(nrm_in, o.nrm);
        if (!(fabs(rx - o.vx) / ref < crit)) continue;
        if (!(fabs(ry - o.vy) / ref < crit) || !(fabs(rz - o.vz) / ref < crit)) continue;
        if (!(fabs(me.om - o.om) < me.dl + o.dl)) continue;
        const double ox = o.vx / o.nrm, oy = o.vy / o.nrm, oz = o.vz / o.nrm;
        const double dot = (tx * ox + ty * oy) + tz * oz;
        const double ang = acos(dot);
        if (!(ang < crit)) continue;
        const unsigned long long at = atomicAdd(count, 1ull);
        if ((int64_t)at < cap) { pin[at] = a_orig; pout[at] = (int)o.pad; }
    }
}

__device__ __forceinline__ double nk_spec0(const double *v, const double *k2, int J, int m, double nx, double ny, double nz, double eta,
                                           double &vdn) {
    const double vx = v[3 * m], vy = v[3 * m + 1], vz = v[3 * m + 2];
    vdn = nx * vx + ny * vy + nz * vz;
    const double vn = sqrt(vx * vx + vy * vy + vz * vz);
    const double c = vdn / vn, e = 2.0 * eta * c;
    const double sp = exp(-(e * e) * k2[m / J]);
    return isnan(sp) ? 0.0 : sp;
}
NK_KERNEL_LINKAGE __global__ __launch_bounds__(NK_WG) void k_rough_pairs(int M, int J, const double *v, const double *k2, int64_t npairs, const int32_t *pin,
                                                      const int32_t *pout, int nf, const int32_t *fidx, const double *nin,
                                                      const double *eta, uint8_t *true_spec, unsigned int *spec_map, double *sub) {
    const int64_t p = (int64_t)blockIdx.x * NK_WG + threadIdx.x;
    if (p >= npairs) return;
    const int a = pin[p], b = pout[p];
    for (int k = 0; k < nf; ++k) {
        const int f = fidx[k];
        double vdn;
        const double sp = nk_spec0(v, k2, J, a, nin[3 * f], nin[3 * f + 1], nin[3 * f + 2], eta[f], vdn);
        true_spec[(int64_t)f * M + a] = 1;
        atomicMin(spec_map + (int64_t)f * M + a, (unsigned int)b);
        atomicAdd(sub + (int64_t)f * M + b, (vdn < 0.0 ? -vdn : 0.0) * sp);
    }
}
// ... 134 lines not shown
```

Baseline: 53.83 billion.

## Pack particle state word into 16 bits for box-mesh store

When the box fast path is used and no next-time-to-surface field is stored, the per-particle packed word (flags plus mode index) shrinks from 32 to 16 bits. The block layout is resized to match, and every reader and writer goes through a widen/narrow accessor, with host upload and download converting as well. The aim is to cut the bytes streamed per particle in the memory-bound sweep, from 36 to 34 in this configuration. In exchange it limits the mode-index width: box mode is now refused for large mode counts. The inline-asm dword prefetch path also reads a 16-bit slot with a 32-bit load, which may pick up a neighbour's bits if that path is enabled.

```diff
diff --git a/nanokappa_amd/csrc/nk_device.h b/nanokappa_amd/csrc/nk_device.h
--- a/nanokappa_amd/csrc/nk_device.h
+++ b/nanokappa_amd/csrc/nk_device.h
@@ -34,14 +34,53 @@
     __host__ __device__ __forceinline__ explicit operator bool() const { return p != nullptr; }
 };
 
+#define NK_BOX_WORD_BITS 16
+#ifndef NK_BOX_WORD_AREA
+#define NK_BOX_WORD_AREA (64 * (NK_BOX_WORD_BITS / 8) / 8)
+#endif
+__host__ __device__ constexpr int nk_word_bytes(bool w16) { return w16 ? NK_BOX_WORD_BITS / 8 : 4; }
+__host__ __device__ constexpr int nk_word_doubles(bool w16) { return w16 ? NK_BOX_WORD_AREA : 64 * 4 / 8; }
+__host__ __device__ __forceinline__ uint32_t nk_word_widen(uint32_t s) { return (s | (s << 16)) & 0xC0003FFFu; }
+__host__ __device__ __forceinline__ uint16_t nk_word_narrow(uint32_t w) { return (uint16_t)(w | (w >> 16)); }
+template <bool W16> struct NkWordOf { typedef uint32_t type; };
+template <> struct NkWordOf<true> { typedef uint16_t type; };
+struct NkWords {
+    void *p;
+    int32_t blk;
+    int32_t w16;
+    __host__ __device__ __forceinline__ int64_t off(int64_t i) const { return (i >> 6) * (int64_t)blk + (i & 63); }
+    __device__ __forceinline__ uint32_t get_at(int64_t o) const {
+        return w16 ? nk_word_widen(static_cast<const uint16_t *>(p)[o]) : static_cast<const uint32_t *>(p)[o];
+    }
+    __device__ __forceinline__ void put_at(int64_t o, uint32_t w) const {
+        if (w16) static_cast<uint16_t *>(p)[o] = nk_word_narrow(w);
+        else static_cast<uint32_t *>(p)[o] = w;
+    }
+    __device__ __forceinline__ uint32_t get(int64_t i) const { return get_at(off(i)); }
+    __device__ __forceinline__ void put(int64_t i, uint32_t w) const { put_at(off(i), w); }
+    __device__ __forceinline__ uint32_t raw_at(int64_t o) const { return w16 ? static_cast<const uint16_t *>(p)[o] : static_cast<const uint32_t *>(p)[o]; }
+    __device__ __forceinline__ void put_raw_at(int64_t o, uint32_t r) const {
+        if (w16) static_cast<uint16_t *>(p)[o] = (uint16_t)r;
+        else static_cast<uint32_t *>(p)[o] = r;
+    }
+    template <bool W16>
+    __device__ __forceinline__ void put_at_as(int64_t o, uint32_t w) const {
+        if (W16) static_cast<uint16_t *>(p)[o] = nk_word_narrow(w);
+        else static_cast<uint32_t *>(p)[o] = w;
+    }
+};
+
 template <bool NTS, bool PID>
 struct NkBlock {
+    typedef typename NkWordOf<!NTS>::type Word;
     static constexpr int NF = 4 + (NTS ? 1 : 0) + (PID ? 1 : 0);
-    static constexpr int BD = NF * 64 + 32;
+    static constexpr int BD = NF * 64 + nk_word_doubles(!NTS);
     static constexpr int O_Y = 64, O_Z = 128, O_OCC = 192, O_NTS = 256, O_PID = 64 * (NTS ? 5 : 4), O_W0 = 64 * NF;
     static __device__ __forceinline__ double *slot(double *s0, int64_t i) { return s0 + (i >> 6) * (int64_t)BD + (i & 63); }
     static __device__ __forceinline__ double *tile(double *s0, int64_t i0, int lane) { return s0 + (i0 >> 6) * (int64_t)BD + lane; }
-    static __device__ __forceinline__ uint32_t *word(double *s0, int64_t i) { return reinterpret_cast<uint32_t *>(s0 + (i >> 6) * (int64_t)BD + O_W0) + (i & 63); }
+    static __device__ __forceinline__ Word *word(double *s0, int64_t i) { return reinterpret_cast<Word *>(s0 + (i >> 6) * (int64_t)BD + O_W0) + (i & 63); }
+    static __device__ __forceinline__ uint32_t widen(uint32_t s) { return NTS ? s : nk_word_widen(s); }
+    static __device__ __forceinline__ Word narrow(uint32_t w) { return NTS ? (Word)w : (Word)nk_word_narrow(w); }
 };
 
 struct __attribute__((aligned(16))) NkFacet {
@@ -153,7 +192,7 @@
     int32_t down;
     int32_t *seg_bound;
     NkField<double> x, y, z, occ, nts;
-    NkField<uint32_t> w0;
+    NkWords w0;
     NkField<uint64_t> pid;
     int32_t part;
     int32_t lb;
diff --git a/nanokappa_amd/csrc/nk_engine.hip b/nanokappa_amd/csrc/nk_engine.hip
--- a/nanokappa_amd/csrc/nk_engine.hip
+++ b/nanokappa_amd/csrc/nk_engine.hip
@@ -165,31 +165,31 @@
     do { int rc_ = nk_upload(ctx, src, n, dst); if (rc_) return rc_; } while (0)
 
 static inline bool nk_layout_soa() { return false; }
-static inline int nk_particle_bytes(bool with_pid, bool with_nts) { return 36 + (with_nts ? 8 : 0) + (with_pid ? 8 : 0); }
+static inline int nk_store_fields(bool with_pid, bool with_nts) { return 4 + (with_nts ? 1 : 0) + (with_pid ? 1 : 0); }
+static inline int nk_block_doubles(bool with_pid, bool with_nts) { return nk_store_fields(with_pid, with_nts) * 64 + nk_word_doubles(!with_nts); }
+static inline int nk_particle_bytes(bool with_pid, bool with_nts) { return nk_store_fields(with_pid, with_nts) * 8 + nk_word_bytes(!with_nts); }
 static inline size_t nk_store_bytes(int64_t cap, bool with_pid, bool with_nts) {
     const int64_t nblk = (cap + 63) / 64;
-    const int nf = 4 + (with_nts ? 1 : 0) + (with_pid ? 1 : 0);
-    const int bd = nf * 64 + 32;
-    const size_t bytes = nk_layout_soa() ? (size_t)nblk * 64 * (nf * 8 + 4) : (size_t)nblk * bd * 8;
+    const size_t bytes = nk_layout_soa() ? (size_t)nblk * 64 * nk_particle_bytes(with_pid, with_nts) : (size_t)nblk * nk_block_doubles(with_pid, with_nts) * 8;
     return bytes ? bytes : 64;
 }
 static void nk_point_fields(NkDev &d, double *b, int64_t cap, bool with_pid, bool with_nts) {
     const int64_t nblk = (cap + 63) / 64;
-    const int nf = 4 + (with_nts ? 1 : 0) + (with_pid ? 1 : 0);
-    const int bd = nf * 64 + 32;
+    const int bd = nk_block_doubles(with_pid, with_nts);
+    const int w16 = with_nts ? 0 : 1, wpd = 8 / nk_word_bytes(!with_nts);
     if (nk_layout_soa()) {
         const int64_t n = nblk * 64;
         int k = 4;
         d.x = {b, 64}; d.y = {b + n, 64}; d.z = {b + 2 * n, 64}; d.occ = {b + 3 * n, 64};
         d.nts = {with_nts ? b + (k++) * n : nullptr, 64};
         d.pid = {with_pid ? (uint64_t *)(b + (k++) * n) : nullptr, 64};
-        d.w0 = {(uint32_t *)(b + k * n), 64};
+        d.w0 = {(void *)(b + k * n), 64, w16};
     } else {
         int k = 4;
         d.x = {b, bd}; d.y = {b + 64, bd}; d.z = {b + 128, bd}; d.occ = {b + 192, bd};
         d.nts = {with_nts ? b + 64 * (k++) : nullptr, bd};
         d.pid = {with_pid ? (uint64_t *)(b + 64 * (k++)) : nullptr, bd};
-        d.w0 = {(uint32_t *)(b + 64 * k), 2 * bd};
+        d.w0 = {(void *)(b + 64 * k), wpd * bd, w16};
     }
 }
 static int nk_alloc_fields(nk_ctx *ctx, NkDev &d, int64_t cap, bool with_pid, bool with_nts) {
@@ -834,7 +834,9 @@
     return NK_OK;
 }
 
+static inline bool nk_want_part(const nk_ctx *ctx);
 static inline bool nk_want_box(const nk_ctx *ctx) {
+    if (!nk_want_part(ctx) && ctx->d.M > (1 << (NK_BOX_WORD_BITS - 2))) return false;
     return ctx->have_mesh && ctx->mesh_box && !ctx->box_forbidden && !getenv("NK_NO_BOX") && !getenv("NK_SPLIT") && !nk_layout_soa() &&
            ctx->d.F <= NK_LDS_FACES && ctx->d.Fc <= NK_LDS_FACES;
 }
@@ -1135,7 +1137,13 @@
             keep(bd, h.nts.data());
         } else { std::fill(h.nts.begin(), h.nts.end(), 0.0); }
     }
-    if ((rc = nk_field_download(ctx, d, d.w0, bw))) return rc; keep(bw, w0.data());
+    if (d.w0.w16) {
+        std::vector<uint16_t> bh;
+        if ((rc = nk_field_download(ctx, d, NkField<uint16_t>{(uint16_t *)d.w0.p, d.w0.blk}, bh))) return rc;
+        bw.resize(bh.size());
+        for (size_t q = 0; q < bh.size(); ++q) bw[q] = nk_word_widen(bh[q]);
+    } else if ((rc = nk_field_download(ctx, d, NkField<uint32_t>{(uint32_t *)d.w0.p, d.w0.blk}, bw))) return rc;
+    keep(bw, w0.data());
     if (d.pid) { if ((rc = nk_field_download(ctx, d, d.pid, bu))) return rc; keep(bu, h.pid.data()); }
     const uint32_t lbmask = (1u << d.lb) - 1u;
     int64_t k = 0;
@@ -1198,7 +1206,11 @@
             const uint32_t idx = d.part ? (uint32_t)(ctx->h_m2s[(size_t)mode[i]] / d.nseg) : (uint32_t)mode[i];
             w0[(size_t)i] = d.nts ? (((uint32_t)(fc + 1) << d.lb) | idx) : (((facet && fc < 0) ? NK_LOST : 0u) | idx);
         }
-        if ((rc = put((const uint32_t *)w0.data(), d.w0))) return rc;
+        if (d.w0.w16) {
+            std::vector<uint16_t> wh((size_t)N);
+            for (int64_t i = 0; i < N; ++i) wh[(size_t)i] = nk_word_narrow(w0[(size_t)i]);
+            if ((rc = put((const uint16_t *)wh.data(), NkField<uint16_t>{(uint16_t *)d.w0.p, d.w0.blk}))) return rc;
+        } else if ((rc = put((const uint32_t *)w0.data(), NkField<uint32_t>{(uint32_t *)d.w0.p, d.w0.blk}))) return rc;
     }
     if (d.pid) {
         if (pid) { if ((rc = put(pid, d.pid))) return rc; }
@@ -1467,6 +1479,7 @@
         int lb = 1;
         while ((1ll << lb) <= maxidx) ++lb;
         NK_ARG(lb < 30 && (int64_t)d.Fc + 1 < (1ll << (31 - lb)), "mesh has too many facets for the packed particle word (facets x modes)");
+        NK_ARG(!d.box || lb + 2 <= NK_BOX_WORD_BITS, "mode index too wide for the box store's 16-bit packed word");
         d.lb = lb;
     }
     int64_t segcap = (capacity + nseg - 1) / nseg;
@@ -3499,13 +3512,13 @@
                 float ms = 0.f;
                 hipEventElapsedTime(&ms, e0, e1);
                 fprintf(stderr, "[nanokappa_hip] copy probe, %d-byte accesses: %.1f us per pass over %lld particles (%.2f TB/s)\n", w, 100.0 * ms,
-                        (long long)ns, (ctx->d.nts ? 88.0 : 72.0) * ns / (ms * 1e-4) / 1e12);
+                        (long long)ns, 2.0 * nk_particle_bytes(false, (bool)ctx->d.nts) * ns / (ms * 1e-4) / 1e12);
             }
         }
         hipEventDestroy(e0); hipEventDestroy(e1);
     }
-    if (bytes_read) *bytes_read = ns * (ctx->d.nts ? 44 : 36);
-    if (bytes_written) *bytes_written = ns * (ctx->d.nts ? 32 : 24);
+    if (bytes_read) *bytes_read = ns * nk_particle_bytes(false, (bool)ctx->d.nts);
+    if (bytes_written) *bytes_written = ns * (nk_particle_bytes(false, (bool)ctx->d.nts) - 8 - nk_word_bytes(!ctx->d.nts));
     return NK_OK;
 }
 int nk_uniform2(uint64_t seed, uint64_t pid, uint32_t step, uint32_t tag, double *u0, double *u1) {
diff --git a/nanokappa_amd/csrc/nk_fgroups.hip b/nanokappa_amd/csrc/nk_fgroups.hip
--- a/nanokappa_amd/csrc/nk_fgroups.hip
+++ b/nanokappa_amd/csrc/nk_fgroups.hip
@@ -43,7 +43,7 @@
         const int32_t *gs = q.gtab + (int64_t)seg * q.gstride;
         for (int k = threadIdx.x; k < count; k += blockDim.x) {
             const int64_t i = base + k;
-            const int idx = (int)(d.w0[i] & lbmask);
+            const int idx = (int)(d.w0.get(i) & lbmask);
             const int g = idx < q.glim ? gs[idx] : -1;
             if ((unsigned)g >= (unsigned)q.G) { n_ung += 1u; continue; }
             const NkMode *rec = sm.rec + idx;
diff --git a/nanokappa_amd/csrc/nk_kernels.h b/nanokappa_amd/csrc/nk_kernels.h
--- a/nanokappa_amd/csrc/nk_kernels.h
+++ b/nanokappa_amd/csrc/nk_kernels.h
@@ -451,7 +451,7 @@
                 d.x.p[q.od] = xa; d.y.p[q.od] = ya; d.z.p[q.od] = za;
                 d.occ.p[q.od] = occ;
                 if (!BOX) d.nts.p[q.od] = na;
-                d.w0.p[q.ow] = BOX ? (NK_NEWBORN | (uint32_t)idx) : (NK_NEWBORN | ((uint32_t)(facet + 1) << d.lb) | (uint32_t)idx);
+                d.w0.put_at_as<BOX>(q.ow, BOX ? (NK_NEWBORN | (uint32_t)idx) : (NK_NEWBORN | ((uint32_t)(facet + 1) << d.lb) | (uint32_t)idx));
                 if (d.pid) d.pid.p[q.od] = pid;
             } else if (!(ahead && d.halt[1])) atomicOr(d.overflow, 1);
         }
@@ -543,7 +543,7 @@
         NK_ST(q, px); NK_ST(q + B::O_Y, py); NK_ST(q + B::O_Z, pz); NK_ST(q + B::O_OCC, pocc);
         if (!BOX) NK_ST(q + B::O_NTS, pnts);
         if (PID) NK_ST(reinterpret_cast<unsigned long long *>(q + B::O_PID), ppid);
-        NK_ST(B::word(d.x.p, i), pw0);
+        NK_ST(B::word(d.x.p, i), B::narrow(pw0));
     }
     template <bool BOX = false>
     __device__ __forceinline__ void store(const NkDev &d, int64_t base, bool put, int o, double px, double py, double pz, double pocc,
@@ -579,7 +579,7 @@
             if (lane < n) {
                 const int e = (ob + lane) & (NK_ORING - 1);
                 const int64_t i = base + wout + lane;
-                d.x[i] = x[e]; d.y[i] = y[e]; d.z[i] = z[e]; d.occ[i] = occ[e]; d.nts[i] = nts[e]; d.w0[i] = w0[e];
+                d.x[i] = x[e]; d.y[i] = y[e]; d.z[i] = z[e]; d.occ[i] = occ[e]; d.nts[i] = nts[e]; d.w0.put(i, w0[e]);
                 if (PID) d.pid[i] = (unsigned long long)__double_as_longlong(pid[e]);
             }
             wout += n;
@@ -688,7 +688,7 @@
             if (PF2) {
                 typedef NkBlock<!BOX, PID> B;
                 const double *px = B::tile(d.x.p, i0, lane), *py = px + B::O_Y, *pz = px + B::O_Z, *po = px + B::O_OCC, *pn = px + B::O_NTS;
-                const uint32_t *pw = B::word(d.x.p, i0) + lane;
+                const typename B::Word *pw = B::word(d.x.p, i0) + lane;
                 asm volatile("global_load_dword %0, %1, off" : "=v"(b.w0) : "v"(pw) : "memory");
                 asm volatile("global_load_dwordx2 %0, %1, off" : "=v"(b.x) : "v"(px) : "memory");
                 asm volatile("global_load_dwordx2 %0, %1, off" : "=v"(b.y) : "v"(py) : "memory");
@@ -701,7 +701,8 @@
             if (rr + lane >= lo && rr + lane < hi && r < nA * NK_TILE) {
                 typedef NkBlock<!BOX, PID> B;
                 const double *q = B::tile(d.x.p, i0, lane);
-                b.w0 = NK_LD(B::word(d.x.p, i0) + lane); b.x = NK_LD(q); b.y = NK_LD(q + B::O_Y); b.z = NK_LD(q + B::O_Z); b.occ = NK_LD(q + B::O_OCC);
+                b.w0 = NK_LD(B::word(d.x.p, i0) + lane); b.x = NK_LD(q);
+                b.y = NK_LD(q + B::O_Y); b.z = NK_LD(q + B::O_Z); b.occ = NK_LD(q + B::O_OCC);
                 if (!BOX) b.nts = NK_LD(q + B::O_NTS);
                 if (PID) b.pid = NK_LD(reinterpret_cast<const unsigned long long *>(q + B::O_PID));
             }
@@ -741,7 +742,7 @@
             if (!flush) {
                 const int r = t * NK_TILE;
                 { const int rr = down ? bhi - r : blo + r; act = rr + lane >= lo && rr + lane < hi; }
-                w0 = buf.w0; x = buf.x; y = buf.y; z = buf.z; occ = buf.occ; nts = buf.nts; pid = buf.pid;
+                w0 = NkBlock<!BOX, PID>::widen(buf.w0); x = buf.x; y = buf.y; z = buf.z; occ = buf.occ; nts = buf.nts; pid = buf.pid;
             }
             if (DEFER) {
                 asm volatile("" : "+v"(x), "+v"(y), "+v"(z), "+v"(occ), "+v"(nts), "+v"(w0));
@@ -1176,7 +1177,7 @@
                 if (slo + o < d.segcap) {
                     const int64_t i = (int64_t)seg * d.segcap + slo + o;
                     const NkSlot q = nk_slot(d, i);
-                    d.x.p[q.od] = p.x; d.y.p[q.od] = p.y; d.z.p[q.od] = p.z; d.occ.p[q.od] = p.occ; d.nts.p[q.od] = p.nts; d.w0.p[q.ow] = w0e;
+                    d.x.p[q.od] = p.x; d.y.p[q.od] = p.y; d.z.p[q.od] = p.z; d.occ.p[q.od] = p.occ; d.nts.p[q.od] = p.nts; d.w0.put_at(q.ow, w0e);
                     if (PID) d.pid.p[q.od] = pid;
                 } else atomicOr(d.overflow, 4);
             } else {
@@ -1223,14 +1224,14 @@
             uint32_t vw = 0u;
             uint64_t vp = 0;
             if (on) {
-                vx = d.x.p[qs.od]; vy = d.y.p[qs.od]; vz = d.z.p[qs.od]; vo = d.occ.p[qs.od]; vw = d.w0.p[qs.ow];
+                vx = d.x.p[qs.od]; vy = d.y.p[qs.od]; vz = d.z.p[qs.od]; vo = d.occ.p[qs.od]; vw = d.w0.raw_at(qs.ow);
                 if (d.nts.p) vn = d.nts.p[qs.od];
                 if (d.pid.p) vp = d.pid.p[qs.od];
             }
             asm volatile("s_waitcnt vmcnt(0)" ::: "memory");
             __builtin_amdgcn_fence(__ATOMIC_SEQ_CST, "wavefront");
             if (on) {
-                d.x.p[qd.od] = vx; d.y.p[qd.od] = vy; d.z.p[qd.od] = vz; d.occ.p[qd.od] = vo; d.w0.p[qd.ow] = vw;
+                d.x.p[qd.od] = vx; d.y.p[qd.od] = vy; d.z.p[qd.od] = vz; d.occ.p[qd.od] = vo; d.w0.put_raw_at(qd.ow, vw);
                 if (d.nts.p) d.nts.p[qd.od] = vn;
                 if (d.pid.p) d.pid.p[qd.od] = vp;
             }
@@ -1247,7 +1248,7 @@
         for (int i = threadIdx.x; i < cnt; i += blockDim.x) {
             n.x[b + i] = o.x[a + i]; n.y[b + i] = o.y[a + i]; n.z[b + i] = o.z[a + i];
             n.occ[b + i] = o.occ[a + i]; if (o.nts && n.nts) n.nts[b + i] = o.nts[a + i];
-            n.w0[b + i] = o.w0[a + i];
+            n.w0.put_raw_at(n.w0.off(b + i), o.w0.raw_at(o.w0.off(a + i)));
             if (o.pid && n.pid) n.pid[b + i] = o.pid[a + i];
         }
         if (threadIdx.x == 0) n.seg_count[seg] = cnt;
@@ -1270,7 +1271,7 @@
             const double2 a = r[0], b = r[1], c = r[2], e = r[3];
             d.x[base + j] = a.x; d.y[base + j] = a.y; d.z[base + j] = b.x; d.occ[base + j] = b.y; if (d.nts) d.nts[base + j] = c.x;
             d.pid[base + j] = (uint64_t)__double_as_longlong(c.y);
-            d.w0[base + j] = (uint32_t)__double_as_longlong(e.x);
+            d.w0.put(base + j, (uint32_t)__double_as_longlong(e.x));
         }
         if (lane == 0) {
             d.seg_count[seg] = count + n;
@@ -1573,7 +1574,7 @@
         const NkSegModes sm = nk_seg_modes(d, seg);
         for (int k = threadIdx.x; k < count; k += NK_WG) {
             const int64_t i = base + k;
-            const int idx = (int)(d.w0[i] & lbmask);
+            const int idx = (int)(d.w0.get(i) & lbmask);
             const double4 *mrec = reinterpret_cast<const double4 *>(sm.rec + idx);
             const double4 ra = mrec[0], rb = mrec[1];
             d.occ[i] = nk_relax(d, L, tw, ra, rb, d.x[i], d.y[i], d.z[i], d.occ[i], sm, idx);
@@ -1593,7 +1594,7 @@
         const NkSegModes sm = nk_seg_modes(d, seg);
         for (int k = threadIdx.x; k < count; k += NK_WG) {
             const int64_t i = base + k;
-            const uint32_t idx = d.w0[i] & lbmask;
+            const uint32_t idx = d.w0.get(i) & lbmask;
             const NkMode *rec = sm.rec + idx;
             double tc; int fc;
             const double x = d.x[i], y = d.y[i], z = d.z[i];
@@ -1601,10 +1602,10 @@
             if (d.box) {
                 const bool inside = x >= d.box_k[0] && x <= -d.box_k[1] && y >= d.box_k[2] && y <= -d.box_k[3] && z >= d.box_k[4] && z <= -d.box_k[5];
                 if (!inside && fc >= 0) atomicAdd(anomalies, 1);
-                d.w0[i] = (fc < 0 ? NK_LOST : 0u) | idx;
+                d.w0.put(i, (fc < 0 ? NK_LOST : 0u) | idx);
             } else {
                 d.nts[i] = tc / d.dt;
-                d.w0[i] = ((uint32_t)(fc + 1) << d.lb) | idx;
+                d.w0.put(i, ((uint32_t)(fc + 1) << d.lb) | idx);
             }
         }
     }
@@ -1621,7 +1622,7 @@
         const NkSegModes sm = nk_seg_modes(d, seg);
         for (int k = threadIdx.x; k < count; k += NK_WG) {
             const int64_t i = base + k;
-            const uint32_t w0 = d.w0[i];
+            const uint32_t w0 = d.w0.get(i);
             if (w0 & NK_LOST) { nts_out[i] = __builtin_inf(); facet_out[i] = -1; continue; }
             const NkMode *rec = sm.rec + (w0 & lbmask);
             double x = d.x[i], y = d.y[i], z = d.z[i];
@@ -1730,7 +1731,7 @@
         const int slot = atomicAdd(d.seg_count + seg, 1);
         if (slot < d.segcap) {
             const int64_t o = (int64_t)seg * d.segcap + slot;
-            d.x[o] = x; d.y[o] = y; d.z[o] = z; d.occ[o] = occ; if (d.nts) d.nts[o] = 0.0; d.w0[o] = (uint32_t)idx;
+            d.x[o] = x; d.y[o] = y; d.z[o] = z; d.occ[o] = occ; if (d.nts) d.nts[o] = 0.0; d.w0.put(o, (uint32_t)idx);
             if (d.pid) d.pid[o] = pid;
         } else atomicOr(d.overflow, 2);
     }
@@ -1747,7 +1748,7 @@
         const NkSegModes sm = nk_seg_modes(d, seg);
         for (int k = threadIdx.x; k < count; k += NK_WG) {
             const int64_t i = base + k;
-            const NkMode *rec = sm.rec + (d.w0[i] & lbmask);
+            const NkMode *rec = sm.rec + (d.w0.get(i) & lbmask);
             nk_tally_one(d, L.tb, L.bins, d.x[i], d.y[i], d.z[i], d.occ[i], rec->omega, rec->E0, rec->vx, rec->vy, rec->vz, true, rep);
         }
     }
@@ -1774,7 +1775,7 @@
         const NkSegModes sm = nk_seg_modes(d, seg);
         for (int k = threadIdx.x; k < count; k += blockDim.x) {
             const int64_t i = base + k;
-            const int idx = (int)(d.w0[i] & lbmask);
+            const int idx = (int)(d.w0.get(i) & lbmask);
             const int b = band_of_mode[sm.mode(idx)] - b0;
             if ((unsigned)b >= (unsigned)Bt) continue;
             const NkMode *rec = sm.rec + idx;
@@ -1863,7 +1864,7 @@
         const NkSegModes sm = nk_seg_modes(d, seg);
         for (int k = threadIdx.x; k < count; k += blockDim.x) {
             const int64_t i = base + k;
-            const int idx = (int)(d.w0[i] & lbmask);
+            const int idx = (int)(d.w0.get(i) & lbmask);
             const NkMode *rec = sm.rec + idx;
             const double x = d.x[i], y = d.y[i], z = d.z[i];
             double e;
@@ -1990,7 +1991,7 @@
         const int nb = (m.owner && live) ? sm.nl * S : 0;
         for (int k = tl; k < count; k += tsize) {
             const int64_t i = base + k;
-            const int idx = (int)(d.w0[i] & lbmask);
+            const int idx = (int)(d.w0.get(i) & lbmask);
             const NkMode *rec = sm.rec + idx;
             const double x = d.x[i], y = d.y[i], z = d.z[i];
             const int s = nk_classify(d, L.tb, x, y, z);
@@ -2075,7 +2076,7 @@
             bool out = x < d.bbox[0] - 1e-10 || y < d.bbox[1] - 1e-10 || z < d.bbox[2] - 1e-10 || x > d.bbox[3] + 1e-10 ||
                        y > d.bbox[4] + 1e-10 || z > d.bbox[5] + 1e-10;
             if (!out) continue;
-            const uint32_t idx = d.w0[i] & lbmask;
+            const uint32_t idx = d.w0.get(i) & lbmask;
             const uint64_t pid = d.pid ? d.pid[i] : nk_state_key(sm.mode((int)idx), x, y, z);
             double u[6];
             nk_uniform2_dev(d.seed, pid, step, NK_TAG_RESAMP + 0, u[0], u[1]);
@@ -2092,8 +2093,8 @@
             double tc; int fc;
             NK_RAY(GEOM, d, L, NK_TREE_NO_SKIP, x, y, z, rec->vx, rec->vy, rec->vz, tc, fc);
             d.x[i] = x; d.y[i] = y; d.z[i] = z;
-            if (d.box) d.w0[i] = (fc < 0 ? NK_LOST : 0u) | idx;
-            else { d.nts[i] = tc / d.dt; d.w0[i] = ((uint32_t)(fc + 1) << d.lb) | idx; }
+            if (d.box) d.w0.put(i, (fc < 0 ? NK_LOST : 0u) | idx);
+            else { d.nts[i] = tc / d.dt; d.w0.put(i, ((uint32_t)(fc + 1) << d.lb) | idx); }
         }
     }
 }
@@ -2178,7 +2179,7 @@
         const int count = d.seg_count[seg];
         for (int k = threadIdx.x; k < count; k += NK_WG) {
             const int64_t i = base + k;
-            uint32_t w0 = d.w0[i];
+            uint32_t w0 = d.w0.get(i);
             double x = d.x[i], y = d.y[i], z = d.z[i], occ = d.occ[i], nts = d.nts ? d.nts[i] : 0.0;
             asm volatile("" : "+v"(w0), "+v"(occ));
             d.x[i] = x; d.y[i] = y; d.z[i] = z; if (d.nts) d.nts[i] = nts;
@@ -2194,12 +2195,12 @@
         const int64_t base = (int64_t)seg * d.segcap;
         const int count = d.seg_count[seg] & ~63;
         double xN = 0, yN = 0, zN = 0, oN = 0, nN = 0; uint32_t wN = 0;
-        if (count > 0) { const int64_t i0 = base; xN = *d.x.tile(i0, lane); yN = *d.y.tile(i0, lane); zN = *d.z.tile(i0, lane); oN = *d.occ.tile(i0, lane); if (hn) nN = *d.nts.tile(i0, lane); wN = *d.w0.tile(i0, lane); }
+        if (count > 0) { const int64_t i0 = base; xN = *d.x.tile(i0, lane); yN = *d.y.tile(i0, lane); zN = *d.z.tile(i0, lane); oN = *d.occ.tile(i0, lane); if (hn) nN = *d.nts.tile(i0, lane); wN = d.w0.raw_at(d.w0.off(i0) + lane); }
         for (int r = 0; r < count; r += 64) {
             const double x = xN, y = yN, z = zN, o = oN, n = nN; const uint32_t w = wN;
-            if (r + 64 < count) { const int64_t i0 = base + r + 64; xN = *d.x.tile(i0, lane); yN = *d.y.tile(i0, lane); zN = *d.z.tile(i0, lane); oN = *d.occ.tile(i0, lane); if (hn) nN = *d.nts.tile(i0, lane); wN = *d.w0.tile(i0, lane); }
+            if (r + 64 < count) { const int64_t i0 = base + r + 64; xN = *d.x.tile(i0, lane); yN = *d.y.tile(i0, lane); zN = *d.z.tile(i0, lane); oN = *d.occ.tile(i0, lane); if (hn) nN = *d.nts.tile(i0, lane); wN = d.w0.raw_at(d.w0.off(i0) + lane); }
             const int64_t i0 = base + r;
-            *d.x.tile(i0, lane) = x + 1e-300; *d.y.tile(i0, lane) = y; *d.z.tile(i0, lane) = z; *d.occ.tile(i0, lane) = o; if (hn) *d.nts.tile(i0, lane) = n; *d.w0.tile(i0, lane) = w;
+            *d.x.tile(i0, lane) = x + 1e-300; *d.y.tile(i0, lane) = y; *d.z.tile(i0, lane) = z; *d.occ.tile(i0, lane) = o; if (hn) *d.nts.tile(i0, lane) = n; d.w0.put_raw_at(d.w0.off(i0) + lane, w);
         }
     }
 }
@@ -2212,13 +2213,13 @@
         const int64_t step = 64;
         const int count = tiles;
         double xN = 0, yN = 0, zN = 0, oN = 0, nN = 0; uint32_t wN = 0;
-        if (count > 0) { const int64_t i0 = base; xN = *d.x.tile(i0, lane); yN = *d.y.tile(i0, lane); zN = *d.z.tile(i0, lane); oN = *d.occ.tile(i0, lane); if (hn) nN = *d.nts.tile(i0, lane); wN = *d.w0.tile(i0, lane); }
+        if (count > 0) { const int64_t i0 = base; xN = *d.x.tile(i0, lane); yN = *d.y.tile(i0, lane); zN = *d.z.tile(i0, lane); oN = *d.occ.tile(i0, lane); if (hn) nN = *d.nts.tile(i0, lane); wN = d.w0.raw_at(d.w0.off(i0) + lane); }
         for (int r = 0; r < count; ++r) {
             double x = xN, y = yN, z = zN, o = oN, n = nN; uint32_t w = wN;
-            if (r + 1 < count) { const int64_t i0 = base + (r + 1) * step; xN = *d.x.tile(i0, lane); yN = *d.y.tile(i0, lane); zN = *d.z.tile(i0, lane); oN = *d.occ.tile(i0, lane); if (hn) nN = *d.nts.tile(i0, lane); wN = *d.w0.tile(i0, lane); }
+            if (r + 1 < count) { const int64_t i0 = base + (r + 1) * step; xN = *d.x.tile(i0, lane); yN = *d.y.tile(i0, lane); zN = *d.z.tile(i0, lane); oN = *d.occ.tile(i0, lane); if (hn) nN = *d.nts.tile(i0, lane); wN = d.w0.raw_at(d.w0.off(i0) + lane); }
             asm volatile("" : "+v"(x), "+v"(y), "+v"(z), "+v"(o), "+v"(n), "+v"(w));
             const int64_t i0 = base + r * step;
-            *d.x.tile(i0, lane) = x; *d.y.tile(i0, lane) = y; *d.z.tile(i0, lane) = z; *d.occ.tile(i0, lane) = o; if (hn) *d.nts.tile(i0, lane) = n; *d.w0.tile(i0, lane) = w;
+            *d.x.tile(i0, lane) = x; *d.y.tile(i0, lane) = y; *d.z.tile(i0, lane) = z; *d.occ.tile(i0, lane) = o; if (hn) *d.nts.tile(i0, lane) = n; d.w0.put_raw_at(d.w0.off(i0) + lane, w);
         }
     }
 }
```

Result: no change. 54.39 billion, median of 4 (+1.0%).
